# HipGraph/iSpLib

Measured on AMD Instinct MI355X. Metric: edges_aggregated_per_sec, higher is better.
Workload: dtype f32

## Files before the change

### include/isplib_hip.h

```cpp
#ifndef ISPLIB_HIP_H
#define ISPLIB_HIP_H

#include <stddef.h>
#include <stdint.h>

#ifdef __cplusplus
extern "C" {
#endif

#define ISPLIB_HIP_ABI_VERSION 1
#define ISPLIB_MAX_SLICES 4096

#define ISPLIB_VOP_COPY_RHS 0x2
#define ISPLIB_ROP_NOOP     0x00
#define ISPLIB_SOP_COPY     0x100
#define ISPLIB_VSC_MUL      0x1000
#define ISPLIB_VSC_MEAN     0x3000
#define ISPLIB_AOP_ADD      0x10000
#define ISPLIB_AOP_MAX      0x20000
#define ISPLIB_AOP_MIN      0x30000
#define ISPLIB_MSG_SPMM_SUM  (ISPLIB_VOP_COPY_RHS | ISPLIB_ROP_NOOP | ISPLIB_SOP_COPY | ISPLIB_VSC_MUL  | ISPLIB_AOP_ADD)
#define ISPLIB_MSG_SPMM_MEAN (ISPLIB_VOP_COPY_RHS | ISPLIB_ROP_NOOP | ISPLIB_SOP_COPY | ISPLIB_VSC_MEAN | ISPLIB_AOP_ADD)
#define ISPLIB_MSG_SPMM_MAX  (ISPLIB_VOP_COPY_RHS | ISPLIB_ROP_NOOP | ISPLIB_SOP_COPY | ISPLIB_VSC_MUL  | ISPLIB_AOP_MAX)
#define ISPLIB_MSG_SPMM_MIN  (ISPLIB_VOP_COPY_RHS | ISPLIB_ROP_NOOP | ISPLIB_SOP_COPY | ISPLIB_VSC_MUL  | ISPLIB_AOP_MIN)
// ... 103 lines not shown
                              const int64_t *pntrb, const int64_t *pntre,
                              const int64_t *sliceptr, int slices,
                              const float *y, int64_t ldy, float *z, int64_t ldz,
                              int64_t *z_arg, void *workspace,
                              size_t workspace_bytes, void *stream);

int    fusedMM_csr_sliced_phase_hip(int32_t imessage, int64_t m, int64_t n, int64_t k,
                                    int64_t nnz, const float *val, const int64_t *indx,
                                    const int64_t *pntrb, const int64_t *pntre,
                                    const int64_t *sliceptr, int slices,
                                    int slice_first, int slice_count, int combine,
                                    const float *y, int64_t ldy, float *z, int64_t ldz,
                                    int64_t *z_arg, void *workspace,
                                    size_t workspace_bytes, void *stream);

typedef struct isplib_task_plan_info {
   int64_t n_tasks;
   int64_t lane_off[9];
   int32_t slices, chunk, short_row, reserved;
} isplib_task_plan_info;

size_t isplib_spmm_tasks_plan_workspace_bytes(int64_t m, int slices);
int    isplib_spmm_tasks_count_hip(int64_t m, const int64_t *pntrb, const int64_t *pntre,
                                   const int64_t *sliceptr, int slices, int chunk, int short_row,
                                   int32_t *seg_off , void *workspace,
                                   size_t workspace_bytes, isplib_task_plan_info *info ,
                                   void *stream);
int    isplib_spmm_tasks_fill_hip(int64_t m, const int64_t *pntrb, const int64_t *pntre,
                                  const int64_t *sliceptr, const isplib_task_plan_info *info,
                                  const int32_t *seg_off, int32_t *task_row, int64_t *task_b,
                                  int32_t *task_len, void *stream);
size_t isplib_spmm_tasks_workspace_bytes(int32_t imessage, int64_t n_tasks, int64_t k);
int    isplib_pack_indices_hip(int64_t nnz, const int64_t *indx, int32_t *indx32, void *stream);
int    fusedMM_csr_tasks_hip(int32_t imessage, int64_t m, int64_t n, int64_t k, int64_t nnz,
                             const float *val, const int64_t *indx, const int32_t *indx32,
                             const int64_t *pntrb, const int64_t *pntre,
                             int64_t n_tasks, const int32_t *task_row,
                             const int64_t *task_b, const int32_t *task_len,
                             const int32_t *seg_off, int slices,
                             const int64_t *lane_off_host ,
                             const float *y, int64_t ldy, float *z, int64_t ldz,
                             int64_t *z_arg, void *workspace, size_t workspace_bytes,
                             void *stream);

typedef struct isplib_epilogue {
   const float *row_scale;
   const float *self;
   int64_t      ld_self;
   const float *bias;
   int          relu;
} isplib_epilogue;
int    fusedMM_csr_tasks_epilogue_hip(int32_t imessage, int64_t m, int64_t n, int64_t k, int64_t nnz,
                                      const float *val, const int64_t *indx, const int32_t *indx32,
                                      const int64_t *pntrb, const int64_t *pntre,
                                      int64_t n_tasks, const int32_t *task_row,
                                      const int64_t *task_b, const int32_t *task_len,
                                      const int32_t *seg_off, int slices,
                                      const int64_t *lane_off_host ,
                                      const float *y, int64_t ldy, float *z, int64_t ldz,
                                      void *workspace, size_t workspace_bytes,
                                      const isplib_epilogue *epilogue ,
                                      void *stream);

int    isplib_row_scale_hip(int64_t n, int64_t k, const float *x , int64_t ldx, const float *scale ,
                            float *y , int64_t ldy, void *stream);
size_t isplib_masked_scale_colsum_workspace_bytes(int64_t n, int64_t k);
int    isplib_masked_scale_colsum_hip(int64_t n, int64_t k, const float *dz, int64_t lddz, const float *out ,
                                      int64_t ldo, const float *scale , float *gy ,
                                      int64_t ldgy, float *grad_bias , void *workspace, size_t workspace_bytes,
                                      void *stream);

typedef struct isplib_stream_plan {
   int64_t rows, cols;
   int32_t slices, gens, waves_per_gen, rows_per_wave, streams , chunk ;
   int64_t n_steps, n_parts, n_hub;
   const int32_t *words;
   const float   *vals;
   const int64_t *wave_step_off;
   const int32_t *wave_row;
   const int32_t *wave_part;
   const int32_t *hub_row;
   const int32_t *hub_off;
   const int32_t *perm;
} isplib_stream_plan;
int  isplib_stream_plan_build_hip(int64_t m, int64_t n, int64_t nnz, const int64_t *rowptr, const int64_t *col,
                                  const float *val, int streams, int slices, int chunk, int waves_per_gen,
                                  isplib_stream_plan *out , void *stream);
#define ISPLIB_STREAM_CAP_ONE 4096u
int  isplib_stream_capacities_hip(int device, int streams, int waves_per_gen, int64_t nnz, uint32_t *caps ,
                                  int *levelled , void *stream);
int  isplib_stream_plan_build_caps_hip(int64_t m, int64_t n, int64_t nnz, const int64_t *rowptr, const int64_t *col,
                                       const float *val, int streams, int slices, int chunk, int waves_per_gen,
                                       const uint32_t *caps , isplib_stream_plan *out , void *stream);
int  isplib_stream_plan_set_values_hip(isplib_stream_plan *plan, const float *val , void *stream);
void isplib_stream_plan_free(isplib_stream_plan *plan);
int    isplib_spmm_stream_geometry(int streams, int *rows_per_wave , int *waves_resident );
int    isplib_suggest_stream(int64_t m, int64_t n, int64_t nnz, int64_t k, int *streams, int *slices, int *chunk);
int    isplib_suggest_stream_weighted(int64_t m, int64_t n, int64_t nnz, int64_t k, int weighted, int *streams, int *slices, int *chunk);
int    isplib_spmm_stream_minmax_geometry(int streams , int *rows_per_wave , int *waves_resident );
int    isplib_suggest_stream_minmax(int64_t m, int64_t n, int64_t nnz, int64_t k, int *streams, int *slices, int *chunk);
int    isplib_stream_plan_build_minmax_hip(int64_t m, int64_t n, int64_t nnz, const int64_t *rowptr, const int64_t *col,
                                           const float *val, int streams, int slices, int chunk, int waves_per_gen,
                                           isplib_stream_plan *out , void *stream);
size_t isplib_spmm_stream_minmax_workspace_bytes(const isplib_stream_plan *plan);
int    fusedMM_csr_stream_minmax_hip(int32_t imessage , int64_t m, int64_t n, int64_t k,
                                     int64_t nnz, const int64_t *pntrb, const int64_t *pntre,
                                     const isplib_stream_plan *plan ,
                                     const float *y, int64_t ldy, float *z, int64_t ldz, int64_t *z_arg,
                                     void *workspace, size_t workspace_bytes, void *stream);
size_t isplib_spmm_stream_workspace_bytes(const isplib_stream_plan *plan);
int    fusedMM_csr_stream_hip(int32_t imessage , int64_t m, int64_t n, int64_t k,
                              int64_t nnz, const int64_t *pntrb, const int64_t *pntre,
                              const isplib_stream_plan *plan ,
                              const float *y, int64_t ldy, float *z, int64_t ldz,
                              void *workspace, size_t workspace_bytes,
                              const isplib_epilogue *epilogue , void *stream);
#define ISPLIB_DTYPE_BF16 1
#define ISPLIB_DTYPE_F16  2
int    fusedMM_csr_stream16_hip(int32_t imessage , int dtype, int64_t m, int64_t n, int64_t k,
                                int64_t nnz, const int64_t *pntrb, const int64_t *pntre,
                                const isplib_stream_plan *plan ,
                                const void *y, int64_t ldy, void *z, int64_t ldz,
                                void *workspace, size_t workspace_bytes, void *stream);
static inline int isplib_stream16_native_pays(int streams, int weighted) {
   (void)streams; (void)weighted;
   return 0;
}
int    isplib_stream16_auto(int streams, int weighted);
int    fusedMM_csr_rows16_hip(int32_t imessage , int dtype ,
                              int64_t m, int64_t n, int64_t k, int64_t nnz, const float *val ,
                              const int64_t *indx, const int64_t *pntrb, const int64_t *pntre,
                              const int32_t *row_order , const void *y, int64_t ldy, void *z, int64_t ldz, void *stream);
static inline int isplib_rows16_native_pays(int64_t n, int64_t ldy, int ordered, int weighted) {
   const int beyond = n > 0 && ldy > 0 && (double)n * (double)ldy * 2.0 > 256.0 * 1048576.0;
   (void)weighted;
   return (beyond || !ordered) ? 1 : 0;
}
int    isplib_rows16_auto(int64_t n, int64_t ldy, int ordered, int weighted);
int    isplib_rows16_domain(int64_t n, int64_t k, int64_t ldy, int64_t ldz);
int    fusedMM_csr_rows16_colscale_hip(int32_t imessage , int dtype ,
                                       int64_t m, int64_t n, int64_t k, int64_t nnz, const float *col_scale ,
                                       const int64_t *indx, const int64_t *pntrb, const int64_t *pntre,
                                       const int32_t *row_order , const void *y, int64_t ldy, void *z, int64_t ldz, void *stream);
static inline int isplib_rows16_colscale_native_pays(int64_t n, int64_t ldy, int ordered) {
   const int beyond = n > 0 && ldy > 0 && (double)n * (double)ldy * 2.0 > 256.0 * 1048576.0;
   return (beyond || !ordered) ? 1 : 0;
}
int    isplib_rows16_colscale_auto(int64_t n, int64_t ldy, int ordered);
typedef struct isplib_epilogue16 {
   const float *row_scale;
   const float *self_scale;
   const float *bias;
   int          relu;
} isplib_epilogue16;
int    fusedMM_csr_rows16_epilogue_hip(int dtype , int64_t m, int64_t n, int64_t k, int64_t nnz,
                                       const float *col_scale , const int64_t *indx, const int64_t *pntrb,
                                       const int64_t *pntre, const int32_t *row_order , const void *y, int64_t ldy, void *z,
                                       int64_t ldz, const isplib_epilogue16 *epilogue , void *stream);
static inline int isplib_rows16_gcn_native_pays(int64_t n, int64_t ldy, int ordered) {
   (void)ordered;
   return (n > 0 && ldy > 0 && (double)n * (double)ldy * 2.0 > 256.0 * 1048576.0) ? 1 : 0;
}
int    isplib_rows16_gcn_auto(int64_t n, int64_t ldy, int ordered);
size_t isplib_masked_colsum16_workspace_bytes(int64_t n, int64_t k);
int    isplib_masked_colsum16_hip(int dtype, int64_t n, int64_t k, const void *dz, int64_t lddz, const void *out , int64_t ldo,
                                  void *g , int64_t ldg, float *grad_bias , void *workspace,
                                  size_t workspace_bytes, void *stream);
// ... 265 lines not shown
```

### isplib_amd/cabi.py

```python
from __future__ import annotations

import ctypes
import os
from typing import Optional

import torch

from . import _lib

MSG_SPMM_SUM = 0x2 | 0x00 | 0x100 | 0x1000 | 0x10000
MSG_SPMM_MEAN = 0x2 | 0x00 | 0x100 | 0x3000 | 0x10000
MSG_SPMM_MAX = 0x2 | 0x00 | 0x100 | 0x1000 | 0x20000
MSG_SPMM_MIN = 0x2 | 0x00 | 0x100 | 0x1000 | 0x30000
MESSAGE = {"sum": MSG_SPMM_SUM, "add": MSG_SPMM_SUM, "mean": MSG_SPMM_MEAN, "max": MSG_SPMM_MAX, "min": MSG_SPMM_MIN}

SUCCESS, FAIL, NOT_ENOUGH_MEM, NO_OPT_IMPL, HIP_ERROR = 0, 1, -1, 128, 256
UNDEFINED_USER_FUNCTION = 64
ISPLIB_SUCCESS, ISPLIB_FAIL, ISPLIB_NOT_ENOUGH_MEM, ISPLIB_NO_OPT_IMPL, ISPLIB_HIP_ERROR = SUCCESS, FAIL, NOT_ENOUGH_MEM, NO_OPT_IMPL, HIP_ERROR

DENSE_BYTES_MAX = 7 * 2 ** 29
DENSE_OOB_OFFSET = 15 * 2 ** 28
STREAM_N_END = 2 ** 24
STREAM_LDY_END = 2 ** 22
STREAM_NNZ_END = 2 ** 31
# ... 65 lines not shown
        return False
    if heads > 1 and (d < 4 or d & (d - 1)):
        return False
    return ld >= heads * d and rows_gathered < 2 ** 31 and (rows_gathered <= 0 or rows_gathered * ld * 4 <= DENSE_BYTES_MAX)


def gat_edge_serves(nnz: int, heads: int) -> bool:
    return heads >= 1 and 0 <= nnz < 2 ** 31 and nnz * heads * 4 <= DENSE_BYTES_MAX


def gatv2_serves(rows_gathered: int, heads: int, d: int, ld: int) -> bool:
    return gat_serves(rows_gathered, heads, d, ld)


ATTENTION16_K_MIN, ATTENTION16_K_MAX = 8, 512


def attention16_serves(rows_gathered: int, k: int, ld: int) -> bool:
    return (ATTENTION16_K_MIN <= k <= ATTENTION16_K_MAX and k % 2 == 0 and ld % 2 == 0 and ld >= k and rows_gathered < 2 ** 31 and
            (rows_gathered <= 0 or rows_gathered * ld * 2 <= DENSE_BYTES_MAX))


def attention16_native_pays(rows_gathered: int, ld: int) -> bool:
    return bool(rows_gathered > 0 and ld > 0)


GAT16_K_MIN, GAT16_K_MAX = 8, 512


def gat16_serves(rows_gathered: int, heads: int, d: int, ld: int) -> bool:
    if heads < 1 or d < 1 or not GAT16_K_MIN <= heads * d <= GAT16_K_MAX:
        return False
    if (d % 2) if heads == 1 else (d < 8 or d & (d - 1)):
        return False
    return (ld % 2 == 0 and ld >= heads * d and rows_gathered < 2 ** 31 and
            (rows_gathered <= 0 or rows_gathered * ld * 2 <= DENSE_BYTES_MAX))


def gat16_native_pays(rows_gathered: int, ld: int) -> bool:
    return bool(rows_gathered > 0 and ld > 0)


def gatv2_16_serves(rows_gathered: int, heads: int, d: int, ld: int) -> bool:
    return gat16_serves(rows_gathered, heads, d, ld)


def gatv2_16_native_pays(rows_gathered: int, ld: int) -> bool:
    return bool(rows_gathered > 0 and ld > 0)


def owner_exchange_serves(m: int, k: int, world: int, cuts) -> bool:
    if not 1 <= world <= OWNER_WORLD_MAX or m < 0 or k < 0 or m * k >= MINMAX_BW_PAIRS_END:
        return False
    return all(cuts[p + 1] >= cuts[p] and (cuts[p + 1] - cuts[p]) * k <= MINMAX_BW_KEYS_MAX for p in range(world))


def scatter_keys_serves(total: int, n: int, k: int) -> bool:
    return 0 <= total < MINMAX_BW_PAIRS_END and n >= 0 and k >= 0 and n * k <= MINMAX_BW_KEYS_MAX

VOP = {"copy_lhs": 0x1, "copy_rhs": 0x2, "add": 0x3, "subl": 0x4, "subr": 0x5, "max": 0x6, "min": 0x7, "udef": 0xF}
ROP = {"noop": 0x00, "dot": 0x10, "add_lhs": 0x20, "add_rhs": 0x30, "norml": 0x40, "normr": 0x50, "udef": 0xF0}
SOP = {"noop": 0x000, "copy": 0x100, "udef": 0xF00}
VSC = {"noop": 0x0000, "mul": 0x1000, "add": 0x2000, "mean": 0x3000, "udef": 0xF000}
AOP = {"add": 0x10000, "max": 0x20000, "min": 0x30000, "udef": 0xF0000}
SOP_UDEF = {"none": 0, "sigmoid": 1, "one_minus_sigmoid": 2, "tdist": 3, "scale": 4, "exp": 5, "leaky_exp": 6}
PATTERNS = {
    "spmm": (MSG_SPMM_SUM, "none"),
    "sigmoid_embedding": (VOP["copy_rhs"] | ROP["dot"] | SOP["udef"] | VSC["mul"] | AOP["add"], "sigmoid"),
    "tdist_embedding": (VOP["subr"] | ROP["normr"] | SOP["udef"] | VSC["mul"] | AOP["add"], "tdist"),
    "attention_sum": (VOP["copy_rhs"] | ROP["dot"] | SOP["udef"] | VSC["mul"] | AOP["add"], "leaky_exp"),
}

EXPORTS = (
    "isplib_hip_abi_version", "isplib_hip_last_error", "isplib_hip_set_empty_row", "isplib_hip_get_empty_row", "fusedMM_csr_hip", "performDummySpMM_hip",
    "isplib_spmm_minmax_bw_hip", "isplib_sddmm_csr_hip", "isplib_csr_row_ids_hip",
    "isplib_csr2csc_workspace_bytes", "isplib_csr2csc_hip",
    "isplib_spmm_slices_bytes", "isplib_spmm_slices_build_hip", "isplib_spmm_sliced_workspace_bytes",
    "fusedMM_csr_sliced_hip", "fusedMM_csr_sliced_phase_hip", "isplib_hip_tune",
    "isplib_spmm_tasks_workspace_bytes", "fusedMM_csr_tasks_hip",
    "isplib_spmm_tasks_plan_workspace_bytes", "isplib_spmm_tasks_count_hip", "isplib_spmm_tasks_fill_hip",
    "isplib_sddmm_csr_tasks_hip", "fusedMM_csr_tasks_epilogue_hip", "fusedMM_csr_udef_hip", "fusedMM_csr_udef_tasks_hip", "isplib_pack_indices_hip",
    "isplib_suggest_slices", "isplib_graph_create", "isplib_graph_set_slices", "isplib_graph_set_values", "isplib_graph_spmm", "isplib_graph_spmm_backward",
    "isplib_graph_destroy", "isplib_suggest_slices_whole_rows", "isplib_graph_sddmm",
    "fusedMM_csr_stream_hip", "isplib_spmm_stream_workspace_bytes", "isplib_spmm_stream_geometry", "isplib_suggest_stream", "isplib_suggest_stream_weighted", "isplib_stream_plan_build_hip", "isplib_stream_plan_build_caps_hip", "isplib_stream_capacities_hip", "isplib_stream_plan_build_minmax_hip", "fusedMM_csr_stream_minmax_hip", "isplib_spmm_stream_minmax_geometry", "isplib_suggest_stream_minmax", "isplib_spmm_stream_minmax_workspace_bytes", "isplib_stream_plan_set_values_hip", "isplib_stream_plan_free", "isplib_spmm_minmax_bw_det_hip", "isplib_spmm_minmax_bw_workspace_bytes", "isplib_scatter_rows_det_hip",
    "isplib_minmax_bw_bucket_workspace_bytes", "isplib_minmax_bw_bucket_hip", "isplib_scatter_keys_workspace_bytes", "isplib_scatter_keys_det_hip",
    "isplib_fusedmm_stream_geometry", "isplib_suggest_fusedmm_stream", "isplib_stream_plan_build_fusedmm_hip", "fusedMM_csr_udef_stream_hip",
    "isplib_row_scale_hip", "isplib_masked_scale_colsum_hip", "isplib_masked_scale_colsum_workspace_bytes",
    "fusedMM_csr_ordered_hip", "isplib_community_order_hip", "isplib_community_order_workspace_bytes", "isplib_order_locality_hip",
    "isplib_graph_set_row_order", "isplib_plain_panels",
    "fusedMM_csr_stream16_hip", "isplib_stream16_auto",
    "fusedMM_csr_rows16_hip", "isplib_rows16_auto", "isplib_rows16_domain",
    "fusedMM_csr_rows16_minmax_hip", "isplib_rows16_minmax_auto",
    "fusedMM_csr_rows16_colscale_hip", "isplib_rows16_colscale_auto",
    "fusedMM_csr_rows16_epilogue_hip", "isplib_rows16_gcn_auto", "isplib_masked_colsum16_hip", "isplib_masked_colsum16_workspace_bytes",
    "isplib_sddmm_csr_rows16_hip", "isplib_sddmm_rows16_auto",
    "isplib_attention_csr_hip", "isplib_attention_bw_rows_hip", "isplib_attention_bw_cols_hip", "isplib_attention_domain",
    "isplib_attention16_csr_hip", "isplib_attention16_bw_rows_hip", "isplib_attention16_bw_cols_hip", "isplib_attention16_domain",
    "isplib_attention16_auto",
    "isplib_gat_csr_hip", "isplib_gat_bw_rows_hip", "isplib_gat_bw_cols_hip", "isplib_gat_domain",
    "isplib_gat_edge_csr_hip", "isplib_gat_edge_bw_rows_hip", "isplib_gat_edge_bw_cols_hip", "isplib_gat_edge_domain",
    "isplib_gat16_csr_hip", "isplib_gat16_bw_rows_hip", "isplib_gat16_bw_cols_hip", "isplib_gat16_domain", "isplib_gat16_auto",
    "isplib_gatv2_csr_hip", "isplib_gatv2_bw_rows_hip", "isplib_gatv2_bw_rows_workspace_bytes", "isplib_gatv2_bw_cols_hip",
    "isplib_gatv2_domain",
)

GATV2_16_EXPORTS = (
    "isplib_gatv2_16_csr_hip", "isplib_gatv2_16_bw_rows_hip", "isplib_gatv2_16_bw_rows_workspace_bytes", "isplib_gatv2_16_bw_cols_hip",
    "isplib_gatv2_16_domain", "isplib_gatv2_16_auto",
)

EXP_EXPORTS = ("fusedMM_csr_sweep_hip", "isplib_spmm_sweep_workspace_bytes", "isplib_spmm_sweep_resident_waves",
               "fusedMM_csr_hybrid_hip", "isplib_spmm_hybrid_geometry", "isplib_spmm_hybrid_workspace_bytes", "isplib_sddmm_stream_hip",
               "isplib_hip_tune_experimental")

_i64, _f32, _vp, _i32 = ctypes.c_int64, ctypes.c_float, ctypes.c_void_p, ctypes.c_int32


class Epilogue(ctypes.Structure):
    _fields_ = [("row_scale", ctypes.c_void_p), ("self", ctypes.c_void_p), ("ld_self", ctypes.c_int64),
                ("bias", ctypes.c_void_p), ("relu", ctypes.c_int)]


class TaskPlanInfo(ctypes.Structure):
    _fields_ = [("n_tasks", ctypes.c_int64), ("lane_off", ctypes.c_int64 * 9), ("slices", ctypes.c_int32),
                ("chunk", ctypes.c_int32), ("short_row", ctypes.c_int32), ("reserved", ctypes.c_int32)]


class SweepPlanStruct(ctypes.Structure):
    _fields_ = [("rows", ctypes.c_int64), ("slices", ctypes.c_int32), ("gens", ctypes.c_int32),
                ("waves_per_gen", ctypes.c_int32), ("rows_per_wave", ctypes.c_int32), ("n_tasks", ctypes.c_int64),
                ("n_parts", ctypes.c_int64), ("n_hub", ctypes.c_int64), ("wave_row", ctypes.c_void_p),
                ("wave_part", ctypes.c_void_p), ("wave_task_off", ctypes.c_void_p), ("task_b", ctypes.c_void_p),
                ("task_meta", ctypes.c_void_p), ("hub_row", ctypes.c_void_p), ("hub_off", ctypes.c_void_p)]


class StreamPlanStruct(ctypes.Structure):
    _fields_ = [("rows", ctypes.c_int64), ("cols", ctypes.c_int64), ("slices", ctypes.c_int32), ("gens", ctypes.c_int32),
                ("waves_per_gen", ctypes.c_int32), ("rows_per_wave", ctypes.c_int32), ("streams", ctypes.c_int32),
                ("chunk", ctypes.c_int32), ("n_steps", ctypes.c_int64), ("n_parts", ctypes.c_int64), ("n_hub", ctypes.c_int64),
                ("words", ctypes.c_void_p), ("vals", ctypes.c_void_p), ("wave_step_off", ctypes.c_void_p),
                ("wave_row", ctypes.c_void_p), ("wave_part", ctypes.c_void_p),
                ("hub_row", ctypes.c_void_p), ("hub_off", ctypes.c_void_p), ("perm", ctypes.c_void_p)]


class HybridPlanStruct(ctypes.Structure):
    _fields_ = [("cold", StreamPlanStruct), ("table_rows", ctypes.c_int32), ("hot_cap", ctypes.c_int32), ("n_hot_steps", ctypes.c_int64),
                ("hot_rows", ctypes.c_void_p), ("hot_words", ctypes.c_void_p), ("hot_step_off", ctypes.c_void_p),
                ("hot_perm", ctypes.c_void_p)]


_sigs_set = False


def lib() -> ctypes.CDLL:
    global _sigs_set
    L = _lib.cdll()
    if not _sigs_set:
        L.isplib_hip_abi_version.restype = ctypes.c_int
        L.isplib_hip_last_error.restype = ctypes.c_char_p
        L.fusedMM_csr_hip.restype = ctypes.c_int
        L.fusedMM_csr_hip.argtypes = [_i32, _i64, _i64, _i64, _f32, _i64, _i64, _i64, _vp, _vp, _vp, _vp,
                                      _vp, _i64, _vp, _i64, _f32, _vp, _i64, _vp, _vp]
        L.fusedMM_csr_udef_hip.restype = ctypes.c_int
        L.fusedMM_csr_udef_hip.argtypes = [_i32, _i64, _i64, _i64, _f32, _i64, _i64, _i64, _vp, _vp, _vp, _vp,
                                           _vp, _i64, _vp, _i64, _f32, _vp, _i64, _vp, ctypes.c_int, _f32, _vp]
        L.fusedMM_csr_udef_tasks_hip.restype = ctypes.c_int
        L.fusedMM_csr_udef_tasks_hip.argtypes = [_i32, _i64, _i64, _i64, _i64, _vp, _vp, _vp, _vp, _vp, _vp, _i64, _i64, _vp, _vp,
                                                 _vp, _vp, ctypes.c_int, _vp, _vp, _i64, _vp, _i64, _vp, ctypes.c_int, _f32,
                                                 _vp, ctypes.c_size_t, _vp]
        L.performDummySpMM_hip.restype = None
        L.performDummySpMM_hip.argtypes = [_i64, _vp]
        L.isplib_spmm_minmax_bw_hip.restype = ctypes.c_int
        L.isplib_spmm_minmax_bw_hip.argtypes = [_i64, _i64, _i64, _i64, _vp, _vp, _vp, _vp, _vp, _vp, _vp, _vp]
        L.isplib_sddmm_csr_hip.restype = ctypes.c_int
        L.isplib_sddmm_csr_hip.argtypes = [_i64, _i64, _vp, _vp, _vp, _vp, _i64, _vp, _i64, ctypes.c_int, _vp, _vp]
        L.isplib_csr_row_ids_hip.restype = ctypes.c_int
        L.isplib_csr_row_ids_hip.argtypes = [_i64, _i64, _vp, _vp, _vp]
        L.isplib_csr2csc_workspace_bytes.restype = ctypes.c_size_t
        L.isplib_csr2csc_workspace_bytes.argtypes = [_i64, _i64, _i64]
        L.isplib_csr2csc_hip.restype = ctypes.c_int
        L.isplib_csr2csc_hip.argtypes = [_i64, _i64, _i64, _vp, _vp, _vp, ctypes.c_int, _vp, _vp, _vp, _vp,
                                         _vp, ctypes.c_size_t, _vp]
        L.isplib_spmm_slices_bytes.restype = ctypes.c_size_t
        L.isplib_spmm_slices_bytes.argtypes = [_i64, ctypes.c_int]
        L.isplib_spmm_slices_build_hip.restype = ctypes.c_int
        L.isplib_spmm_slices_build_hip.argtypes = [_i64, _i64, _i64, _vp, _vp, _vp, ctypes.c_int, _vp, _vp, _vp]
        L.isplib_spmm_sliced_workspace_bytes.restype = ctypes.c_size_t
        L.isplib_spmm_sliced_workspace_bytes.argtypes = [_i32, _i64, _i64, ctypes.c_int]
        L.fusedMM_csr_sliced_hip.restype = ctypes.c_int
        L.fusedMM_csr_sliced_hip.argtypes = [_i32, _i64, _i64, _i64, _i64, _vp, _vp, _vp, _vp, _vp, ctypes.c_int,
                                             _vp, _i64, _vp, _i64, _vp, _vp, ctypes.c_size_t, _vp]
        L.fusedMM_csr_sliced_phase_hip.restype = ctypes.c_int
        L.fusedMM_csr_sliced_phase_hip.argtypes = [_i32, _i64, _i64, _i64, _i64, _vp, _vp, _vp, _vp, _vp, ctypes.c_int,
                                                   ctypes.c_int, ctypes.c_int, ctypes.c_int, _vp, _i64, _vp, _i64, _vp,
                                                   _vp, ctypes.c_size_t, _vp]
        L.isplib_spmm_tasks_workspace_bytes.restype = ctypes.c_size_t
        L.isplib_spmm_tasks_workspace_bytes.argtypes = [_i32, _i64, _i64]
        L.fusedMM_csr_tasks_hip.restype = ctypes.c_int
        L.isplib_pack_indices_hip.restype = ctypes.c_int
        L.isplib_pack_indices_hip.argtypes = [_i64, _vp, _vp, _vp]
        L.fusedMM_csr_tasks_hip.argtypes = [_i32, _i64, _i64, _i64, _i64, _vp, _vp, _vp, _vp, _vp, _i64, _vp, _vp, _vp, _vp,
                                            ctypes.c_int, _vp, _vp, _i64, _vp, _i64, _vp, _vp, ctypes.c_size_t, _vp]
        L.isplib_spmm_tasks_plan_workspace_bytes.restype = ctypes.c_size_t
        L.isplib_spmm_tasks_plan_workspace_bytes.argtypes = [_i64, ctypes.c_int]
        L.isplib_spmm_tasks_count_hip.restype = ctypes.c_int
        L.isplib_spmm_tasks_count_hip.argtypes = [_i64, _vp, _vp, _vp, ctypes.c_int, ctypes.c_int, ctypes.c_int, _vp, _vp,
                                                  ctypes.c_size_t, ctypes.POINTER(TaskPlanInfo), _vp]
        L.isplib_spmm_tasks_fill_hip.restype = ctypes.c_int
        L.isplib_spmm_tasks_fill_hip.argtypes = [_i64, _vp, _vp, _vp, ctypes.POINTER(TaskPlanInfo), _vp, _vp, _vp, _vp, _vp]
        L.isplib_sddmm_csr_tasks_hip.restype = ctypes.c_int
        L.isplib_sddmm_csr_tasks_hip.argtypes = [_i64, _i64, _i64, _vp, _vp, _vp, _vp, _i64, _vp, _vp, _vp, _vp, _vp, _i64, _vp,
                                                 _i64, ctypes.c_int, _vp, _vp]
        L.fusedMM_csr_tasks_epilogue_hip.restype = ctypes.c_int
        L.fusedMM_csr_tasks_epilogue_hip.argtypes = [_i32, _i64, _i64, _i64, _i64, _vp, _vp, _vp, _vp, _vp, _i64, _vp, _vp, _vp, _vp,
                                                     ctypes.c_int, _vp, _vp, _i64, _vp, _i64, _vp, ctypes.c_size_t,
                                                     ctypes.POINTER(Epilogue), _vp]
        L.isplib_suggest_slices.restype = ctypes.c_int
        L.isplib_suggest_slices.argtypes = [_i64, _i64, _i64, _i64, ctypes.c_int]
        L.isplib_graph_create.restype = ctypes.c_int
        L.isplib_graph_create.argtypes = [_i64, _i64, _i64, _vp, _vp, _vp, ctypes.POINTER(_vp)]
        L.isplib_graph_set_slices.restype = ctypes.c_int
        L.isplib_graph_set_slices.argtypes = [_vp, ctypes.c_int]
        L.isplib_graph_set_values.restype = ctypes.c_int
        L.isplib_graph_set_values.argtypes = [_vp, _vp]
        L.isplib_graph_spmm.restype = ctypes.c_int
        L.isplib_graph_spmm.argtypes = [_vp, _i32, _i64, _vp, _i64, _vp, _i64, _vp, _vp]
        L.isplib_graph_spmm_backward.restype = ctypes.c_int
        L.isplib_graph_spmm_backward.argtypes = [_vp, ctypes.c_int, _i64, _vp, _i64, _vp, _i64, _vp]
        L.isplib_suggest_slices_whole_rows.restype = ctypes.c_int
        L.isplib_suggest_slices_whole_rows.argtypes = [_i64, _i64, _i64, _i64]
        L.isplib_graph_sddmm.restype = ctypes.c_int
        L.isplib_graph_sddmm.argtypes = [_vp, ctypes.c_int, _i64, _vp, _i64, _vp, _i64, _vp, _vp]
        L.isplib_graph_destroy.restype = None
        L.isplib_graph_destroy.argtypes = [_vp]
        L.isplib_hip_tune.restype = ctypes.c_int
        L.isplib_hip_tune.argtypes = [ctypes.c_int, ctypes.c_int]
        L.isplib_spmm_minmax_bw_workspace_bytes.restype = ctypes.c_size_t
        L.isplib_spmm_minmax_bw_workspace_bytes.argtypes = [_i64, _i64, _i64]
        L.isplib_spmm_minmax_bw_det_hip.restype = ctypes.c_int
        L.isplib_spmm_minmax_bw_det_hip.argtypes = [_i64, _i64, _i64, _i64, _vp, _vp, _vp, _vp, _vp, _vp, _vp, _vp, ctypes.c_size_t, _vp]
        L.isplib_fusedmm_stream_geometry.restype = ctypes.c_int
        L.isplib_fusedmm_stream_geometry.argtypes = [ctypes.c_int, ctypes.POINTER(ctypes.c_int), ctypes.POINTER(ctypes.c_int)]
        L.isplib_suggest_fusedmm_stream.restype = ctypes.c_int
        L.isplib_suggest_fusedmm_stream.argtypes = [_i32, _i64, _i64, _i64, _i64] + [ctypes.POINTER(ctypes.c_int)] * 3
        L.isplib_stream_plan_build_fusedmm_hip.restype = ctypes.c_int
        L.isplib_stream_plan_build_fusedmm_hip.argtypes = [_i64, _i64, _i64, _vp, _vp, ctypes.c_int, ctypes.c_int, ctypes.c_int, ctypes.c_int,
                                                           ctypes.POINTER(StreamPlanStruct), _vp]
        L.fusedMM_csr_udef_stream_hip.restype = ctypes.c_int
        L.fusedMM_csr_udef_stream_hip.argtypes = [_i32, _i64, _i64, _i64, _i64, _vp, _vp, ctypes.POINTER(StreamPlanStruct), _vp, _i64, _vp, _i64,
                                                  _vp, _i64, ctypes.c_int, _f32, _vp, ctypes.c_size_t, _vp]
        L.isplib_row_scale_hip.restype = ctypes.c_int
        L.isplib_row_scale_hip.argtypes = [_i64, _i64, _vp, _i64, _vp, _vp, _i64, _vp]
        L.isplib_masked_scale_colsum_workspace_bytes.restype = ctypes.c_size_t
        L.isplib_masked_scale_colsum_workspace_bytes.argtypes = [_i64, _i64]
        L.isplib_masked_scale_colsum_hip.restype = ctypes.c_int
        L.isplib_masked_scale_colsum_hip.argtypes = [_i64, _i64, _vp, _i64, _vp, _i64, _vp, _vp, _i64, _vp, _vp, ctypes.c_size_t, _vp]
        L.isplib_scatter_rows_det_hip.restype = ctypes.c_int
        L.isplib_scatter_rows_det_hip.argtypes = [_i64, _i64, _i64, _i64, _vp, _vp, _vp, _vp, ctypes.c_size_t, _vp]
        L.isplib_minmax_bw_bucket_workspace_bytes.restype = ctypes.c_size_t
        L.isplib_minmax_bw_bucket_workspace_bytes.argtypes = [_i64, _i64, ctypes.c_int]
        L.isplib_minmax_bw_bucket_hip.restype = ctypes.c_int
        L.isplib_minmax_bw_bucket_hip.argtypes = [_i64, _i64, _i64, _i64, _vp, _vp, _vp, _vp, ctypes.c_int, ctypes.POINTER(_i64), _vp, _vp, _vp,
                                                  _vp, ctypes.c_size_t, _vp]
        L.isplib_scatter_keys_workspace_bytes.restype = ctypes.c_size_t
        L.isplib_scatter_keys_workspace_bytes.argtypes = [_i64, _i64, _i64]
        L.isplib_scatter_keys_det_hip.restype = ctypes.c_int
        L.isplib_scatter_keys_det_hip.argtypes = [_i64, _i64, _i64, _vp, _vp, _vp, _vp, ctypes.c_size_t, _vp]
        L.isplib_stream_plan_build_hip.restype = ctypes.c_int
        L.isplib_stream_plan_build_hip.argtypes = [_i64, _i64, _i64, _vp, _vp, _vp, ctypes.c_int, ctypes.c_int, ctypes.c_int, ctypes.c_int,
                                                   ctypes.POINTER(StreamPlanStruct), _vp]
        L.isplib_stream_plan_build_caps_hip.restype = ctypes.c_int
        L.isplib_stream_plan_build_caps_hip.argtypes = [_i64, _i64, _i64, _vp, _vp, _vp, ctypes.c_int, ctypes.c_int, ctypes.c_int, ctypes.c_int,
                                                        _vp, ctypes.POINTER(StreamPlanStruct), _vp]
        L.isplib_stream_capacities_hip.restype = ctypes.c_int
        L.isplib_stream_capacities_hip.argtypes = [ctypes.c_int, ctypes.c_int, ctypes.c_int, _i64, _vp, ctypes.POINTER(ctypes.c_int), _vp]
        L.isplib_stream_level_set.restype = ctypes.c_int
        L.isplib_stream_level_set.argtypes = [ctypes.c_int]
        L.isplib_stream_plan_build_minmax_hip.restype = ctypes.c_int
        L.isplib_stream_plan_build_minmax_hip.argtypes = [_i64, _i64, _i64, _vp, _vp, _vp, ctypes.c_int, ctypes.c_int, ctypes.c_int, ctypes.c_int,
                                                          ctypes.POINTER(StreamPlanStruct), _vp]
        L.isplib_spmm_stream_minmax_geometry.restype = ctypes.c_int
        L.isplib_spmm_stream_minmax_geometry.argtypes = [ctypes.c_int, ctypes.POINTER(ctypes.c_int), ctypes.POINTER(ctypes.c_int)]
        L.isplib_suggest_stream_minmax.restype = ctypes.c_int
        L.isplib_suggest_stream_minmax.argtypes = [_i64, _i64, _i64, _i64, ctypes.POINTER(ctypes.c_int), ctypes.POINTER(ctypes.c_int), ctypes.POINTER(ctypes.c_int)]
        L.isplib_spmm_stream_minmax_workspace_bytes.restype = ctypes.c_size_t
        L.isplib_spmm_stream_minmax_workspace_bytes.argtypes = [ctypes.POINTER(StreamPlanStruct)]
        L.fusedMM_csr_stream_minmax_hip.restype = ctypes.c_int
        L.fusedMM_csr_stream_minmax_hip.argtypes = [_i32, _i64, _i64, _i64, _i64, _vp, _vp, ctypes.POINTER(StreamPlanStruct), _vp, _i64,
                                                    _vp, _i64, _vp, _vp, ctypes.c_size_t, _vp]
        L.isplib_stream_plan_set_values_hip.restype = ctypes.c_int
        L.isplib_stream_plan_set_values_hip.argtypes = [ctypes.POINTER(StreamPlanStruct), _vp, _vp]
        L.isplib_stream_plan_free.restype = None
        L.isplib_stream_plan_free.argtypes = [ctypes.POINTER(StreamPlanStruct)]
        L.isplib_community_order_workspace_bytes.restype = ctypes.c_size_t
        L.isplib_community_order_workspace_bytes.argtypes = [_i64, _i64]
        L.isplib_community_order_hip.restype = ctypes.c_int
        L.isplib_community_order_hip.argtypes = [_i64, _i64, _vp, _vp, ctypes.c_int, ctypes.c_int, _vp, _vp, ctypes.POINTER(ctypes.c_int), _vp,
                                                 ctypes.c_size_t, _vp]
        L.isplib_order_locality_hip.restype = ctypes.c_int
        L.isplib_order_locality_hip.argtypes = [_i64, _i64, _vp, _vp, _vp, _i64, ctypes.POINTER(ctypes.c_double), _vp, ctypes.c_size_t, _vp]
        L.isplib_graph_set_row_order.restype = ctypes.c_int
        L.isplib_graph_set_row_order.argtypes = [_vp, _vp, _vp]
        L.fusedMM_csr_ordered_hip.restype = ctypes.c_int
        L.fusedMM_csr_ordered_hip.argtypes = [_i32, _i64, _i64, _i64, _i64, _vp, _vp, _vp, _vp, _vp, _vp, _i64, _vp, _i64, _vp, _vp]
        L.isplib_plain_panels.restype = ctypes.c_int
        L.isplib_plain_panels.argtypes = [_i64, _i64]
        L.isplib_suggest_stream.restype = ctypes.c_int
        L.isplib_suggest_stream.argtypes = [_i64, _i64, _i64, _i64, ctypes.POINTER(ctypes.c_int), ctypes.POINTER(ctypes.c_int), ctypes.POINTER(ctypes.c_int)]
        L.isplib_suggest_stream_weighted.restype = ctypes.c_int
        L.isplib_suggest_stream_weighted.argtypes = [_i64, _i64, _i64, _i64, ctypes.c_int, ctypes.POINTER(ctypes.c_int), ctypes.POINTER(ctypes.c_int), ctypes.POINTER(ctypes.c_int)]
        L.isplib_spmm_stream_geometry.restype = ctypes.c_int
        L.isplib_spmm_stream_geometry.argtypes = [ctypes.c_int, ctypes.POINTER(ctypes.c_int), ctypes.POINTER(ctypes.c_int)]
        L.isplib_spmm_stream_workspace_bytes.restype = ctypes.c_size_t
        L.isplib_spmm_stream_workspace_bytes.argtypes = [ctypes.POINTER(StreamPlanStruct)]
        L.fusedMM_csr_stream_hip.restype = ctypes.c_int
        L.fusedMM_csr_stream_hip.argtypes = [_i32, _i64, _i64, _i64, _i64, _vp, _vp, ctypes.POINTER(StreamPlanStruct), _vp, _i64,
                                             _vp, _i64, _vp, ctypes.c_size_t, ctypes.POINTER(Epilogue), _vp]
        L.fusedMM_csr_stream16_hip.restype = ctypes.c_int
        L.fusedMM_csr_stream16_hip.argtypes = [_i32, ctypes.c_int, _i64, _i64, _i64, _i64, _vp, _vp, ctypes.POINTER(StreamPlanStruct), _vp, _i64,
                                               _vp, _i64, _vp, ctypes.c_size_t, _vp]
        L.isplib_stream16_auto.restype = ctypes.c_int
        L.isplib_stream16_auto.argtypes = [ctypes.c_int, ctypes.c_int]
        L.fusedMM_csr_rows16_hip.restype = ctypes.c_int
        L.fusedMM_csr_rows16_hip.argtypes = [_i32, ctypes.c_int, _i64, _i64, _i64, _i64, _vp, _vp, _vp, _vp, _vp, _vp, _i64, _vp, _i64, _vp]
        L.isplib_rows16_auto.restype = ctypes.c_int
        L.isplib_rows16_auto.argtypes = [_i64, _i64, ctypes.c_int, ctypes.c_int]
        L.isplib_rows16_domain.restype = ctypes.c_int
        L.isplib_rows16_domain.argtypes = [_i64, _i64, _i64, _i64]
        L.fusedMM_csr_rows16_minmax_hip.restype = ctypes.c_int
        L.fusedMM_csr_rows16_minmax_hip.argtypes = [_i32, ctypes.c_int, _i64, _i64, _i64, _i64, _vp, _vp, _vp, _vp, _vp, _vp, _i64, _vp, _i64, _vp, _i64, _vp]
        L.isplib_rows16_minmax_auto.restype = ctypes.c_int
        L.isplib_rows16_minmax_auto.argtypes = [_i64, _i64, ctypes.c_int, ctypes.c_int, ctypes.c_int]
        L.fusedMM_csr_rows16_colscale_hip.restype = ctypes.c_int
        L.fusedMM_csr_rows16_colscale_hip.argtypes = [_i32, ctypes.c_int, _i64, _i64, _i64, _i64, _vp, _vp, _vp, _vp, _vp, _vp, _i64, _vp, _i64, _vp]
        L.isplib_rows16_colscale_auto.restype = ctypes.c_int
        L.isplib_rows16_colscale_auto.argtypes = [_i64, _i64, ctypes.c_int]
        L.fusedMM_csr_rows16_epilogue_hip.restype = ctypes.c_int
        L.fusedMM_csr_rows16_epilogue_hip.argtypes = [ctypes.c_int, _i64, _i64, _i64, _i64, _vp, _vp, _vp, _vp, _vp, _vp, _i64, _vp, _i64, _vp, _vp]
        L.isplib_rows16_gcn_auto.restype = ctypes.c_int
        L.isplib_rows16_gcn_auto.argtypes = [_i64, _i64, ctypes.c_int]
        L.isplib_masked_colsum16_workspace_bytes.restype = ctypes.c_size_t
        L.isplib_masked_colsum16_workspace_bytes.argtypes = [_i64, _i64]
        L.isplib_masked_colsum16_hip.restype = ctypes.c_int
        L.isplib_masked_colsum16_hip.argtypes = [ctypes.c_int, _i64, _i64, _vp, _i64, _vp, _i64, _vp, _i64, _vp, _vp, ctypes.c_size_t, _vp]
        L.isplib_sddmm_csr_rows16_hip.restype = ctypes.c_int
        L.isplib_sddmm_csr_rows16_hip.argtypes = [ctypes.c_int, _i64, _i64, _i64, _i64, _vp, _vp, _vp, _vp, _vp, _i64, _vp, _i64, ctypes.c_int, _vp, _vp]
        L.isplib_sddmm_rows16_auto.restype = ctypes.c_int
        L.isplib_sddmm_rows16_auto.argtypes = [_i64, _i64, ctypes.c_int]
        L.isplib_attention_domain.restype = ctypes.c_int
        L.isplib_attention_domain.argtypes = [_i64, _i64, _i64]
        L.isplib_attention_csr_hip.restype = ctypes.c_int
        L.isplib_attention_csr_hip.argtypes = [_i64, _i64, _i64, _i64, _vp, _vp, _vp, _vp, _i64, _vp, _i64, _f32, _vp, _i64, _vp, _vp]
        L.isplib_attention_bw_rows_hip.restype = ctypes.c_int
        L.isplib_attention_bw_rows_hip.argtypes = [_i64, _i64, _i64, _i64, _vp, _vp, _vp, _vp, _i64, _vp, _i64, _f32, _vp, _i64, _vp, _i64, _vp,
                                                   _vp, _i64, _vp, _vp]
        L.isplib_attention_bw_cols_hip.restype = ctypes.c_int
        L.isplib_attention_bw_cols_hip.argtypes = [_i64, _i64, _i64, _i64, _vp, _vp, _vp, _vp, _i64, _vp, _i64, _f32, _vp, _i64, _vp, _vp, _vp,
                                                   _i64, _vp]
# ... 2138 lines not shown
    return tuple(x.value for x in v)


def fusedMM_csr_hybrid_hip(imessage: int, rowptr, nnz: int, plan, y, z, workspace=None, epilogue=None, check: bool = True) -> int:
    assert y.is_cuda and y.dtype == torch.float32 and y.dim() == 2 and y.stride(1) == 1
    m, n, k = rowptr.numel() - 1, y.size(0), y.size(1)
    rp = rowptr.data_ptr()
    ps = plan.struct()
    with torch.cuda.device(y.device):
        st = exp_lib().fusedMM_csr_hybrid_hip(int(imessage), m, n, k, int(nnz), ctypes.c_void_p(rp), ctypes.c_void_p(rp + 8),
                                          ctypes.byref(ps), _ptr(y), y.stride(0) if n > 1 else max(k, y.stride(0)), _ptr(z),
                                          z.stride(0) if m > 1 else max(k, z.stride(0)), _ptr(workspace),
                                          0 if workspace is None else workspace.numel(),
                                          None if epilogue is None else ctypes.byref(epilogue), _stream(y.device))
    if check:
        _check(st, "fusedMM_csr_hybrid_hip")
    return st


def spmm_hybrid(rowptr, nnz: int, plan, y, reduce: str = "sum", workspace=None, row_scale=None, self_term=None, bias=None, relu=False):
    rowptr = _dev(rowptr, "rowptr", torch.int64)
    y = y.contiguous()
    m, k = rowptr.numel() - 1, y.size(1)
    out = torch.empty((m, k), dtype=torch.float32, device=y.device)
    if workspace is None:
        workspace = plan.workspace()
    ep = None
    if row_scale is not None or self_term is not None or bias is not None or relu:
        ep = Epilogue(None if row_scale is None else row_scale.data_ptr(), None if self_term is None else self_term.data_ptr(),
                      k if self_term is None else self_term.stride(0), None if bias is None else bias.data_ptr(), int(bool(relu)))
    fusedMM_csr_hybrid_hip(MESSAGE[reduce], rowptr, nnz, plan, y, out, workspace, ep)
    return out


def suggest_stream(m: int, n: int, nnz: int, k: int, weighted: bool = False):
    st, sl, ch = ctypes.c_int(0), ctypes.c_int(0), ctypes.c_int(0)
    if not lib().isplib_suggest_stream_weighted(int(m), int(n), int(nnz), int(k), int(bool(weighted)), ctypes.byref(st), ctypes.byref(sl), ctypes.byref(ch)):
        return None
    return st.value, sl.value, ch.value


class _DevView:

    def __init__(self, ptr: int, count: int, typestr: str, owner=None):
        self.__cuda_array_interface__ = {"shape": (count,), "typestr": typestr, "data": (ptr, False), "version": 2}
        self._owner = owner


class NativeStreamPlan:

    def __init__(self, rowptr, col, val, ncols: int, streams: int, slices: int, chunk: int, waves_per_gen: int = 0,
                 minmax: bool = False, fusedmm: bool = False, capacities=None):
        assert capacities is None or not (minmax or fusedmm), "max / min and FusedMM plans keep equal capacities"
        self._s = StreamPlanStruct()
        self.device = col.device
        m = rowptr.numel() - 1
        with torch.cuda.device(col.device):
            if fusedmm:
                _check(lib().isplib_stream_plan_build_fusedmm_hip(m, int(ncols), col.numel(), _ptr(rowptr), _ptr(col), int(streams), int(slices),
                                                                  int(chunk), int(waves_per_gen), ctypes.byref(self._s), _stream(col.device)),
                       "isplib_stream_plan_build_fusedmm_hip")
            elif minmax:
                _check(lib().isplib_stream_plan_build_minmax_hip(m, int(ncols), col.numel(), _ptr(rowptr), _ptr(col), _ptr(val),
                                                                 int(streams), int(slices), int(chunk), int(waves_per_gen), ctypes.byref(self._s),
                                                                 _stream(col.device)), "isplib_stream_plan_build_minmax_hip")
            elif capacities is not None:
                caps = (ctypes.c_uint32 * len(capacities))(*[int(c) for c in capacities])
                rpw, resident = stream_geometry(streams)
                if len(caps) != (int(waves_per_gen) if waves_per_gen > 0 else resident):
                    raise ValueError("one capacity per wave of a generation")
                _check(lib().isplib_stream_plan_build_caps_hip(m, int(ncols), col.numel(), _ptr(rowptr), _ptr(col), _ptr(val), int(streams),
                                                               int(slices), int(chunk), int(waves_per_gen), ctypes.cast(caps, _vp),
                                                               ctypes.byref(self._s), _stream(col.device)), "isplib_stream_plan_build_caps_hip")
            else:
                _check(lib().isplib_stream_plan_build_hip(m, int(ncols), col.numel(), _ptr(rowptr), _ptr(col), _ptr(val), int(streams),
                                                          int(slices), int(chunk), int(waves_per_gen), ctypes.byref(self._s),
                                                          _stream(col.device)), "isplib_stream_plan_build_hip")
        for name in ("rows", "cols", "slices", "gens", "waves_per_gen", "rows_per_wave", "streams", "n_steps", "n_parts", "n_hub"):
            setattr(self, name, int(getattr(self._s, name)))

    def struct(self):
        return self._s

    def workspace(self, minmax: bool = False):
        L = lib()
        nbytes = (L.isplib_spmm_stream_minmax_workspace_bytes if minmax else L.isplib_spmm_stream_workspace_bytes)(ctypes.byref(self._s))
        return torch.empty(nbytes, dtype=torch.uint8, device=self.device)

    def set_values(self, val):
        with torch.cuda.device(self.device):
            _check(lib().isplib_stream_plan_set_values_hip(ctypes.byref(self._s), _ptr(val), _stream(self.device)), "isplib_stream_plan_set_values_hip")

    def array(self, name: str) -> torch.Tensor:
        nw = self.gens * self.waves_per_gen
        count, typestr = {"words": (self.n_steps * self.streams, "<i4"), "perm": (self.n_steps * self.streams, "<i4"),
                          "vals": (self.n_steps * self.streams, "<f4"), "wave_step_off": (nw + 1, "<i8"),
                          "wave_row": (nw * self.rows_per_wave, "<i4"), "wave_part": (nw * self.rows_per_wave, "<i4"),
                          "hub_row": (self.n_hub, "<i4"), "hub_off": (self.n_hub + 1, "<i4")}[name]
        ptr = getattr(self._s, name)
        if not ptr or count == 0:
            return torch.empty(0, device=self.device)
        return torch.as_tensor(_DevView(ptr, count, typestr), device=self.device).clone()

    def view(self, name: str, dtype: torch.dtype) -> torch.Tensor:
        nw = self.gens * self.waves_per_gen
        count, typestr = {"words": (self.n_steps * self.streams, "<i4"), "perm": (self.n_steps * self.streams, "<i4"),
                          "wave_step_off": (nw + 1, "<i8"), "wave_row": (nw * self.rows_per_wave, "<i4"),
                          "wave_part": (nw * self.rows_per_wave, "<i4"), "hub_row": (self.n_hub, "<i4"),
                          "hub_off": (self.n_hub + 1, "<i4")}[name]
        ptr = getattr(self._s, name)
        if not ptr or count == 0:
            return torch.empty(0, dtype=dtype, device=self.device)
        t = torch.as_tensor(_DevView(ptr, count, typestr, owner=self), device=self.device)
        assert t.dtype == dtype and t.data_ptr() == ptr, "zero-copy view of a library array"
        return t

    def close(self):
        if self._s.words or self._s.wave_row:
            lib().isplib_stream_plan_free(ctypes.byref(self._s))

    def __del__(self):
        try:
            self.close()
        except Exception:
            pass


STREAM_CAP_ONE = 4096


def stream_capacities(device, streams: int, waves_per_gen: int, nnz: int):
    device = torch.device(device)
    if device.type != "cuda":
        return None
    _, resident = stream_geometry(streams)
    wpg = int(waves_per_gen) if waves_per_gen > 0 else resident
    caps = (ctypes.c_uint32 * wpg)()
    levelled = ctypes.c_int(0)
    with torch.cuda.device(device):
        _check(lib().isplib_stream_capacities_hip(-1, int(streams), wpg, int(nnz), ctypes.cast(caps, _vp), ctypes.byref(levelled),
                                                  _stream(device)), "isplib_stream_capacities_hip")
    return list(caps) if levelled.value else None


def stream_level_set(mode: int) -> None:
    _check(lib().isplib_stream_level_set(int(mode)), "isplib_stream_level_set")


def stream_geometry(streams: int = 4):
    rpw, res = ctypes.c_int(0), ctypes.c_int(0)
    _check(lib().isplib_spmm_stream_geometry(int(streams), ctypes.byref(rpw), ctypes.byref(res)), "isplib_spmm_stream_geometry")
    return rpw.value, res.value


def sweep_resident_waves(reduce: str, k: int, rows_per_wave: int = 16) -> int:
    return int(exp_lib().isplib_spmm_sweep_resident_waves(MESSAGE[reduce], int(k), int(rows_per_wave)))


class GraphHandle:

    def __init__(self, rowptr, col, val, ncols: int):
        self.rowptr = _dev(rowptr, "rowptr", torch.int64)
        self.col = _dev(col, "col", torch.int64)
        self.val = None if val is None else _dev(val, "val", torch.float32)
        self.m, self.n = self.rowptr.numel() - 1, int(ncols)
        self._cols_ok = None
        self._h = ctypes.c_void_p()
        with torch.cuda.device(self.col.device):
            _check(lib().isplib_graph_create(self.m, self.n, self.col.numel(), _ptr(self.rowptr), _ptr(self.col),
                                             _ptr(self.val), ctypes.byref(self._h)), "isplib_graph_create")

    def set_slices(self, slices: int) -> None:
        _check(lib().isplib_graph_set_slices(self._h, int(slices)), "isplib_graph_set_slices")

    def set_row_order(self, order, order_t=None) -> None:
        self.order = None if order is None else _dev(order, "order", torch.int32)
        self.order_t = None if order_t is None else _dev(order_t, "order_t", torch.int32)
        assert self.order is None or self.order.numel() == self.m
        assert self.order_t is None or self.order_t.numel() == self.n
        _check(lib().isplib_graph_set_row_order(self._h, _ptr(self.order), _ptr(self.order_t)), "isplib_graph_set_row_order")

    def set_values(self, val) -> None:
        self.val = None if val is None else _dev(val, "val", torch.float32)
        assert self.val is None or self.val.numel() == self.col.numel()
        _check(lib().isplib_graph_set_values(self._h, _ptr(self.val)), "isplib_graph_set_values")

    def spmm(self, y: torch.Tensor, reduce: str = "sum"):
        if not (y.is_cuda and y.dtype == torch.float32 and y.dim() == 2 and y.stride(1) == 1 and y.stride(0) >= y.size(1)):
            y = _dev(y, "y", torch.float32)
        k = y.size(1)
        ldy = y.stride(0) if y.size(0) > 1 else max(k, y.stride(0))
        out = torch.empty((self.m, k), dtype=torch.float32, device=y.device)
        arg = torch.empty((self.m, k), dtype=torch.int64, device=y.device) if reduce in ("max", "min") else None
        with torch.cuda.device(y.device):
            _check(lib().isplib_graph_spmm(self._h, MESSAGE[reduce], k, _ptr(y), ldy, _ptr(out), k, _ptr(arg), _stream(y.device)),
                   "isplib_graph_spmm")
        return out, arg

    def spmm_backward(self, dy: torch.Tensor, mean: bool = False) -> torch.Tensor:
        dy = _dev(dy, "dy", torch.float32)
        k = dy.size(1)
        dx = torch.empty((self.n, k), dtype=torch.float32, device=dy.device)
        with torch.cuda.device(dy.device):
            _check(lib().isplib_graph_spmm_backward(self._h, int(bool(mean)), k, _ptr(dy), k, _ptr(dx), k, _stream(dy.device)),
                   "isplib_graph_spmm_backward")
        return dx

    def sddmm(self, y: torch.Tensor, g: torch.Tensor, mean: bool = False, *, out=None, check: bool = True) -> torch.Tensor:
        _, _, out, ldy, ldg = _sddmm_operands(self.rowptr, self.col, y, g, out, False, self.n, "the handle")
        if check and self._cols_ok is None:
            self._cols_ok = self.col.numel() == 0 or (int(self.col.min()) >= 0 and int(self.col.max()) < self.n)
        if check and not self._cols_ok:
            raise ValueError(f"isplib_amd: the handle's column ids must lie in [0, {self.n})")
        k = y.size(1)
        with torch.cuda.device(y.device):
            _check(lib().isplib_graph_sddmm(self._h, int(bool(mean)), k, _ptr(y), ldy, _ptr(g), ldg, _ptr(out), _stream(y.device)),
                   "isplib_graph_sddmm")
        return out

    def close(self) -> None:
        if self._h:
            lib().isplib_graph_destroy(self._h)
            self._h = ctypes.c_void_p()

    def __del__(self):
        try:
            self.close()
# ... 3 lines not shown
```

### isplib_amd/csrc/common.h

```cpp
#pragma once
#include <hip/hip_runtime.h>
#include <stdio.h>
#include <string.h>

#include "../../include/isplib_hip.h"

namespace isplib {

char *error_buffer();
int empty_row_init();

int stream_stage_mode();
void stream_stage_report(unsigned panels);
int stream_kernel_calibrate(int streams, int waves_per_gen, int launches, int degree, int col_mult, double *wave_ticks, hipStream_t st);
int stream_level_mode();

inline void clear_error() { error_buffer()[0] = '\0'; }

inline int fail(int code, const char *msg) {
   snprintf(error_buffer(), 512, "%s", msg);
   return code;
}

inline int fail(int code, const char *entry, const char *msg) {
   snprintf(error_buffer(), 512, "%s: %s", entry, msg);
   return code;
}

inline int hip_fail(hipError_t e, const char *what) {
   snprintf(error_buffer(), 512, "%s: %s", what, hipGetErrorString(e));
   return ISPLIB_HIP_ERROR;
}

__attribute__((noinline)) inline int check_launch(const char *what) {
   const hipError_t e = hipGetLastError();
   return e == hipSuccess ? ISPLIB_SUCCESS : hip_fail(e, what);
}

#define ISPLIB_HIP_TRY(expr)                                        \
   do {                                                             \
      const hipError_t e_ = (expr);                                 \
      if (e_ != hipSuccess) return ::isplib::hip_fail(e_, #expr);   \
   } while (0)

}
```

### isplib_amd/csrc/runtime.hip

```cpp
#include <stdlib.h>
#include <string.h>

#include "common.h"

namespace isplib {
char *error_buffer() {
   static thread_local char buf[512] = {0};
   return buf;
}
}

namespace isplib {
static int g_empty_row = -1;
int empty_row_init() {
   if (g_empty_row < 0) {
      const char *e = getenv("ISPLIB_EMPTY_ROW");
      g_empty_row = (e && (strcmp(e, "init") == 0 || strcmp(e, "1") == 0)) ? 1 : 0;
   }
   return g_empty_row;
}
}

extern "C" int isplib_hip_set_empty_row(int init) {
   isplib::clear_error();
   if (init != 0 && init != 1) return isplib::fail(ISPLIB_FAIL, "isplib_hip_set_empty_row: 0 (zero) or 1 (the launcher's init value)");
   isplib::g_empty_row = init;
   return ISPLIB_SUCCESS;
}
extern "C" int isplib_hip_get_empty_row(void) { return isplib::empty_row_init(); }

namespace isplib {
static int g_stream_stage = -1;
static thread_local unsigned g_stream_stage_last = 0;
int stream_stage_mode() {
   if (g_stream_stage < 0) {
      const char *e = getenv("ISPLIB_STREAM_STAGE");
      g_stream_stage = !e ? ISPLIB_STAGE_AUTO : strcmp(e, "0") == 0 ? ISPLIB_STAGE_OFF : strcmp(e, "1") == 0 ? ISPLIB_STAGE_FORCE : ISPLIB_STAGE_AUTO;
   }
   return g_stream_stage;
}
void stream_stage_report(unsigned panels) { g_stream_stage_last = panels; }
}

extern "C" int isplib_stream_stage_set(int mode) {
   isplib::clear_error();
   if (mode != ISPLIB_STAGE_OFF && mode != ISPLIB_STAGE_FORCE && mode != ISPLIB_STAGE_AUTO) return isplib::fail(ISPLIB_FAIL, "isplib_stream_stage_set: 0 (off), 1 (force) or 2 (auto)");
   isplib::g_stream_stage = mode;
   return ISPLIB_SUCCESS;
}
extern "C" unsigned isplib_stream_stage_last(void) { return isplib::g_stream_stage_last; }

namespace isplib {
static int g_stream_level = -1;
int stream_level_mode() {
   if (g_stream_level < 0) {
      const char *e = getenv("ISPLIB_STREAM_LEVEL");
      g_stream_level = !e ? 2 : strcmp(e, "0") == 0 ? 0 : strcmp(e, "1") == 0 ? 1 : 2;
   }
   return g_stream_level;
}
}

extern "C" int isplib_stream_level_set(int mode) {
   isplib::clear_error();
   if (mode < 0 || mode > 2) return isplib::fail(ISPLIB_FAIL, "isplib_stream_level_set: 0 (off), 1 (on) or 2 (auto)");
   isplib::g_stream_level = mode;
   return ISPLIB_SUCCESS;
}

extern "C" int isplib_hip_abi_version(void) { return ISPLIB_HIP_ABI_VERSION; }
extern "C" const char *isplib_hip_last_error(void) { return isplib::error_buffer(); }
```

### isplib_amd/csrc/spmm_sweep.hip

```cpp
#include <vector>

#include "sweep_common.h"

extern "C" void isplib_debug_wave_times(unsigned long long *buf);

namespace isplib {

template <int LPR, bool HAS_VAL, int NVMAX, int NBW, int WGS, bool TIMED = false>
__global__ __launch_bounds__(256, (stream_wgs_per_cu<LPR, NVMAX, WGS>())) void spmm_stream_kernel(const SweepArgs a) {
   using Wave = StreamWave<LPR, NVMAX, NBW>;
   constexpr int WAVES = Wave::WAVES, G = Wave::G, PANEL = Wave::PANEL, U = Wave::U, PER = Wave::PER;
   constexpr int WAVE_FLOATS = NVMAX * PANEL;
   static_assert(NVMAX <= 256 && NVMAX % G == 0, "the local row is the top byte of a word");
   __shared__ __attribute__((aligned(16))) float s_all[WAVES * WAVE_FLOATS];
   Wave sw;
   if (!stream_wave_id(a, sw)) return;
   const int lane = sw.lane;
   unsigned long long t_start = 0, t_loop = 0, t_loop_end = 0;
   if constexpr (TIMED) t_start = __builtin_amdgcn_s_memtime();
   float *my = s_all + sw.wave * WAVE_FLOATS;
   for (int i = lane * 4; i < WAVE_FLOATS; i += 256)
      *reinterpret_cast<float4 *>(my + i) = make_float4(0.0f, 0.0f, 0.0f, 0.0f);
   __amdgpu_buffer_rsrc_t rsrc = dense_rsrc(a);
   stream_columns<true>(a, sw);
   float *lane_base = my + sw.lc * 4;
   stream_bounds(a, sw);
   const float *vp = HAS_VAL ? a.vals + sw.s0 * G : nullptr;
   unsigned w1[NBW], w2[NBW];
   float v0[NBW] = {}, v1[NBW] = {};
   v4i_t t[U];
   unsigned la[U];
   const unsigned pad_word = stream_pad_own_row(a, sw);
   stream_load_batch(sw, sw.wp, 0, pad_word, w1);
   if (HAS_VAL) stream_load_batch(sw, vp, 0, 0.0f, v0);
#pragma unroll
   for (int u = 0; u < U; u++) stream_issue<ISPLIB_EXP_GATHER_AUX>(sw, rsrc, w1, u, la[u], t[u]);
   stream_load_batch(sw, sw.wp, 64 * NBW, pad_word, w1);
   if (HAS_VAL) stream_load_batch(sw, vp, 64 * NBW, 0.0f, v1);
   stream_load_batch(sw, sw.wp, 128 * NBW, pad_word, w2);
   unsigned cur = (unsigned)(sw.g * PER * PANEL);
   float acc[4] = {0.0f, 0.0f, 0.0f, 0.0f};
   const int64_t nb = (sw.nwords + 64 * NBW - 1) / (64 * NBW);
   if constexpr (TIMED) t_loop = __builtin_amdgcn_s_memtime();
   for (int64_t b = 0; b < nb; b++) {
      float vnext = HAS_VAL ? __shfl(v0[0], sw.g) : 0.0f;
#pragma unroll
      for (int u = 0; u < U; u++) {
         const float vcur = vnext;
         if (HAS_VAL && u + 1 < U) vnext = __shfl(v0[((u + 1) * G) / 64], ((u + 1) * G) % 64 + sw.g);
         if (la[u] != cur) {
            stream_flush(lane_base + cur, acc);
            cur = la[u];
            acc[0] = acc[1] = acc[2] = acc[3] = 0.0f;
         }
#pragma unroll
         for (int v = 0; v < 4; v++) {
            const float x = __int_as_float(t[u][v]);
            acc[v] = HAS_VAL ? fmaf(vcur, x, acc[v]) : acc[v] + x;
         }
         stream_issue<ISPLIB_EXP_GATHER_AUX>(sw, rsrc, w1, u, la[u], t[u]);
      }
#pragma unroll
      for (int q = 0; q < NBW; q++) { w1[q] = w2[q]; v0[q] = v1[q]; }
      stream_load_batch(sw, sw.wp, (b + 3) * 64 * NBW, pad_word, w2);
      if (HAS_VAL) stream_load_batch(sw, vp, (b + 2) * 64 * NBW, 0.0f, v1);
   }
   stream_flush(lane_base + cur, acc);
   if constexpr (TIMED) t_loop_end = __builtin_amdgcn_s_memtime();
   int row_[PER], part_[PER];
#pragma unroll
   for (int jj = 0; jj < PER; jj++) {
      row_[jj] = sw.cok ? a.wave_row[(size_t)sw.w * NVMAX + sw.g * PER + jj] : -1;
      part_[jj] = a.wave_part[(size_t)sw.w * NVMAX + sw.g * PER + jj];
   }
#pragma unroll 4
   for (int jj = 0; jj < PER; jj++) {
      const int lrow = sw.g * PER + jj;
      const int row = row_[jj];
      if (row < 0) continue;
      const int part = part_[jj];
      const float4 t4 = *reinterpret_cast<const float4 *>(lane_base + lrow * PANEL);
      float v[4] = {t4.x, t4.y, t4.z, t4.w};
      int bi[4] = {INT_MAX, INT_MAX, INT_MAX, INT_MAX};
      const int c = sw.ccol;
      if (part >= 0) {
         store_tail<4>(a.part_val + (size_t)part * (size_t)a.k + c, v, sw.vfirst);
         continue;
      }
      int64_t arg[4];
      finish_row<OP_ADD>(a, row, c, v, bi, arg);
      store_tail<4>(a.z + (size_t)row * (size_t)a.ldz + c, v, sw.vfirst);
   }
   if constexpr (TIMED) if (a.dbg && lane == 0) {
      a.dbg[(size_t)sw.wl * 5 + 0] = t_start;
      a.dbg[(size_t)sw.wl * 5 + 1] = t_loop;
      a.dbg[(size_t)sw.wl * 5 + 2] = t_loop_end;
      a.dbg[(size_t)sw.wl * 5 + 3] = __builtin_amdgcn_s_memtime();
      a.dbg[(size_t)sw.wl * 5 + 4] = (__builtin_amdgcn_s_getreg(20u | (3u << 11)) << 24) | ((__builtin_amdgcn_s_getreg(4u | (31u << 11)) >> 8) & 0xFFFFu);
   }
}

typedef float v2f_t __attribute__((ext_vector_type(2)));

template <int OP, int LPR, bool HAS_VAL, int NVMAX, int NBW, int WGS, bool ARG>
__global__ __launch_bounds__(256, (stream_wgs_per_cu<LPR, 2 * (NVMAX + 1), WGS>())) void spmm_stream_minmax_kernel(const SweepArgs a) {
   using Wave = StreamWave<LPR, NVMAX, NBW>;
   constexpr int WAVES = Wave::WAVES, G = Wave::G, PANEL = Wave::PANEL, U = Wave::U, PER = Wave::PER;
   constexpr int ROWS = NVMAX + 1;
   constexpr int WAVE_DWORDS = 2 * ROWS * PANEL;
   constexpr int IDX0 = ROWS * PANEL;
   constexpr int NONE = INT_MAX;
   static_assert(ROWS <= 256 && NVMAX % G == 0, "the local row (and the spare row) is the top byte of a word");
   __shared__ __attribute__((aligned(16))) float s_all[WAVES * WAVE_DWORDS];
   Wave sw;
   if (!stream_wave_id(a, sw)) return;
   const int lane = sw.lane;
   float *my = s_all + sw.wave * WAVE_DWORDS;
   for (int i = lane * 4; i < ROWS * PANEL; i += 256)
      *reinterpret_cast<float4 *>(my + i) = make_float4(identity<OP>(), identity<OP>(), identity<OP>(), identity<OP>());
   if (ARG)
      for (int i = lane * 4; i < ROWS * PANEL; i += 256)
         *reinterpret_cast<int4 *>(my + IDX0 + i) = make_int4(INT_MAX, INT_MAX, INT_MAX, INT_MAX);
   __amdgpu_buffer_rsrc_t rsrc = dense_rsrc(a);
   stream_columns<true>(a, sw);
   const unsigned cbyte = sw.cok ? sw.cbyte : 0x80000000u;
   float *lane_base = my + sw.lc * 4;
   int *lane_idx = reinterpret_cast<int *>(my + IDX0) + sw.lc * 4;
   stream_bounds(a, sw);
   const float *vp = HAS_VAL ? a.vals + sw.s0 * G : nullptr;
   const unsigned pad_word = stream_pad_spare_row(a, sw);
   const int g4 = sw.g * 4;
   unsigned w1[NBW], w2[NBW];
   float v0[NBW] = {}, v1[NBW] = {};
   v4i_t t[U];
   unsigned la[U];
   auto fetch = [&](int u, const unsigned (&word_l)[NBW]) {
      return (unsigned)__builtin_amdgcn_ds_bpermute(g4 + (int)(((u * G) % 64) * 4), (int)word_l[(u * G) / 64]);
   };
   auto issue = [&](int u, unsigned word) {
      const unsigned o = __umul24(word, sw.ldyb) + cbyte;
      la[u] = word;
      t[u] = __builtin_amdgcn_raw_buffer_load_b128(rsrc, (int)o, 0, 0);
   };
   stream_load_batch(sw, sw.wp, 0, pad_word, w1);
   if (HAS_VAL) stream_load_batch(sw, vp, 0, 0.0f, v0);
#pragma unroll
   for (int u = 0; u < U; u++) issue(u, fetch(u, w1));
// ... 64 lines not shown
   const int32_t *ids = a.ids + sw.s0 * G;
   int row_[PER], part_[PER], best_[PER][4];
   float val_[PER][4];
#pragma unroll
   for (int jj = 0; jj < PER; jj++) {
      const int lrow = sw.g * PER + jj;
      row_[jj] = sw.cok ? a.wave_row[(size_t)sw.w * NVMAX + lrow] : -1;
      part_[jj] = a.wave_part[(size_t)sw.w * NVMAX + lrow];
      const float4 t4 = *reinterpret_cast<const float4 *>(lane_base + lrow * PANEL);
      val_[jj][0] = t4.x; val_[jj][1] = t4.y; val_[jj][2] = t4.z; val_[jj][3] = t4.w;
      if constexpr (ARG) {
         const int4 i4 = *reinterpret_cast<const int4 *>(lane_idx + lrow * PANEL);
         best_[jj][0] = i4.x; best_[jj][1] = i4.y; best_[jj][2] = i4.z; best_[jj][3] = i4.w;
      } else {
         best_[jj][0] = best_[jj][1] = best_[jj][2] = best_[jj][3] = INT_MAX;
      }
   }
   if constexpr (ARG) {
#pragma unroll
      for (int jj = 0; jj < PER; jj++)
#pragma unroll
         for (int i = 0; i < 4; i++)
            best_[jj][i] = (row_[jj] >= 0 && (unsigned)best_[jj][i] < (unsigned)sw.nwords) ? ids[best_[jj][i]] : INT_MAX;
   }
#pragma unroll
   for (int jj = 0; jj < PER; jj++) {
      const int row = row_[jj];
      if (row < 0) continue;
      const int c = sw.ccol;
      if (part_[jj] >= 0) {
         const size_t po = (size_t)part_[jj] * (size_t)a.k + c;
         store_tail<4>(a.part_val + po, val_[jj], sw.vfirst);
         if constexpr (ARG) {
#pragma unroll
            for (int i = 0; i < 4; i++) if (i >= sw.vfirst) a.part_idx[po + i] = best_[jj][i];
         }
         continue;
      }
      int64_t arg[4];
      finish_row<OP>(a, row, c, val_[jj], best_[jj], arg);
      store_tail<4>(a.z + (size_t)row * (size_t)a.ldz + c, val_[jj], sw.vfirst);
      if (a.z_arg) {
         int64_t *ar = a.z_arg + (size_t)row * (size_t)a.ldz + c;
#pragma unroll
         for (int i = 0; i < 4; i++) if (i >= sw.vfirst) ar[i] = arg[i];
      }
   }
}


__global__ __launch_bounds__(256) void stream_stage_copy_kernel(const float *__restrict__ y, int64_t ldy, int64_t n, float *__restrict__ dst) {
   const int64_t total = n * 16;
   const int64_t stride = (int64_t)gridDim.x * blockDim.x;
   for (int64_t i = (int64_t)blockIdx.x * blockDim.x + threadIdx.x; i < total; i += stride) {
      const int64_t r = i >> 4;
      const int j = (int)(i & 15) * 4;
      *reinterpret_cast<float4 *>(dst + r * (ISPLIB_STREAM_STAGE_PITCH / 4) + j) = *reinterpret_cast<const float4 *>(y + r * ldy + j);
   }
}

static int launch_stage_copy(const float *y, int64_t ldy, int64_t n, float *dst, hipStream_t st) {
   int64_t blocks = (n * 16 + 255) / 256;
   if (blocks > 4096) blocks = 4096;
   if (blocks <= 0) return ISPLIB_SUCCESS;
   hipLaunchKernelGGL(stream_stage_copy_kernel, dim3((unsigned)blocks), dim3(256), 0, st, y, ldy, n, dst);
   return check_launch("stream_stage_copy_kernel");
}

static thread_local unsigned long long *g_dbg = nullptr;
static thread_local int g_dbg_launch = 0;
template <int STREAMS, bool HAS_VAL>
static int launch_stream(const SweepArgs &a_in, hipStream_t st) {
   constexpr StreamGeom ge = stream_geom(STREAM_SUM, STREAMS);
   SweepArgs a = a_in;
   const unsigned blocks = (unsigned)((a.wave_count + 3) / 4);
   if (blocks == 0) return ISPLIB_SUCCESS;
   if constexpr (!HAS_VAL) {
      if (g_dbg) {
         a.dbg = g_dbg + (size_t)(g_dbg_launch++ % 4) * (size_t)a.wave_count * 5;
         hipLaunchKernelGGL((spmm_stream_kernel<ge.lpr, false, ge.nvmax, ge.nbw, ge.wgs, true>), dim3(blocks), dim3(256), 0, st, a);
         return check_launch("spmm_stream_kernel");
      }
   }
   hipLaunchKernelGGL((spmm_stream_kernel<ge.lpr, HAS_VAL, ge.nvmax, ge.nbw, ge.wgs>), dim3(blocks), dim3(256), 0, st, a);
   return check_launch("spmm_stream_kernel");
}

template <int OP, int STREAMS, bool HAS_VAL, bool ARG>
static void launch_minmax_kernel(const SweepArgs &a, unsigned blocks, hipStream_t st) {
   constexpr StreamGeom ge = stream_geom(STREAM_MINMAX, STREAMS);
   hipLaunchKernelGGL((spmm_stream_minmax_kernel<OP, ge.lpr, HAS_VAL, ge.nvmax, ge.nbw, ge.wgs, ARG>), dim3(blocks), dim3(256), 0, st, a);
}

template <int OP, bool HAS_VAL>
static int launch_stream_minmax(const SweepArgs &a, hipStream_t st, int streams) {
   const unsigned blocks = (unsigned)((a.wave_count + 3) / 4);
   if (blocks == 0) return ISPLIB_SUCCESS;
   return with_streams<STREAM_MINMAX>(streams, [&](auto s) {
      if (a.z_arg) launch_minmax_kernel<OP, s(), HAS_VAL, true>(a, blocks, st);
      else launch_minmax_kernel<OP, s(), HAS_VAL, false>(a, blocks, st);
      return check_launch("spmm_stream_minmax_kernel");
   });
}

}

using namespace isplib;


extern "C" int isplib_spmm_stream_geometry(int streams, int *rows_per_wave, int *waves_resident) {
   return stream_geometry("isplib_spmm_stream_geometry", STREAM_SUM, streams, rows_per_wave, waves_resident);
}

extern "C" int isplib_spmm_stream_minmax_geometry(int streams, int *rows_per_wave, int *waves_resident) {
   return stream_geometry("isplib_spmm_stream_minmax_geometry", STREAM_MINMAX, streams, rows_per_wave, waves_resident);
}

extern "C" int isplib_suggest_stream_weighted(int64_t m, int64_t n, int64_t nnz, int64_t k, int weighted, int *streams, int *slices, int *chunk) {
   clear_error();
   if (m <= 0 || n <= 0 || nnz < STREAM_MIN_NNZ) return 0;
   if (!isplib_stream_serves(n, k, k, nnz, 0)) return 0;
   int st = k <= 32 ? 8 : (k <= 64 ? 4 : (k < 128 ? 2 : 4));
   if (weighted && k >= 128 && (k % 128) == 0) st = 2;
   int rpw = 0, resident = 0;
   if (isplib_spmm_stream_geometry(st, &rpw, &resident) != ISPLIB_SUCCESS || rpw <= 0 || resident <= 0) return 0;
   if (!suggest_stream_geom(m, n, nnz, st, rpw, resident, 1.9e6, 3.4, slices, chunk)) {
      if (st != 2 || k < 128) return 0;
      st = 4;
      if (isplib_spmm_stream_geometry(st, &rpw, &resident) != ISPLIB_SUCCESS || rpw <= 0 || resident <= 0) return 0;
      if (!suggest_stream_geom(m, n, nnz, st, rpw, resident, 1.9e6, 3.4, slices, chunk)) return 0;
   }
   if (streams) *streams = st;
   return 1;
}

extern "C" int isplib_suggest_stream(int64_t m, int64_t n, int64_t nnz, int64_t k, int *streams, int *slices, int *chunk) {
   return isplib_suggest_stream_weighted(m, n, nnz, k, 0, streams, slices, chunk);
}

extern "C" int isplib_suggest_stream_minmax(int64_t m, int64_t n, int64_t nnz, int64_t k, int *streams, int *slices, int *chunk) {
   clear_error();
   if (m <= 0 || n <= 0 || nnz < STREAM_MIN_NNZ) return 0;
   if (!isplib_stream_serves(n, k, k, nnz, 1)) return 0;
   const int st = k <= 32 ? 8 : 4;
   int rpw = 0, resident = 0;
   if (isplib_spmm_stream_minmax_geometry(st, &rpw, &resident) != ISPLIB_SUCCESS || rpw <= 0 || resident <= 0) return 0;
   if (!suggest_stream_geom(m, n, nnz, st, rpw, resident, 3.3e6, st == 8 ? 1.7 : 1.17, slices, chunk)) return 0;
   if (streams) *streams = st;
   return 1;
}

extern "C" size_t isplib_spmm_stream_workspace_bytes(const isplib_stream_plan *plan) {
   size_t bytes = stream_parts_bytes(plan);
   if (plan && plan->streams == 4 && plan->cols > 0 && (uint64_t)plan->cols <= (ISPLIB_STREAM_STAGE_BYTES_MAX - ISPLIB_STREAM_STAGE_PITCH) / ISPLIB_STREAM_STAGE_PITCH)
      bytes += (size_t)plan->cols * ISPLIB_STREAM_STAGE_PITCH + ISPLIB_STREAM_STAGE_PITCH;
   return bytes;
}

extern "C" size_t isplib_spmm_stream_minmax_workspace_bytes(const isplib_stream_plan *plan) {
   return 2 * stream_parts_bytes(plan);
}

static int stream_run(int32_t imessage, int64_t m, int64_t n, int64_t k, int64_t nnz, const int64_t *pntrb, const int64_t *pntre,
                      const isplib_stream_plan *plan, const float *y, int64_t ldy, float *z, int64_t ldz, int64_t *z_arg,
                      void *workspace, size_t workspace_bytes, const isplib_epilogue *ep, void *stream) {
   clear_error();
   const char *entry = "fusedMM_csr_stream_hip";
   const bool mm = imessage == ISPLIB_MSG_SPMM_MAX || imessage == ISPLIB_MSG_SPMM_MIN;
   if (imessage != ISPLIB_MSG_SPMM_SUM && imessage != ISPLIB_MSG_SPMM_MEAN && !mm) return fail(ISPLIB_NO_OPT_IMPL, entry, "message outside the SpMM set");
   const StreamCall c = {entry, "fusedMM_csr_hip", mm ? STREAM_MINMAX : STREAM_SUM, m, n, k, nnz,  m == 0 || k == 0, pntrb, pntre, plan, y, ldy,
                          ldz,  z != nullptr,  true, workspace, workspace_bytes, (mm ? 2 : 1) * stream_parts_bytes(plan)};
   bool done;
   int rc = check_stream_call(c, &done);
   if (done) return rc;
   if (mm && plan->n_steps > 0 && !plan->perm) return fail(ISPLIB_FAIL, entry, "max / min need the plan's perm array (the winners' CSR positions)");
   if (mm && nnz >= ISPLIB_STREAM_NNZ_END) return fail(ISPLIB_FAIL, entry, "max / min need nnz < 2^31");
   if (mm && !isplib_rows_within(n, ldy, ISPLIB_STREAM_MINMAX_BYTES_END - 1u))
      return fail(ISPLIB_FAIL, "fusedMM_csr_stream_minmax_hip", "dense operand of 2 GiB or more (use fusedMM_csr_tasks_hip)");
   if ((rc = check_stream_workspace(c)) != ISPLIB_SUCCESS) return rc;
   SweepArgs a = stream_args(c, z, ldz);
   a.z_arg = z_arg;
   a.mean = imessage == ISPLIB_MSG_SPMM_MEAN ? 1 : 0;
   a.part_idx = mm && workspace ? (int *)((char *)workspace + stream_parts_bytes(plan)) : nullptr;
   if ((rc = set_epilogue(entry, ep, a)) != ISPLIB_SUCCESS) return rc;
   hipStream_t st = (hipStream_t)stream;
   const bool has_val = plan->vals != nullptr;
   const int stage_mode = mm ? ISPLIB_STAGE_OFF : stream_stage_mode();
   float *stage_base = nullptr;
   uint64_t stage_room = 0;
   if (stage_mode != ISPLIB_STAGE_OFF && workspace) {
      const uintptr_t lo = ((uintptr_t)workspace + stream_parts_bytes(plan) + (ISPLIB_STREAM_STAGE_PITCH - 1)) & ~(uintptr_t)(ISPLIB_STREAM_STAGE_PITCH - 1);
      const uintptr_t hi = (uintptr_t)workspace + workspace_bytes;
      if (lo < hi) { stage_base = (float *)lo; stage_room = hi - lo; }
   }
   unsigned staged = 0;
   auto stage = [&](SweepArgs &p, int64_t c0) {
      if (!isplib_stream_stage_panel((uint64_t)(uintptr_t)y, ldy, c0, k, plan->streams, n, nnz, stage_room, stage_mode)) return (int)ISPLIB_SUCCESS;
      const int rc = launch_stage_copy(p.y, ldy, n, stage_base, st);
      if (rc) return rc;
      p.y = stage_base;
      p.ldy = ISPLIB_STREAM_STAGE_PITCH / 4;
      p.ybytes = (unsigned)((uint64_t)n * ISPLIB_STREAM_STAGE_PITCH);
      staged |= 1u << ((c0 / 64) & 31);
      return (int)ISPLIB_SUCCESS;
   };
   const int rc_run = run_stream_panels(plan, a,
      [&](const SweepArgs &p) {
         if (imessage == ISPLIB_MSG_SPMM_MAX) return has_val ? launch_stream_minmax<OP_MAX, true>(p, st, plan->streams) : launch_stream_minmax<OP_MAX, false>(p, st, plan->streams);
         if (imessage == ISPLIB_MSG_SPMM_MIN) return has_val ? launch_stream_minmax<OP_MIN, true>(p, st, plan->streams) : launch_stream_minmax<OP_MIN, false>(p, st, plan->streams);
         return with_streams<STREAM_SUM>(plan->streams, [&](auto s) { return has_val ? launch_stream<s(), true>(p, st) : launch_stream<s(), false>(p, st); });
      },
      [&](const SweepArgs &p) {
         return imessage == ISPLIB_MSG_SPMM_MAX ? launch_hub_fold<OP_MAX, true>(p, st)
              : imessage == ISPLIB_MSG_SPMM_MIN ? launch_hub_fold<OP_MIN, true>(p, st) : launch_hub_fold<OP_ADD, true>(p, st);
      }, stage);
   if (!mm) stream_stage_report(staged);
   return rc_run;
}

extern "C" int fusedMM_csr_stream_hip(int32_t imessage, int64_t m, int64_t n, int64_t k, int64_t nnz,
                                      const int64_t *pntrb, const int64_t *pntre, const isplib_stream_plan *plan,
                                      const float *y, int64_t ldy, float *z, int64_t ldz, void *workspace,
                                      size_t workspace_bytes, const isplib_epilogue *ep, void *stream) {
   if (imessage != ISPLIB_MSG_SPMM_SUM && imessage != ISPLIB_MSG_SPMM_MEAN) {
      clear_error();
      return fail(ISPLIB_NO_OPT_IMPL, "fusedMM_csr_stream_hip: sum and mean only (max / min: fusedMM_csr_stream_minmax_hip)");
   }
   return stream_run(imessage, m, n, k, nnz, pntrb, pntre, plan, y, ldy, z, ldz, nullptr, workspace, workspace_bytes, ep, stream);
}

extern "C" int fusedMM_csr_stream_minmax_hip(int32_t imessage, int64_t m, int64_t n, int64_t k, int64_t nnz,
                                             const int64_t *pntrb, const int64_t *pntre, const isplib_stream_plan *plan,
                                             const float *y, int64_t ldy, float *z, int64_t ldz, int64_t *z_arg,
                                             void *workspace, size_t workspace_bytes, void *stream) {
   if (imessage != ISPLIB_MSG_SPMM_MAX && imessage != ISPLIB_MSG_SPMM_MIN) {
      clear_error();
      return fail(ISPLIB_NO_OPT_IMPL, "fusedMM_csr_stream_minmax_hip: max and min only");
   }
   return stream_run(imessage, m, n, k, nnz, pntrb, pntre, plan, y, ldy, z, ldz, z_arg, workspace, workspace_bytes, nullptr, stream);
}

namespace isplib {
__global__ __launch_bounds__(256) void stream_calib_graph_kernel(int64_t n, int64_t ncols, int64_t degree, int64_t *__restrict__ rowptr, int64_t *__restrict__ col) {
   const int64_t stride = (int64_t)gridDim.x * blockDim.x, nnz = n * degree;
   for (int64_t i = (int64_t)blockIdx.x * blockDim.x + threadIdx.x; i <= n; i += stride) rowptr[i] = i * degree;
   for (int64_t e = (int64_t)blockIdx.x * blockDim.x + threadIdx.x; e < nnz; e += stride) {
      uint64_t h = (uint64_t)e * 0x9E3779B97F4A7C15ull;
      h ^= h >> 29; h *= 0xBF58476D1CE4E5B9ull; h ^= h >> 32;
      col[e] = (int64_t)(h % (uint64_t)ncols);
   }
}

int stream_kernel_calibrate(int streams, int waves_per_gen, int launches, int degree, int col_mult, double *wave_ticks, hipStream_t st) {
   int rpw = 0, resident = 0;
   if (isplib_spmm_stream_geometry(streams, &rpw, &resident) != ISPLIB_SUCCESS) return ISPLIB_FAIL;
   if (waves_per_gen < 4 || waves_per_gen % 4 != 0 || waves_per_gen > resident || launches < 1 || launches > 16 || degree < 1 || degree > 1024 ||
       col_mult < 1 || col_mult > 8)
      return fail(ISPLIB_FAIL, "stream calibration: whole workgroups of one resident generation, 1..16 launches");
   const int64_t n = (int64_t)waves_per_gen * rpw, ncols = n * col_mult, nnz = n * degree, k = 256 / streams;
   struct Temps {
      std::vector<void *> p;
      isplib_stream_plan plan;
      unsigned long long *callers_dbg = g_dbg;
      Temps() { memset(&plan, 0, sizeof(plan)); }
      ~Temps() { isplib_debug_wave_times(callers_dbg); isplib_stream_plan_free(&plan); for (void *q : p) (void)hipFree(q); }
      void *get(size_t bytes) { void *q = nullptr; if (hipMalloc(&q, bytes) != hipSuccess) { (void)hipGetLastError(); return nullptr; } p.push_back(q); return q; }
   } T;
   int64_t *rowptr = (int64_t *)T.get((size_t)(n + 1) * 8), *col = (int64_t *)T.get((size_t)nnz * 8);
   float *y = (float *)T.get((size_t)ncols * k * 4), *z = (float *)T.get((size_t)n * k * 4);
// ... 28 lines not shown
```

### isplib_amd/csrc/stream_plan.hip

```cpp
#include <hip/hip_runtime.h>
#include <stdint.h>
#include <string.h>

#include <map>
#include <mutex>
#include <new>
#include <tuple>
#include <vector>

#include "../../include/isplib_hip.h"
#include "common.h"

#include "prims.h"
#include "sweep_common.h"

namespace isplib {

static inline unsigned sp_grid(int64_t n) {
   int64_t b = (n + 255) / 256;
   if (b < 1) b = 1;
   if (b > 256 * 64) b = 256 * 64;
   return (unsigned)b;
}

// ... 76 lines not shown
   }
}

__device__ __forceinline__ int64_t sp_row_of(int64_t e, int64_t m, const int64_t *rowptr) {
   int64_t lo = 0, hi = m;
   while (hi - lo > 1) {
      const int64_t mid = lo + (hi - lo) / 2;
      if (rowptr[mid] <= e) lo = mid; else hi = mid;
   }
   return lo;
}

__global__ __launch_bounds__(256) void sp_edge_keys_kernel(int64_t m, int64_t nnz, int64_t width, int slices, int per, int snake,
                                                           const int64_t *__restrict__ rowptr, const int64_t *__restrict__ col,
                                                           const int *__restrict__ nchunk, const int *__restrict__ first,
                                                           const int *__restrict__ sid, const int *__restrict__ rnd,
                                                           uint32_t *__restrict__ keys, uint32_t *__restrict__ vals) {
   const int64_t stride = (int64_t)gridDim.x * blockDim.x;
   for (int64_t e = (int64_t)blockIdx.x * blockDim.x + threadIdx.x; e < nnz; e += stride) {
      const int64_t row = sp_row_of(e, m, rowptr);
      const int v = first[row] + (int)((e - rowptr[row]) % nchunk[row]);
      const int64_t sl = col[e] / width;
      keys[e] = (uint32_t)(((int64_t)sid[v] * slices + sl) * per + ((snake && (sl & 1)) ? per - 1 - rnd[v] : rnd[v]));
      vals[e] = (uint32_t)e;
   }
}

__global__ __launch_bounds__(256) void sp_pad_kernel(int64_t n_words, int streams, int per, int pad_row, uint32_t null_col, int32_t *__restrict__ words,
                                                     int32_t *__restrict__ perm, float *__restrict__ vals) {
   const int64_t stride = (int64_t)gridDim.x * blockDim.x;
   for (int64_t i = (int64_t)blockIdx.x * blockDim.x + threadIdx.x; i < n_words; i += stride) {
      const uint32_t lrow = pad_row >= 0 ? (uint32_t)pad_row : (uint32_t)(i % streams) * (uint32_t)per;
      words[i] = (int32_t)((lrow << 24) | null_col);
      perm[i] = -1;
      if (vals) vals[i] = 0.0f;
   }
}

__global__ __launch_bounds__(256) void sp_place_kernel(int64_t m, int64_t nnz, int streams, int per, const int64_t *__restrict__ rowptr,
                                                       const int64_t *__restrict__ col, const float *__restrict__ val,
                                                       const int *__restrict__ nchunk, const int *__restrict__ first,
                                                       const int *__restrict__ sid, const int *__restrict__ rnd,
                                                       const uint32_t *__restrict__ sorted_e, const int64_t *__restrict__ stream_start,
                                                       const int64_t *__restrict__ wave_step_off, int32_t *__restrict__ words,
                                                       int32_t *__restrict__ perm, float *__restrict__ vals) {
   const int64_t stride = (int64_t)gridDim.x * blockDim.x;
   for (int64_t q = (int64_t)blockIdx.x * blockDim.x + threadIdx.x; q < nnz; q += stride) {
      const int64_t e = (int64_t)sorted_e[q];
      const int64_t row = sp_row_of(e, m, rowptr);
      const int v = first[row] + (int)((e - rowptr[row]) % nchunk[row]);
      const int s = sid[v];
      const int64_t p = q - stream_start[s];
      const int64_t idx = (wave_step_off[s / streams] + p) * streams + s % streams;
      const uint32_t lrow = (uint32_t)((s % streams) * per + rnd[v]);
      words[idx] = (int32_t)((lrow << 24) | (uint32_t)col[e]);
      perm[idx] = (int32_t)e;
      if (vals) vals[idx] = val[e];
   }
}

__global__ __launch_bounds__(256) void sp_wave_rows_kernel(int64_t nv, int streams, int per, int rows_per_wave,
                                                           const int *__restrict__ vrow_row, const int *__restrict__ vhub,
                                                           const int *__restrict__ part_of, const int *__restrict__ sid,
                                                           const int *__restrict__ rnd, int32_t *__restrict__ wave_row,
                                                           int32_t *__restrict__ wave_part, const int *__restrict__ first,
                                                           const int *__restrict__ hub_idx, int32_t *__restrict__ hub_off) {
   const int64_t stride = (int64_t)gridDim.x * blockDim.x;
   for (int64_t v = (int64_t)blockIdx.x * blockDim.x + threadIdx.x; v < nv; v += stride) {
      const int s = sid[v];
      const int64_t at = (int64_t)(s / streams) * rows_per_wave + (s % streams) * per + rnd[v];
      const int row = vrow_row[v];
      wave_row[at] = row;
      wave_part[at] = vhub[v] ? part_of[v] : -1;
      if (vhub[v] && first[row] == (int)v) hub_off[hub_idx[row]] = part_of[v];
   }
}

__global__ __launch_bounds__(256) void sp_gather_vals_kernel(int64_t n_words, const int32_t *__restrict__ perm, const float *__restrict__ src,
                                                             float *__restrict__ vals) {
   const int64_t stride = (int64_t)gridDim.x * blockDim.x;
   for (int64_t i = (int64_t)blockIdx.x * blockDim.x + threadIdx.x; i < n_words; i += stride) vals[i] = perm[i] >= 0 ? src[perm[i]] : 0.0f;
}

struct SpTemp {
   std::vector<void *> ptrs;
   ~SpTemp() { for (void *p : ptrs) (void)hipFree(p); }
   template <class T> bool alloc(T **out, size_t count) {
      void *p = nullptr;
      if (hipMalloc(&p, (count ? count : 1) * sizeof(T)) != hipSuccess) { (void)hipGetLastError(); *out = nullptr; return false; }
      ptrs.push_back(p);
      *out = (T *)p;
      return true;
   }
};

template <class T> static bool sp_alloc_out(T **out, size_t count) {
   void *p = nullptr;
   if (hipMalloc(&p, (count ? count : 1) * sizeof(T)) != hipSuccess) { (void)hipGetLastError(); *out = nullptr; return false; }
   *out = (T *)p;
   return true;
}

static hipError_t sp_sort(void *temp, size_t &temp_bytes, const uint32_t *kin, uint32_t *kout, const uint32_t *vin, uint32_t *vout,
                          size_t n, unsigned bits, hipStream_t st) {
   return sort_pairs_u32(temp, temp_bytes, kin, kout, vin, vout, n, 0u, bits, st);
}

}

using namespace isplib;

extern "C" void isplib_stream_plan_free(isplib_stream_plan *plan) {
   if (!plan) return;
   (void)hipDeviceSynchronize();
   (void)hipFree(const_cast<int32_t *>(plan->words)); (void)hipFree(const_cast<float *>(plan->vals));
   (void)hipFree(const_cast<int64_t *>(plan->wave_step_off)); (void)hipFree(const_cast<int32_t *>(plan->wave_row));
   (void)hipFree(const_cast<int32_t *>(plan->wave_part)); (void)hipFree(const_cast<int32_t *>(plan->hub_row));
   (void)hipFree(const_cast<int32_t *>(plan->hub_off)); (void)hipFree(const_cast<int32_t *>(plan->perm));
   memset(plan, 0, sizeof(*plan));
}

extern "C" int isplib_stream_plan_set_values_hip(isplib_stream_plan *plan, const float *val, void *stream) {
   clear_error();
   if (!plan || !plan->perm) return fail(ISPLIB_FAIL, "isplib_stream_plan_set_values_hip: not a plan built by isplib_stream_plan_build_hip");
   const int64_t n_words = plan->n_steps * plan->streams;
   if (!val) {
      if (plan->vals) { (void)hipStreamSynchronize((hipStream_t)stream); (void)hipFree(const_cast<float *>(plan->vals)); plan->vals = nullptr; }
      return ISPLIB_SUCCESS;
   }
   if (!plan->vals) {
      float *v = nullptr;
      if (!sp_alloc_out(&v, (size_t)n_words)) return fail(ISPLIB_NOT_ENOUGH_MEM, "isplib_stream_plan_set_values_hip: device allocation failed");
      plan->vals = v;
   }
   if (n_words > 0) {
      hipLaunchKernelGGL(sp_gather_vals_kernel, dim3(sp_grid(n_words)), dim3(256), 0, (hipStream_t)stream, n_words, plan->perm, val,
                         const_cast<float *>(plan->vals));
      return check_launch("sp_gather_vals_kernel");
   }
   return ISPLIB_SUCCESS;
}

static int stream_plan_build(int64_t m, int64_t n, int64_t nnz, const int64_t *rowptr, const int64_t *col, const float *val,
                             int streams, int rpw, int resident, int slices, int chunk, int waves_per_gen,
                             isplib_stream_plan *out, void *stream, int pad_row = -1, const uint32_t *caps = nullptr) {
   if (!out) return fail(ISPLIB_FAIL, "isplib_stream_plan_build_hip: out is NULL");
   memset(out, 0, sizeof(*out));
   if (m <= 0 || n <= 0 || nnz < 0 || !rowptr || (nnz > 0 && !col)) return fail(ISPLIB_FAIL, "isplib_stream_plan_build_hip: bad operand");
   if (n >= ISPLIB_STREAM_N_END || nnz >= ISPLIB_STREAM_NNZ_END || m >= (1LL << 31)) return fail(ISPLIB_FAIL, "isplib_stream_plan_build_hip: n < 2^24, nnz < 2^31, m < 2^31 required");
   if (slices < 1 || slices > 4096 || chunk < 1 || chunk >= (1 << 24)) return fail(ISPLIB_FAIL, "isplib_stream_plan_build_hip: slices in [1, 4096], chunk in [1, 2^24)");
   if (waves_per_gen <= 0) waves_per_gen = resident;
   const int per = rpw / streams;
   hipStream_t st = (hipStream_t)stream;
   SpTemp T;
   if (caps) {
      bool equal = true;
      for (int w = 0; w < waves_per_gen; w++) {
         if (caps[w] < ISPLIB_STREAM_CAP_ONE / 16 || caps[w] > ISPLIB_STREAM_CAP_ONE * 16)
            return fail(ISPLIB_FAIL, "isplib_stream_plan_build_caps_hip: a capacity outside [ISPLIB_STREAM_CAP_ONE / 16, ISPLIB_STREAM_CAP_ONE * 16]");
         equal = equal && caps[w] == caps[0];
      }
      if (equal) caps = nullptr;
   }
   int *nchunk, *hub_flag, *first, *hub_idx;
   if (!T.alloc(&nchunk, (size_t)m) || !T.alloc(&hub_flag, (size_t)m) || !T.alloc(&first, (size_t)m + 1) || !T.alloc(&hub_idx, (size_t)m + 1))
      return fail(ISPLIB_NOT_ENOUGH_MEM, "isplib_stream_plan_build_hip: device allocation failed");
   hipLaunchKernelGGL(sp_row_chunks_kernel, dim3(sp_grid(m)), dim3(256), 0, st, m, (int64_t)chunk, rowptr, nchunk, hub_flag);
   int rc = check_launch("sp_row_chunks_kernel");
   if (rc) return rc;
   size_t scan_bytes = 0;
   ISPLIB_HIP_TRY(scan_exclusive_i32(nullptr, scan_bytes, nullptr, nullptr, (size_t)m, st));
   void *scan_tmp;
   {
      char *p;
      if (!T.alloc(&p, scan_bytes + 256)) return fail(ISPLIB_NOT_ENOUGH_MEM, "isplib_stream_plan_build_hip: device allocation failed");
      scan_tmp = p;
   }
   size_t sb = scan_bytes;
   ISPLIB_HIP_TRY(scan_exclusive_i32(scan_tmp, sb, (const int *)nchunk, first, (size_t)m, st));
   sb = scan_bytes;
   ISPLIB_HIP_TRY(scan_exclusive_i32(scan_tmp, sb, (const int *)hub_flag, hub_idx, (size_t)m, st));
   int last[4];
   ISPLIB_HIP_TRY(hipMemcpyAsync(&last[0], first + (m - 1), sizeof(int), hipMemcpyDeviceToHost, st));
   ISPLIB_HIP_TRY(hipMemcpyAsync(&last[1], nchunk + (m - 1), sizeof(int), hipMemcpyDeviceToHost, st));
   ISPLIB_HIP_TRY(hipMemcpyAsync(&last[2], hub_idx + (m - 1), sizeof(int), hipMemcpyDeviceToHost, st));
   ISPLIB_HIP_TRY(hipMemcpyAsync(&last[3], hub_flag + (m - 1), sizeof(int), hipMemcpyDeviceToHost, st));
   ISPLIB_HIP_TRY(hipStreamSynchronize(st));
   const int64_t nv = (int64_t)last[0] + last[1], n_hub = (int64_t)last[2] + last[3];
   const int64_t per_gen = (int64_t)waves_per_gen * rpw;
   const int64_t gens = (nv + per_gen - 1) / per_gen;
   const int64_t nw = gens * waves_per_gen, ns = nw * streams;
   if (gens > 4096 || ns >= (1LL << 31) || (double)ns * slices * per >= 4294967295.0)
      return fail(ISPLIB_FAIL, "isplib_stream_plan_build_hip: graph too large for this geometry (32-bit stream keys)");
   int *vrow_row, *vlen, *vhub, *part_of, *sid, *rnd;
   uint32_t *k_in, *k_out, *v_in, *v_out, *loads, *lk_out, *lv_in, *lv_out, *lk_in = nullptr, *d_caps = nullptr;
   const size_t big = (size_t)(nnz > nv ? nnz : nv) + 1;
   if (!T.alloc(&vrow_row, (size_t)nv) || !T.alloc(&vlen, (size_t)nv) || !T.alloc(&vhub, (size_t)nv) || !T.alloc(&part_of, (size_t)nv + 1) ||
       !T.alloc(&sid, (size_t)nv) || !T.alloc(&rnd, (size_t)nv) || !T.alloc(&k_in, big) || !T.alloc(&k_out, big) || !T.alloc(&v_in, big) ||
       !T.alloc(&v_out, big) || !T.alloc(&loads, (size_t)ns) || !T.alloc(&lk_out, (size_t)ns) || !T.alloc(&lv_in, (size_t)ns) ||
       !T.alloc(&lv_out, (size_t)ns))
      return fail(ISPLIB_NOT_ENOUGH_MEM, "isplib_stream_plan_build_hip: device allocation failed");
// ... 103 lines not shown
   }
   SP_TRY(hipStreamSynchronize(st));
#undef SP_FAIL
#undef SP_TRY
#undef SP_LAUNCHED
   out->rows = m; out->cols = n; out->slices = slices; out->gens = (int32_t)gens; out->waves_per_gen = waves_per_gen;
   out->rows_per_wave = rpw; out->streams = streams; out->chunk = chunk;
   out->n_steps = n_steps; out->n_parts = n_parts; out->n_hub = n_hub;
   return ISPLIB_SUCCESS;
}

namespace isplib {
constexpr int SP_CALIB_DEGREE = 512, SP_CALIB_COLS = 2;
constexpr double SP_CAP_CLAMP = 0.08;
static std::mutex g_caps_mutex;
static std::map<std::tuple<int, int, int>, std::vector<uint32_t>> g_caps;

static void caps_from_ticks(int streams, int waves_per_gen, const double *ticks, uint32_t *caps) {
   const int wgs_per_cu = with_streams<STREAM_SUM>(streams, [&](auto s) {
      constexpr StreamGeom ge = stream_geom(STREAM_SUM, s());
      return lds_wgs_per_cu(stream_lds_bytes(ge.lpr, ge.nvmax), ge.wgs);
   });
   const int nwg = waves_per_gen / 4;
   std::vector<double> sum((size_t)8 * wgs_per_cu, 0.0);
   std::vector<int> cnt((size_t)8 * wgs_per_cu, 0);
   double all = 0.0;
   auto group = [&](int w) { const int wg = w / 4; return (wg % 8) * wgs_per_cu + (int)((int64_t)wg * wgs_per_cu / nwg); };
   for (int w = 0; w < waves_per_gen; w++) { sum[group(w)] += ticks[w]; cnt[group(w)]++; all += ticks[w]; }
   for (int w = 0; w < waves_per_gen; w++) {
      double f = all > 0.0 && cnt[group(w)] ? (sum[group(w)] / cnt[group(w)]) / (all / waves_per_gen) - 1.0 : 0.0;
      f = f > SP_CAP_CLAMP ? SP_CAP_CLAMP : (f < -SP_CAP_CLAMP ? -SP_CAP_CLAMP : f);
      caps[w] = (uint32_t)((double)ISPLIB_STREAM_CAP_ONE / (1.0 + f) + 0.5);
   }
}
}

extern "C" int isplib_stream_calibrate_raw(int streams, int waves_per_gen, int launches, int degree, int col_mult, double *wave_ticks , void *stream) {
   clear_error();
   int rpw = 0, resident = 0;
   if (isplib_spmm_stream_geometry(streams, &rpw, &resident) != ISPLIB_SUCCESS) return ISPLIB_FAIL;
   if (!wave_ticks) return fail(ISPLIB_FAIL, "isplib_stream_calibrate_raw: wave_ticks is NULL");
   std::lock_guard<std::mutex> lock(g_caps_mutex);
   return stream_kernel_calibrate(streams, waves_per_gen, launches, degree, col_mult, wave_ticks, (hipStream_t)stream);
}

extern "C" int isplib_stream_capacities_hip(int device, int streams, int waves_per_gen, int64_t nnz, uint32_t *caps, int *levelled, void *stream) {
   clear_error();
   if (levelled) *levelled = 0;
   int rpw = 0, resident = 0;
   if (isplib_spmm_stream_geometry(streams, &rpw, &resident) != ISPLIB_SUCCESS) return ISPLIB_FAIL;
   if (waves_per_gen <= 0) waves_per_gen = resident;
   if (!caps) return fail(ISPLIB_FAIL, "isplib_stream_capacities_hip: caps is NULL");
   for (int w = 0; w < waves_per_gen; w++) caps[w] = ISPLIB_STREAM_CAP_ONE;
   const int mode = stream_level_mode();
   if (mode == 0 || waves_per_gen != resident || resident % 32 != 0 || (mode == 2 && nnz < STREAM_MIN_NNZ)) return ISPLIB_SUCCESS;
   int current = 0;
   ISPLIB_HIP_TRY(hipGetDevice(&current));
   if (device < 0) device = current;
   std::lock_guard<std::mutex> lock(g_caps_mutex);
   const auto key = std::make_tuple(device, streams, waves_per_gen);
   auto it = g_caps.find(key);
   if (it == g_caps.end()) {
      std::vector<double> ticks((size_t)waves_per_gen);
      if (device != current) ISPLIB_HIP_TRY(hipSetDevice(device));
      const int rc = stream_kernel_calibrate(streams, waves_per_gen, 3, SP_CALIB_DEGREE, SP_CALIB_COLS, ticks.data(), device == current ? (hipStream_t)stream : (hipStream_t) nullptr);
      if (device != current) (void)hipSetDevice(current);
      if (rc == ISPLIB_NOT_ENOUGH_MEM) { clear_error(); return ISPLIB_SUCCESS; }
      if (rc) return rc;
      std::vector<uint32_t> c((size_t)waves_per_gen);
      caps_from_ticks(streams, waves_per_gen, ticks.data(), c.data());
      it = g_caps.emplace(key, std::move(c)).first;
   }
   memcpy(caps, it->second.data(), (size_t)waves_per_gen * sizeof(uint32_t));
   if (levelled) *levelled = 1;
   return ISPLIB_SUCCESS;
}

extern "C" int isplib_stream_plan_build_caps_hip(int64_t m, int64_t n, int64_t nnz, const int64_t *rowptr, const int64_t *col,
                                                 const float *val, int streams, int slices, int chunk, int waves_per_gen,
                                                 const uint32_t *caps, isplib_stream_plan *out, void *stream) {
   clear_error();
   int rpw = 0, resident = 0;
   if (isplib_spmm_stream_geometry(streams, &rpw, &resident) != ISPLIB_SUCCESS) return ISPLIB_FAIL;
   return stream_plan_build(m, n, nnz, rowptr, col, val, streams, rpw, resident, slices, chunk, waves_per_gen, out, stream, -1, caps);
}

extern "C" int isplib_stream_plan_build_hip(int64_t m, int64_t n, int64_t nnz, const int64_t *rowptr, const int64_t *col,
                                            const float *val, int streams, int slices, int chunk, int waves_per_gen,
                                            isplib_stream_plan *out, void *stream) {
   clear_error();
   int rpw = 0, resident = 0, levelled = 0;
   if (isplib_spmm_stream_geometry(streams, &rpw, &resident) != ISPLIB_SUCCESS) return ISPLIB_FAIL;
   std::vector<uint32_t> caps((size_t)(waves_per_gen > 0 ? waves_per_gen : resident));
   const int rc = isplib_stream_capacities_hip(-1, streams, waves_per_gen, nnz, caps.data(), &levelled, stream);
   if (rc) return rc;
   return stream_plan_build(m, n, nnz, rowptr, col, val, streams, rpw, resident, slices, chunk, waves_per_gen, out, stream, -1,
                            levelled ? caps.data() : nullptr);
}

__global__ __launch_bounds__(256) void sp_unsorted_kernel(int64_t m, int64_t nnz, const int64_t *__restrict__ rowptr,
                                                          const int64_t *__restrict__ col, int *__restrict__ flag) {
   const int64_t stride = (int64_t)gridDim.x * blockDim.x;
   bool bad = false;
   for (int64_t e = (int64_t)blockIdx.x * blockDim.x + threadIdx.x + 1; e < nnz; e += stride)
      if (col[e] < col[e - 1] && e > rowptr[sp_row_of(e, m, rowptr)]) bad = true;
   if (bad) atomicOr(flag, 1);
}

extern "C" int isplib_stream_plan_build_minmax_hip(int64_t m, int64_t n, int64_t nnz, const int64_t *rowptr, const int64_t *col,
                                                   const float *val, int streams, int slices, int chunk, int waves_per_gen,
                                                   isplib_stream_plan *out, void *stream) {
   clear_error();
   int rpw = 0, resident = 0;
   if (isplib_spmm_stream_minmax_geometry(streams, &rpw, &resident) != ISPLIB_SUCCESS) return ISPLIB_FAIL;
   if (out) memset(out, 0, sizeof(*out));
   if (m <= 0 || nnz < 0 || !rowptr || (nnz > 0 && !col)) return fail(ISPLIB_FAIL, "isplib_stream_plan_build_minmax_hip: bad operand");
   if (nnz > 1) {
      int *flag = nullptr, host = 1;
      if (hipMalloc((void **)&flag, 256) != hipSuccess) { (void)hipGetLastError(); return fail(ISPLIB_NOT_ENOUGH_MEM, "isplib_stream_plan_build_minmax_hip: device allocation failed"); }
      hipStream_t st = (hipStream_t)stream;
      bool ok = hipMemsetAsync(flag, 0, sizeof(int), st) == hipSuccess;
      if (ok) {
         hipLaunchKernelGGL(sp_unsorted_kernel, dim3(sp_grid(nnz)), dim3(256), 0, st, m, nnz, rowptr, col, flag);
         ok = hipGetLastError() == hipSuccess && hipMemcpyAsync(&host, flag, sizeof(int), hipMemcpyDeviceToHost, st) == hipSuccess &&
              hipStreamSynchronize(st) == hipSuccess;
      }
      (void)hipFree(flag);
      if (!ok) return hip_fail(hipGetLastError(), "isplib_stream_plan_build_minmax_hip: sortedness check");
      if (host) return fail(ISPLIB_FAIL, "isplib_stream_plan_build_minmax_hip: rows are not column-sorted (use the task list)");
   }
   return stream_plan_build(m, n, nnz, rowptr, col, val, streams, rpw, resident, slices, chunk, waves_per_gen, out, stream,  rpw);
}

extern "C" int isplib_stream_plan_build_fusedmm_hip(int64_t m, int64_t n, int64_t nnz, const int64_t *rowptr, const int64_t *col,
                                                    int streams, int slices, int chunk, int waves_per_gen,
                                                    isplib_stream_plan *out, void *stream) {
   clear_error();
   int rpw = 0, resident = 0;
   if (isplib_fusedmm_stream_geometry(streams, &rpw, &resident) != ISPLIB_SUCCESS) return ISPLIB_FAIL;
   return stream_plan_build(m, n, nnz, rowptr, col, nullptr, streams, rpw, resident, slices, chunk, waves_per_gen, out, stream,  rpw);
}
```

### isplib_amd/csrc/sweep_common.h

```cpp
#pragma once
#include <hip/hip_runtime.h>
#include <stdint.h>
#include <float.h>
#include <limits.h>
#include <type_traits>

#include "../../include/isplib_hip.h"
#include "common.h"
#include "gather.h"

#ifndef ISPLIB_STREAM_NV4
#define ISPLIB_STREAM_NV4 64
#endif
#ifndef ISPLIB_STREAM_NBW4
#define ISPLIB_STREAM_NBW4 2
#endif
#ifndef ISPLIB_STREAM_WGS4
#define ISPLIB_STREAM_WGS4 2
#endif
#ifndef ISPLIB_EXP_GATHER_AUX
#define ISPLIB_EXP_GATHER_AUX 0
#endif
#ifndef ISPLIB_HYB4_NV
#define ISPLIB_HYB4_NV 64
// ... 9 lines not shown
#endif
#ifndef ISPLIB_HYB8_NV
#define ISPLIB_HYB8_NV 128
#endif
#ifndef ISPLIB_HYB8_NBW
#define ISPLIB_HYB8_NBW 4
#endif
#ifndef ISPLIB_HYB8_HT
#define ISPLIB_HYB8_HT 256
#endif
#ifndef ISPLIB_HYB8_HWR
#define ISPLIB_HYB8_HWR 8
#endif
#ifndef ISPLIB_STREAM_NV8
#define ISPLIB_STREAM_NV8 128
#endif
#ifndef ISPLIB_STREAM_NBW8
#define ISPLIB_STREAM_NBW8 4
#endif
#ifndef ISPLIB_STREAM_WGS8
#define ISPLIB_STREAM_WGS8 2
#endif
#ifndef ISPLIB_STREAM_MM_NV
#define ISPLIB_STREAM_MM_NV 32
#endif
#ifndef ISPLIB_STREAM_MM_NBW
#define ISPLIB_STREAM_MM_NBW 2
#endif
#ifndef ISPLIB_STREAM_MM_WGS
#define ISPLIB_STREAM_MM_WGS 2
#endif
#ifndef ISPLIB_STREAM_MM8_NV
#define ISPLIB_STREAM_MM8_NV 64
#endif
#ifndef ISPLIB_STREAM_MM8_NBW
#define ISPLIB_STREAM_MM8_NBW 4
#endif
#ifndef ISPLIB_STREAM_MM8_WGS
#define ISPLIB_STREAM_MM8_WGS 2
#endif

namespace isplib {

struct SweepArgs {
   int64_t k, nnz;
   const float *val;
   const int64_t *indx, *pntrb, *pntre;
   const int32_t *indx32;
   const float *y;
   int64_t ldy;
   unsigned ybytes;
   float *z;
   int64_t ldz;
   int64_t *z_arg;
   int mean;
   int empty_init;
   const int32_t *wave_row;
   const int32_t *wave_part;
   const int64_t *wave_task_off;
   const int64_t *task_b;
   const int32_t *task_meta;
   int wave_base, wave_count;
   const int32_t *words;
   const float *vals;
   const int64_t *wave_step_off;
   unsigned null_word;
   const int32_t *ids;
   int abs_ids;
   const int32_t *hot_rows;
   const int32_t *hot_words;
   const int64_t *hot_step_off;
   int slices;
   const float *g;
   int64_t ldg;
   float *dval;
   unsigned long long *dbg;
   float *part_val;
   int *part_idx;
   const int32_t *hub_row, *hub_off;
   int64_t n_hub;
   const float *ep_row_scale, *ep_self, *ep_bias;
   int64_t ep_ld_self;
   int ep_relu;
};

template <int OP, int VEC>
__device__ __forceinline__ void finish_row(const SweepArgs &a, int row, int c, float (&v)[VEC], int (&bi)[VEC], int64_t (&arg)[VEC]) {
   const int64_t rb = a.pntrb[row];
   const int64_t deg = a.pntre[row] - rb;
   if (OP == OP_ADD) {
      if (a.mean) {
         const float d = (float)(deg > 1 ? deg : 1);
#pragma unroll
         for (int i = 0; i < VEC; i++) v[i] = v[i] / d;
      }
      if (a.ep_self) {
         const float *sr = a.ep_self + (size_t)row * (size_t)a.ep_ld_self + c;
#pragma unroll
         for (int i = 0; i < VEC; i++) v[i] += sr[i];
      }
      if (a.ep_row_scale) {
         const float rs = a.ep_row_scale[row];
#pragma unroll
         for (int i = 0; i < VEC; i++) v[i] *= rs;
      }
      if (a.ep_bias) {
#pragma unroll
         for (int i = 0; i < VEC; i++) v[i] += a.ep_bias[c + i];
      }
      if (a.ep_relu) {
#pragma unroll
         for (int i = 0; i < VEC; i++) v[i] = v[i] > 0.0f ? v[i] : 0.0f;
      }
   } else {
#pragma unroll
      for (int i = 0; i < VEC; i++) {
         if (deg <= 0) v[i] = a.empty_init ? identity<OP>() : 0.0f;
         arg[i] = bi[i] == INT_MAX ? a.nnz : (a.abs_ids ? (int64_t)bi[i] : rb + (int64_t)bi[i]);
      }
   }
}

template <int OP, int VEC>
__global__ __launch_bounds__(256) void sweep_hub_fold_kernel(const SweepArgs a) {
   const int64_t kv = a.k / VEC;
   const int64_t total = a.n_hub * kv;
   const int64_t stride = (int64_t)gridDim.x * blockDim.x;
   for (int64_t i = (int64_t)blockIdx.x * blockDim.x + threadIdx.x; i < total; i += stride) {
      const int64_t h = i / kv;
      const int c = (int)(i - h * kv) * VEC;
      float v[VEC];
      int bi[VEC];
#pragma unroll
      for (int q = 0; q < VEC; q++) { v[q] = identity<OP>(); bi[q] = INT_MAX; }
      const int p1 = a.hub_off[h + 1];
      for (int p = a.hub_off[h]; p < p1; p++) {
         const size_t po = (size_t)p * (size_t)a.k + c;
         float t[VEC];
         load_vec<VEC>(a.part_val + po, t);
#pragma unroll
         for (int q = 0; q < VEC; q++) {
            if (OP == OP_ADD) {
               v[q] += t[q];
            } else {
               const int oi = a.z_arg ? a.part_idx[po + q] : p;
               const bool take = better<OP>(t[q], oi, v[q], bi[q]);
               v[q] = take ? t[q] : v[q];
               bi[q] = take ? oi : bi[q];
            }
         }
      }
      const int row = a.hub_row[h];
      int64_t arg[VEC];
      finish_row<OP, VEC>(a, row, c, v, bi, arg);
      store_vec<VEC>(a.z + (size_t)row * (size_t)a.ldz + c, v);
      if (OP != OP_ADD && a.z_arg) {
         int64_t *ar = a.z_arg + (size_t)row * (size_t)a.ldz + c;
#pragma unroll
         for (int q = 0; q < VEC; q++) ar[q] = arg[q];
      }
   }
}

template <int LPR_, int NVMAX_, int NBW_, int WAVES_ = 4>
struct StreamWave {
   static constexpr int LPR = LPR_, NVMAX = NVMAX_, NBW = NBW_, WAVES = WAVES_;
   static constexpr int G = 64 / LPR, PANEL = LPR * 4, U = 64 * NBW / G, PER = NVMAX / G;
   int lane, wave, g, lc;
   int wl;
   int64_t w;
   bool cok;
   int ccol, vfirst;
   unsigned cbyte, poison;
   int64_t s0, nwords;
   const int32_t *wp;
   unsigned ldyb;
};

template <class SW> __device__ __forceinline__ bool stream_wave_id(const SweepArgs &a, SW &sw) {
   sw.lane = threadIdx.x & 63;
   sw.wave = __builtin_amdgcn_readfirstlane(threadIdx.x >> 6);
   sw.g = sw.lane / SW::LPR;
   sw.lc = sw.lane % SW::LPR;
   sw.wl = (int)blockIdx.x * SW::WAVES + sw.wave;
   sw.w = (int64_t)a.wave_base + sw.wl;
   return sw.wl < a.wave_count;
}

template <bool RAGGED, class SW> __device__ __forceinline__ void stream_columns(const SweepArgs &a, SW &sw) {
   sw.cok = sw.lc * 4 < a.k;
   sw.ccol = sw.lc * 4;
   sw.vfirst = 0;
   if (RAGGED && sw.cok && sw.ccol + 4 > (int)a.k) { sw.vfirst = sw.ccol + 4 - (int)a.k; sw.ccol = (int)a.k - 4; }
   sw.cbyte = (unsigned)sw.ccol * 4u;
   sw.poison = sw.cok ? 0u : BUF_OOB;
}

template <class SW> __device__ __forceinline__ void stream_bounds(const SweepArgs &a, SW &sw) {
   sw.s0 = a.wave_step_off[sw.w];
   const int64_t s1 = a.wave_step_off[sw.w + 1];
   sw.nwords = (s1 - sw.s0) * SW::G;
   sw.wp = a.words + sw.s0 * SW::G;
   sw.ldyb = (unsigned)a.ldy * 4u;
}

template <class SW> __device__ __forceinline__ unsigned stream_pad_own_row(const SweepArgs &a, const SW &sw) {
   return ((unsigned)((sw.lane % SW::G) * SW::PER) << 24) | a.null_word;
}
template <class SW> __device__ __forceinline__ unsigned stream_pad_spare_row(const SweepArgs &a, const SW &) {
   return ((unsigned)SW::NVMAX << 24) | a.null_word;
}

template <class SW, class S, class T>
__device__ __forceinline__ void stream_load_batch(const SW &sw, const S *src, int64_t first, T pad, T (&reg)[SW::NBW]) {
#pragma unroll
   for (int q = 0; q < SW::NBW; q++) {
      const int64_t i = first + q * 64 + sw.lane;
      reg[q] = i < sw.nwords ? (T)src[i] : pad;
   }
}

template <int AUX, class SW>
__device__ __forceinline__ void stream_issue(const SW &sw, __amdgpu_buffer_rsrc_t rsrc, const unsigned (&word_l)[SW::NBW], int u, unsigned &la, v4i_t &t) {
   const unsigned word = (unsigned)__shfl((int)word_l[(u * SW::G) / 64], (u * SW::G) % 64 + sw.g);
   const unsigned o = (__umul24(word & 0xFFFFFFu, sw.ldyb) + sw.cbyte) | sw.poison;
   la = (word >> 24) * (unsigned)SW::PANEL;
   t = __builtin_amdgcn_raw_buffer_load_b128(rsrc, (int)o, 0, AUX);
}

__device__ __forceinline__ void stream_flush(float *lds_row, const float (&acc)[4]) {
   float4 *p = reinterpret_cast<float4 *>(lds_row);
   float4 o = *p;
   o.x += acc[0]; o.y += acc[1]; o.z += acc[2]; o.w += acc[3];
   *p = o;
}

enum StreamFamily { STREAM_SUM = 0, STREAM_MINMAX, STREAM_FUSEDMM, STREAM_HYBRID, STREAM_FAMILIES };
struct StreamGeom { int lpr, nvmax, nbw, wgs; bool two_planes; };
constexpr StreamGeom STREAM_GEOMS[STREAM_FAMILIES][3] = {
   {{32, 32, 1, 2, false},
    {16, ISPLIB_STREAM_NV4, ISPLIB_STREAM_NBW4, ISPLIB_STREAM_WGS4, false},
    {8, ISPLIB_STREAM_NV8, ISPLIB_STREAM_NBW8, ISPLIB_STREAM_WGS8, false}},
   {{32, 0, 0, 0, true},
    {16, ISPLIB_STREAM_MM_NV, ISPLIB_STREAM_MM_NBW, ISPLIB_STREAM_MM_WGS, true},
    {8, ISPLIB_STREAM_MM8_NV, ISPLIB_STREAM_MM8_NBW, ISPLIB_STREAM_MM8_WGS, true}},
   {{32, 16, 1, 2, true},
    {16, 32, 2, 2, true},
    {8, 64, 4, 2, true}},
   {{32, 0, 0, 0, false},
    {16, ISPLIB_HYB4_NV, ISPLIB_HYB4_NBW, 1, false},
    {8, ISPLIB_HYB8_NV, ISPLIB_HYB8_NBW, 1, false}},
};
constexpr bool stream_count_ok(int streams) { return streams == 2 || streams == 4 || streams == 8; }
constexpr StreamGeom stream_geom(int family, int streams) { return STREAM_GEOMS[family][streams == 2 ? 0 : (streams == 4 ? 1 : 2)]; }

template <int FAMILY, class F>
static inline int with_streams(int streams, F f) {
   if constexpr (stream_geom(FAMILY, 2).nvmax != 0) {
      if (streams == 2) return f(std::integral_constant<int, 2>());
   }
   if constexpr (stream_geom(FAMILY, 4).nvmax != 0) {
      if (streams == 4) return f(std::integral_constant<int, 4>());
   }
   return f(std::integral_constant<int, 8>());
}

constexpr int CU_LDS_BYTES = 163840;
constexpr int stream_lds_bytes(int lpr, int rows) { return 4 * rows * lpr * 4 * 4; }
constexpr int stream_lds_rows(const StreamGeom &ge) { return ge.two_planes ? 2 * (ge.nvmax + 1) : ge.nvmax; }
constexpr int lds_wgs_per_cu(int lds_bytes, int cap) { return CU_LDS_BYTES / lds_bytes < cap ? CU_LDS_BYTES / lds_bytes : cap; }
template <int LPR, int ROWS, int WGS> constexpr int stream_wgs_per_cu() { return lds_wgs_per_cu(stream_lds_bytes(LPR, ROWS), WGS); }
constexpr int stream_resident_waves(const StreamGeom &ge, int cus) {
   return cus * lds_wgs_per_cu(stream_lds_bytes(ge.lpr, stream_lds_rows(ge)), ge.wgs) * 4;
}

static inline int device_cus() {
   int dev = 0, cus = 0;
   if (hipGetDevice(&dev) != hipSuccess || hipDeviceGetAttribute(&cus, hipDeviceAttributeMultiprocessorCount, dev) != hipSuccess || cus <= 0) {
      (void)hipGetLastError();
      cus = 256;
   }
   return cus;
}

static inline int stream_geometry(const char *entry, int family, int streams, int *rows_per_wave, int *waves_resident) {
   clear_error();
   if (!stream_count_ok(streams) || !stream_geom(family, streams).nvmax)
      return fail(ISPLIB_FAIL, entry, stream_geom(family, 2).nvmax ? "streams must be 2, 4 or 8" : "streams must be 4 (64-column slots) or 8 (32-column slots)");
   const StreamGeom ge = stream_geom(family, streams);
   if (rows_per_wave) *rows_per_wave = ge.nvmax;
   if (waves_resident) *waves_resident = stream_resident_waves(ge, device_cus());
   return ISPLIB_SUCCESS;
}

constexpr int64_t STREAM_MIN_NNZ = 4 * 1048576;

static inline int suggest_stream_geom(int64_t m, int64_t n, int64_t nnz, int st, int rpw, int resident, double slice_bytes, double chunk_div,
                                      int *slices, int *chunk) {
   const int64_t per_gen = (int64_t)rpw * resident;
   const int64_t gens = (m + per_gen - 1) / per_gen;
   if ((double)nnz / (double)gens / 8.0 < 3.0 * (double)n) return 0;
   const double panel_bytes = 1024.0 / st;
   int sl = (int)((double)n * panel_bytes / slice_bytes + 0.5);
   sl = sl < 1 ? 1 : (sl > 512 ? 512 : sl);
   int64_t ch = (int64_t)((double)nnz / ((double)gens * resident * st) / chunk_div);
   ch = ch < 256 ? 256 : (ch > (1 << 20) ? (1 << 20) : ch);
   if (slices) *slices = sl;
   if (chunk) *chunk = (int)ch;
   return 1;
}

struct StreamCall {
   const char *entry;
   const char *instead;
   int family;
   int64_t m, n, k, nnz;
   bool empty;
   const int64_t *pntrb, *pntre;
   const isplib_stream_plan *plan;
   const float *y;
   int64_t ldy;
   int64_t ld_other;
   bool others;
   bool hub_fold;
   void *workspace;
   size_t workspace_bytes, workspace_need;
   int elt_bytes = 4;
};

static inline int check_stream_call(const StreamCall &c, bool *done) {
   const isplib_stream_plan *plan = c.plan;
   auto use_instead = [&](const char *what) {
      char msg[256];
      snprintf(msg, sizeof msg, "%s (use %s)", what, c.instead);
      return fail(ISPLIB_FAIL, c.entry, msg);
   };
   *done = true;
   if (c.m < 0 || c.n < 0 || c.k < 0 || c.nnz < 0) return fail(ISPLIB_FAIL, c.entry, "negative dimension");
   if (c.empty) return ISPLIB_SUCCESS;
   if (!plan) return fail(ISPLIB_FAIL, c.entry, "plan is required");
   if (plan->rows != c.m || plan->cols != c.n) return fail(ISPLIB_FAIL, c.entry, "the plan was built for another shape");
   if (c.n >= ISPLIB_STREAM_N_END || c.ldy >= ISPLIB_STREAM_LDY_END) return fail(ISPLIB_FAIL, c.entry, "n must be < 2^24 and ldy < 2^22 (24-bit address arithmetic)");
   if (!stream_count_ok(plan->streams)) return fail(ISPLIB_FAIL, c.entry, "bad plan geometry (streams 2, 4 or 8)");
   if (!stream_geom(c.family, plan->streams).nvmax) return fail(ISPLIB_FAIL, c.entry, "bad plan geometry (this entry runs on 4- or 8-stream plans)");
   if (plan->gens < 1 || plan->waves_per_gen < 1 || plan->rows_per_wave != stream_geom(c.family, plan->streams).nvmax)
      return fail(ISPLIB_FAIL, c.entry, "bad plan geometry (rows_per_wave must be what the geometry entry of this plan family reports)");
   if (c.k < ISPLIB_K_MIN) return use_instead("k >= 4 required");
   if (c.ldy < c.k || c.ld_other < c.k) return fail(ISPLIB_FAIL, c.entry, "leading dimension smaller than k");
   if (!isplib_rows_within(c.n, c.ldy, (uint64_t)ISPLIB_DENSE_BYTES_MAX * 4u / (uint64_t)c.elt_bytes)) return use_instead("dense operand larger than 3.5 GiB");
   if (!c.pntrb || !c.pntre || !c.y || !c.others || !plan->wave_row || !plan->wave_step_off || (plan->n_steps > 0 && !plan->words) ||
       (c.hub_fold && (!plan->wave_part || (plan->n_hub > 0 && (!plan->hub_row || !plan->hub_off)))))
      return fail(ISPLIB_FAIL, c.entry, "null operand");
   *done = false;
   return ISPLIB_SUCCESS;
}

static inline int check_stream_workspace(const StreamCall &c) {
   if (c.plan->n_parts <= 0) return ISPLIB_SUCCESS;
   if (!c.workspace || c.workspace_bytes < c.workspace_need) return fail(ISPLIB_NOT_ENOUGH_MEM, c.entry, "workspace too small");
   if (((uintptr_t)c.workspace & 255) != 0) return fail(ISPLIB_FAIL, c.entry, "workspace must be 256-byte aligned");
   return ISPLIB_SUCCESS;
}

static inline SweepArgs stream_args(const StreamCall &c, float *z, int64_t ldz) {
   const isplib_stream_plan *plan = c.plan;
   SweepArgs a = {};
   a.empty_init = empty_row_init();
   a.k = c.k; a.nnz = c.nnz; a.pntrb = c.pntrb; a.pntre = c.pntre;
   a.y = c.y; a.ldy = c.ldy; a.ybytes = (unsigned)((unsigned long long)c.n * (unsigned long long)c.ldy * 4ull); a.z = z; a.ldz = ldz;
   a.ids = plan->perm; a.abs_ids = 1;
   a.wave_row = plan->wave_row; a.wave_part = plan->wave_part;
   a.words = plan->words; a.vals = plan->vals; a.wave_step_off = plan->wave_step_off; a.null_word = (unsigned)c.n;
   a.hub_row = plan->hub_row; a.hub_off = plan->hub_off; a.n_hub = plan->n_hub;
   a.part_val = (float *)c.workspace;
   return a;
}

static inline int set_epilogue(const char *entry, const isplib_epilogue *ep, SweepArgs &a) {
   if (!ep) return ISPLIB_SUCCESS;
   if (ep->self && ep->ld_self < a.k) return fail(ISPLIB_FAIL, entry, "ld_self smaller than k");
   a.ep_row_scale = ep->row_scale; a.ep_self = ep->self; a.ep_ld_self = ep->ld_self; a.ep_bias = ep->bias;
   a.ep_relu = ep->relu ? 1 : 0;
   return ISPLIB_SUCCESS;
}

template <int OP, bool RAGGED>
static inline int launch_hub_fold(const SweepArgs &p, hipStream_t st) {
   if (p.n_hub <= 0) return ISPLIB_SUCCESS;
   const bool v4 = !RAGGED || ((p.k % 4) == 0 && (p.ldz % 4) == 0 && ((uintptr_t)p.z & 15) == 0 &&
                               (!p.ep_self || ((p.ep_ld_self % 4) == 0 && ((uintptr_t)p.ep_self & 15) == 0)));
   int64_t blocks = (p.n_hub * (v4 ? p.k / 4 : p.k) + 255) / 256;
   if (blocks > 4096) blocks = 4096;
   if (v4) hipLaunchKernelGGL((sweep_hub_fold_kernel<OP, 4>), dim3((unsigned)blocks), dim3(256), 0, st, p);
   else if constexpr (RAGGED) hipLaunchKernelGGL((sweep_hub_fold_kernel<OP, 1>), dim3((unsigned)blocks), dim3(256), 0, st, p);
   return check_launch("sweep_hub_fold_kernel");
}

template <class Launch>
static inline int run_generations(int gens, int waves_per_gen, SweepArgs &p, Launch launch) {
   for (int gen = 0; gen < gens; gen++) {
      p.wave_base = gen * waves_per_gen;
      p.wave_count = waves_per_gen;
      const int rc = launch(p);
      if (rc) return rc;
   }
   return ISPLIB_SUCCESS;
}

static inline size_t stream_parts_bytes(const isplib_stream_plan *plan) {
   if (!plan || plan->n_parts <= 0) return 256;
   const size_t pk = (size_t)(256 / (plan->streams > 0 ? plan->streams : 4));
   return ((size_t)plan->n_parts * pk * sizeof(float) + 255) & ~(size_t)255;
}

struct NoStage { int operator()(SweepArgs &, int64_t) const { return ISPLIB_SUCCESS; } };

template <class Launch, class Fold, class Stage>
static inline int run_stream_panels(const isplib_stream_plan *plan, const SweepArgs &a, Launch launch, Fold fold, Stage stage) {
   const int64_t k = a.k, pw = 256 / plan->streams;
   for (int64_t c0 = 0; c0 < k; c0 += pw) {
      SweepArgs p = a;
      p.k = (k - c0) < pw ? (k - c0) : pw;
      if (p.k < 4) {
         p.k = 4;
         c0 = k - 4;
      }
      p.y = a.y + c0;
      p.z = a.z + c0;
      p.ep_self = a.ep_self ? a.ep_self + c0 : nullptr;
      p.ep_bias = a.ep_bias ? a.ep_bias + c0 : nullptr;
      p.z_arg = a.z_arg ? a.z_arg + c0 : nullptr;
      p.ybytes = a.ybytes - (unsigned)c0 * 4u;
      int rc = stage(p, c0);
      if (!rc) rc = run_generations(plan->gens, plan->waves_per_gen, p, launch);
      if (!rc) rc = fold(p);
      if (rc) return rc;
   }
   return ISPLIB_SUCCESS;
}

}
```

### isplib_amd/csrc/torch_ops.cpp

```cpp
#include <ATen/ATen.h>
#include <c10/core/DeviceGuard.h>
#include <c10/hip/HIPStream.h>
#include <torch/csrc/autograd/custom_function.h>
#include <torch/library.h>

#include <hip/hip_runtime_api.h>

#include <cstdio>
#include <cstdlib>
#include <initializer_list>
#include <limits>
#include <mutex>
#include <tuple>
#include <unordered_map>
#include <vector>

#include "../../include/isplib_hip.h"

namespace {

using at::Tensor;
using c10::optional;
using torch::autograd::AutogradContext;
using torch::autograd::Variable;
// ... 20 lines not shown
bool is_half(const Tensor &t) { return t.defined() && (t.scalar_type() == at::kBFloat16 || t.scalar_type() == at::kHalf); }

void check_feature(const Tensor &t, const char *name) {
   TORCH_CHECK(t.defined(), "isplib: `", name, "` is missing");
   TORCH_CHECK(t.is_cuda(), "isplib: `", name, "` must be a GPU tensor -- isplib_amd has no CPU path");
   TORCH_CHECK(t.scalar_type() == at::kFloat || is_half(t), "isplib: `", name, "` must be float32, bfloat16 or float16");
}

Tensor as_float(const Tensor &t) { return t.defined() && t.scalar_type() != at::kFloat ? t.to(at::kFloat) : t; }

void *current_stream(const Tensor &t) { return (void *)c10::hip::getCurrentHIPStream(t.device().index()).stream(); }

struct OpTimer {
   const char *name;
   bool on;
   hipStream_t st = nullptr;
   hipEvent_t a = nullptr, b = nullptr;
   OpTimer(const char *n, const Tensor &t) : name(n) {
      static const bool enabled = [] { const char *e = std::getenv("ISPLIB_DEBUG"); return e && *e && *e != '0'; }();
      on = enabled && t.defined() && t.is_cuda();
      if (!on) return;
      st = (hipStream_t)current_stream(t);
      on = hipEventCreate(&a) == hipSuccess && hipEventCreate(&b) == hipSuccess && hipEventRecord(a, st) == hipSuccess;
   }
   ~OpTimer() {
      if (on && hipEventRecord(b, st) == hipSuccess && hipEventSynchronize(b) == hipSuccess) {
         float ms = 0.0f;
         if (hipEventElapsedTime(&ms, a, b) == hipSuccess) std::fprintf(stderr, "%s: %.3f ms\n", name, ms);
      }
      if (a) (void)hipEventDestroy(a);
      if (b) (void)hipEventDestroy(b);
   }
};

using Plan = std::vector<Tensor>;
static inline bool is_task_plan(const Plan &p) { return p.size() == 5 || p.size() == 6; }
static inline bool is_stream_plan(const Plan &p) { return p.size() == 8 || p.size() == 9; }
static inline Plan auto_plan() { return Plan{Tensor()}; }
static inline bool is_auto_plan(const Plan &p) { return p.size() == 1 && !p[0].defined(); }
static inline bool is_rows16_plan(const Plan &p) {
   return p.size() == 2 && p[0].defined() && p[0].scalar_type() == at::kInt && p[1].defined() && !p[1].is_cuda() &&
          p[1].scalar_type() == at::kInt && p[1].numel() == 1 && p[1].data_ptr<int32_t>()[0] == 16;
}
static inline bool is_rows16_colscale_plan(const Plan &p) {
   return p.size() == 3 && is_rows16_plan(Plan{p[0], p[1]}) && p[2].defined() && p[2].is_cuda() && p[2].scalar_type() == at::kFloat &&
          p[2].dim() == 1;
}
static inline bool is_rows16_da_plan(const Plan &p) {
   return p.size() == 3 && is_rows16_plan(Plan{p[0], p[1]}) && p[2].defined() && !p[2].is_cuda() && p[2].scalar_type() == at::kInt &&
          p[2].numel() == 1 && p[2].data_ptr<int32_t>()[0] == 0xDA;
}
static inline Plan forward_plan(const Plan &p) { return is_rows16_da_plan(p) ? Plan{p[0], p[1]} : p; }
static inline const int32_t *plan_col32(const Plan &p, const Tensor &col) {
   if (p.size() != 6) return nullptr;
   TORCH_CHECK(p[5].scalar_type() == at::kInt && p[5].numel() == col.numel() && p[5].device() == col.device(),
               "isplib: the plan's packed column ids do not match col");
   return p[5].data_ptr<int32_t>();
}
static isplib_stream_plan stream_plan_of(const Plan &plan) {
   const Tensor &words = plan[0], &vals = plan[1], &step_off = plan[2], &wave_row = plan[3], &wave_part = plan[4],
                &hub_row = plan[5], &hub_off = plan[6], &meta = plan[7];
   TORCH_CHECK(!meta.is_cuda() && meta.scalar_type() == at::kLong && meta.numel() == 11, "isplib: stream plan meta must be 11 host int64");
   TORCH_CHECK(words.is_cuda() && words.scalar_type() == at::kInt && step_off.scalar_type() == at::kLong &&
                   wave_row.scalar_type() == at::kInt && wave_part.scalar_type() == at::kInt &&
                   hub_row.scalar_type() == at::kInt && hub_off.scalar_type() == at::kInt &&
                   (vals.numel() == 0 || (vals.scalar_type() == at::kFloat && vals.numel() == words.numel())),
               "isplib: malformed stream plan");
   const int64_t *mt = meta.data_ptr<int64_t>();
   isplib_stream_plan sp;
   sp.rows = mt[0]; sp.cols = mt[1]; sp.slices = (int32_t)mt[2]; sp.gens = (int32_t)mt[3]; sp.waves_per_gen = (int32_t)mt[4];
   sp.rows_per_wave = (int32_t)mt[5]; sp.streams = (int32_t)mt[6]; sp.n_steps = mt[7]; sp.n_parts = mt[8]; sp.n_hub = mt[9]; sp.chunk = (int32_t)mt[10];
   TORCH_CHECK(words.numel() == sp.n_steps * sp.streams && step_off.numel() == (int64_t)sp.gens * sp.waves_per_gen + 1 &&
                   wave_row.numel() == (int64_t)sp.gens * sp.waves_per_gen * sp.rows_per_wave && wave_part.numel() == wave_row.numel() &&
                   hub_row.numel() == sp.n_hub && hub_off.numel() == sp.n_hub + 1,
               "isplib: stream plan arrays do not match its meta");
   sp.words = words.data_ptr<int32_t>();
   sp.vals = vals.numel() ? vals.data_ptr<float>() : nullptr;
   sp.wave_step_off = step_off.data_ptr<int64_t>();
   sp.wave_row = wave_row.data_ptr<int32_t>();
   sp.wave_part = wave_part.data_ptr<int32_t>();
   sp.hub_row = sp.n_hub ? hub_row.data_ptr<int32_t>() : nullptr;
   sp.hub_off = hub_off.data_ptr<int32_t>();
   sp.perm = nullptr;
   if (plan.size() == 9) {
      TORCH_CHECK(plan[8].is_cuda() && plan[8].scalar_type() == at::kInt && plan[8].numel() == words.numel(), "isplib: stream plan perm must be int32, one per word");
      sp.perm = plan[8].data_ptr<int32_t>();
   }
   return sp;
}

struct GraphCacheEntry {
   c10::weak_intrusive_ptr<c10::TensorImpl> rowptr, col, value;
   uint32_t v_rowptr = 0, v_col = 0, v_value = 0;
   bool has_value = false;
   isplib_graph *handle = nullptr;
   GraphCacheEntry(const Tensor &r, const Tensor &c, const Tensor &v)
       : rowptr(r.getIntrusivePtr()), col(c.getIntrusivePtr()), value(v.defined() ? v.getIntrusivePtr() : c.getIntrusivePtr()),
         v_rowptr(r._version()), v_col(c._version()), v_value(v.defined() ? v._version() : 0), has_value(v.defined()) {}
   bool alive() const { return !rowptr.expired() && !col.expired(); }
   bool same_structure(const Tensor &r, const Tensor &c) const {
      return rowptr.lock() == r.getIntrusivePtr() && col.lock() == c.getIntrusivePtr() && v_rowptr == r._version() && v_col == c._version();
   }
   bool same_values(const Tensor &v) const {
      return has_value == v.defined() && (!v.defined() || (value.lock() == v.getIntrusivePtr() && v_value == v._version()));
   }
   void remember_values(const Tensor &v, const Tensor &c) {
      value = c10::weak_intrusive_ptr<c10::TensorImpl>(v.defined() ? v.getIntrusivePtr() : c.getIntrusivePtr());
      v_value = v.defined() ? v._version() : 0;
      has_value = v.defined();
   }
};
struct GraphKey {
   const void *rowptr, *col;
   int64_t n;
   bool operator==(const GraphKey &o) const { return rowptr == o.rowptr && col == o.col && n == o.n; }
};
struct GraphKeyHash {
   size_t operator()(const GraphKey &k) const {
      return std::hash<const void *>()(k.rowptr) ^ (std::hash<const void *>()(k.col) << 1) ^ std::hash<int64_t>()(k.n);
   }
};
std::mutex g_graph_mutex;
std::unordered_map<GraphKey, GraphCacheEntry, GraphKeyHash> g_graphs;
std::vector<isplib_graph *> g_retired;

void retire_handle_locked(isplib_graph *h) { g_retired.push_back(h); }

void destroy_retired_locked() {
   for (isplib_graph *r : g_retired) isplib_graph_destroy(r);
   g_retired.clear();
}

isplib_graph *graph_handle_locked(const Tensor &rowptr, const Tensor &col, const Tensor &value, int64_t N, bool with_values = true) {
   const int64_t M = rowptr.numel() - 1, nnz = col.numel();
   const GraphKey key{rowptr.data_ptr(), col.data_ptr(), N};
   auto it = g_graphs.find(key);
   if (it != g_graphs.end() && !it->second.same_structure(rowptr, col)) {
      retire_handle_locked(it->second.handle);
      g_graphs.erase(it);
      it = g_graphs.end();
   }
   if (it == g_graphs.end()) {
      for (auto dead = g_graphs.begin(); dead != g_graphs.end();) {
         if (!dead->second.alive()) {
            retire_handle_locked(dead->second.handle);
            dead = g_graphs.erase(dead);
         } else {
            ++dead;
         }
      }
      destroy_retired_locked();
      const Tensor first = with_values ? value : Tensor();
      GraphCacheEntry e(rowptr, col, first);
      check_status(isplib_graph_create(M, N, nnz, rowptr.data_ptr<int64_t>(), col.data_ptr<int64_t>(),
                                       first.defined() ? first.data_ptr<float>() : nullptr, &e.handle),
                   "isplib_graph_create");
      it = g_graphs.emplace(key, std::move(e)).first;
   } else if (with_values && !it->second.same_values(value)) {
      check_status(isplib_graph_set_values(it->second.handle, value.defined() ? value.data_ptr<float>() : nullptr), "isplib_graph_set_values");
      it->second.remember_values(value, col);
   }
   return it->second.handle;
}

bool spmm_through_handle(int32_t msg, const Tensor &rowptr, const Tensor &col, const Tensor &value, const Tensor &mat,
                         Tensor &out, Tensor &arg) {
// ... 1625 lines not shown
```

### isplib_amd/plan.py

```python
from __future__ import annotations

import os
from dataclasses import dataclass
from typing import Optional

import torch

from . import cabi


@dataclass
class TaskPlan:
    slices: int
    n_tasks: int
    task_row: torch.Tensor
    task_b: torch.Tensor
    task_len: torch.Tensor
    seg_off: torch.Tensor
    lane_off: list
    chunk: int
    short_row: int
    col32: Optional[torch.Tensor] = None
    ncols: Optional[int] = None

# ... 94 lines not shown
    vlen = ve - vb
    gens = max(1, -(-nv // (waves_per_gen * rows_per_wave)))
    nw = gens * waves_per_gen
    order = torch.sort(vlen, descending=True, stable=True).indices
    rank = torch.empty(nv, **i64)
    rank[order] = torch.arange(nv, **i64)
    rnd, pos = rank // nw, rank % nw
    wave = torch.where(rnd % 2 == 0, pos, nw - 1 - pos)
    slot = rnd
    is_hub = nchunk[vrow] > 1
    part = torch.where(is_hub, torch.cumsum(is_hub.to(torch.int64), 0) - 1, torch.full((nv,), -1, **i64))
    wave_row = torch.full((nw * rows_per_wave,), -1, dtype=torch.int32, device=dev)
    wave_part = torch.full((nw * rows_per_wave,), -1, dtype=torch.int32, device=dev)
    at = wave * rows_per_wave + slot
    wave_row[at] = vrow.to(torch.int32)
    wave_part[at] = part.to(torch.int32)
    hub_rows = torch.nonzero(nchunk > 1).flatten()
    hub_off = torch.zeros(hub_rows.numel() + 1, dtype=torch.int32, device=dev)
    if hub_rows.numel():
        hub_off[1:] = torch.cumsum(nchunk[hub_rows], 0).to(torch.int32)
    s_r = (vlen // max(min_seg, 1)).clamp(min=1, max=slices)
    sl = torch.arange(slices, **i64)
    grp = (sl[None, :] * s_r[:, None]) // slices
    is_start = torch.ones((nv, slices), dtype=torch.bool, device=dev)
    is_start[:, 1:] = grp[:, 1:] != grp[:, :-1]
    e_slice = ((grp + 1) * slices + s_r[:, None] - 1) // s_r[:, None]
    tb = table[vrow]
    seg_b = torch.minimum(torch.maximum(tb[:, :-1], vb[:, None]), ve[:, None])
    seg_e = torch.minimum(torch.maximum(torch.gather(tb, 1, e_slice.clamp(max=slices)), vb[:, None]), ve[:, None])
    seg_len = seg_e - seg_b
    keep = is_start & (seg_len > 0)
    del grp, e_slice, tb, is_start
    vi, si = torch.nonzero(keep, as_tuple=True)
    t_b, t_len = seg_b[vi, si], seg_len[vi, si]
    del seg_b, seg_e, seg_len, keep
    t_wave, t_slot = wave[vi], slot[vi]
    key = (t_wave * slices + si) * rows_per_wave + t_slot
    perm = torch.sort(key).indices
    t_b, t_len, t_wave, t_slot = t_b[perm], t_len[perm], t_wave[perm], t_slot[perm]
    wave_task_off = torch.zeros(nw + 1, **i64)
    if t_wave.numel():
        wave_task_off[1:] = torch.cumsum(torch.bincount(t_wave, minlength=nw), 0)
    task_meta = ((t_slot << 24) | t_len).to(torch.int32)
    return dict(rows=m, slices=slices, gens=gens, waves_per_gen=waves_per_gen, rows_per_wave=rows_per_wave,
                n_tasks=int(t_b.numel()), n_parts=int(is_hub.sum()), n_hub=int(hub_rows.numel()), wave_row=wave_row,
                wave_part=wave_part, wave_task_off=wave_task_off, task_b=t_b.contiguous(), task_meta=task_meta.contiguous(),
                hub_row=hub_rows.to(torch.int32), hub_off=hub_off, chunk=chunk, min_seg=min_seg)


def build_sweep_plan(rowptr: torch.Tensor, col: torch.Tensor, ncols: int, slices: int, waves_per_gen: int,
                     rows_per_wave: int = 16, chunk: int = 2048, min_seg: int = 16,
                     col32: Optional[torch.Tensor] = None) -> Optional[SweepPlan]:
    table, ok = cabi.spmm_slices(rowptr, col, ncols, slices)
    if not ok:
        return None
    arrays = sweep_plan_arrays(rowptr, table, slices, waves_per_gen, rows_per_wave, chunk, min_seg)
    del table
    if col32 is None:
        col32 = cabi.pack_indices(col)
    return SweepPlan(col32=col32, **arrays)


@dataclass
class StreamPlan:
    rows: int
    cols: int
    slices: int
    gens: int
    waves_per_gen: int
    rows_per_wave: int
    streams: int
    n_steps: int
    n_parts: int
    n_hub: int
    words: torch.Tensor
    vals: Optional[torch.Tensor]
    perm: torch.Tensor
    wave_step_off: torch.Tensor
    wave_row: torch.Tensor
    wave_part: torch.Tensor
    hub_row: torch.Tensor
    hub_off: torch.Tensor
    chunk: int

    def struct(self) -> "cabi.StreamPlanStruct":
        p = lambda t: t.data_ptr() if t is not None and t.numel() else None
        return cabi.StreamPlanStruct(self.rows, self.cols, self.slices, self.gens, self.waves_per_gen, self.rows_per_wave,
                                     self.streams, int(self.chunk), self.n_steps, self.n_parts, self.n_hub, p(self.words), p(self.vals),
                                     p(self.wave_step_off), p(self.wave_row), p(self.wave_part), p(self.hub_row), p(self.hub_off),
                                     p(self.perm) if self.perm.dtype == torch.int32 else None)

    def workspace(self, minmax: bool = False) -> torch.Tensor:
        import ctypes
        ps = self.struct()
        L = cabi.lib()
        nbytes = (L.isplib_spmm_stream_minmax_workspace_bytes if minmax else L.isplib_spmm_stream_workspace_bytes)(ctypes.byref(ps))
        return torch.empty(nbytes, dtype=torch.uint8, device=self.words.device)

    def set_values(self, val: Optional[torch.Tensor]) -> None:
        if val is None:
            self.vals = None
            return
        ok = self.perm >= 0
        out = torch.zeros(self.perm.numel(), dtype=torch.float32, device=self.perm.device)
        out[ok] = val.detach().to(torch.float32)[self.perm[ok].to(torch.int64)]
        self.vals = out


def stream_plan_arrays(rowptr: torch.Tensor, col: torch.Tensor, ncols: int, slices: int, waves_per_gen: int,
                       rows_per_wave: int = 16, streams: int = 4, chunk: int = 2048, pad_row: Optional[int] = None,
                       capacities=None) -> dict:
    assert 1 <= slices <= 4096 and streams in (2, 4, 8) and waves_per_gen >= 1
    assert rows_per_wave % streams == 0 and rows_per_wave <= 128
    assert ncols < (1 << 24), "column ids share a 32-bit word with the local row and are multiplied in 24 bits"
    m = rowptr.numel() - 1
    dev = col.device
    i64 = dict(dtype=torch.int64, device=dev)
    nnz = col.numel()
    deg = rowptr[1:] - rowptr[:-1]
    nchunk = ((deg + chunk - 1) // chunk).clamp(min=1)
    nv = int(nchunk.sum())
    vrow = torch.repeat_interleave(torch.arange(m, **i64), nchunk)
    first = torch.cumsum(nchunk, 0) - nchunk
    ci = torch.arange(nv, **i64) - first[vrow]
    vlen = (deg[vrow] - ci + nchunk[vrow] - 1) // nchunk[vrow]
    erow = torch.repeat_interleave(torch.arange(m, **i64), deg)
    ev = first[erow] + (torch.arange(nnz, **i64) - rowptr[erow]) % nchunk[erow]
    del erow
    per = rows_per_wave // streams
    gens = max(1, -(-nv // (waves_per_gen * rows_per_wave)))
    nw = gens * waves_per_gen
    ns = nw * streams
    order = torch.sort(vlen, descending=True, stable=True).indices
    sid = torch.empty(nv, **i64)
    rnd = torch.empty(nv, **i64)
    loads = torch.zeros(ns, **i64)
    cap_s = None
    if capacities is not None:
        caps = torch.as_tensor(capacities, dtype=torch.int64).to(dev)
        assert caps.numel() == waves_per_gen and int(caps.min()) >= cabi.STREAM_CAP_ONE // 16 and int(caps.max()) <= cabi.STREAM_CAP_ONE * 16
        if bool((caps != caps[0]).any()):
            cap_s = caps[torch.arange(ns, **i64) // streams % waves_per_gen]
    for r in range(-(-nv // ns)):
        items = order[r * ns:(r + 1) * ns]
        keys = loads if cap_s is None else (loads * cabi.STREAM_CAP_ONE // cap_s).clamp(max=2 ** 32 - 1)
        to = torch.sort(keys, stable=True).indices[:items.numel()]
        sid[items] = to
        rnd[items] = r
        loads[to] += vlen[items]
    wave, slot = sid // streams, sid % streams
    lrow = slot * per + rnd
    is_hub = nchunk[vrow] > 1
    part = torch.where(is_hub, torch.cumsum(is_hub.to(torch.int64), 0) - 1, torch.full((nv,), -1, **i64))
    wave_row = torch.full((nw * rows_per_wave,), -1, dtype=torch.int32, device=dev)
    wave_part = torch.full((nw * rows_per_wave,), -1, dtype=torch.int32, device=dev)
    at = wave * rows_per_wave + lrow
    wave_row[at] = vrow.to(torch.int32)
    wave_part[at] = part.to(torch.int32)
    hub_rows = torch.nonzero(nchunk > 1).flatten()
    hub_off = torch.zeros(hub_rows.numel() + 1, dtype=torch.int32, device=dev)
    if hub_rows.numel():
        hub_off[1:] = torch.cumsum(nchunk[hub_rows], 0).to(torch.int32)
    width = -(-ncols // slices)
    if os.environ.get("ISPLIB_EXP_STREAM_ORDER") == "col":
        key = (sid[ev] * slices + col // width) * width + col % width
    elif pad_row is not None or os.environ.get("ISPLIB_EXP_SNAKE") == "1":
        sl = col // width
        key = (sid[ev] * slices + sl) * per + torch.where(sl % 2 == 1, per - 1 - rnd[ev], rnd[ev])
    else:
        key = (sid[ev] * slices + col // width) * per + rnd[ev]
    perm = torch.sort(key, stable=True).indices
    del key
    e_sid = sid[ev][perm]
    lens = torch.bincount(e_sid, minlength=ns)
    start = torch.cumsum(lens, 0) - lens
    p = torch.arange(nnz, **i64) - start[e_sid]
    steps = lens.view(nw, streams).max(dim=1).values
    wave_step_off = torch.zeros(nw + 1, **i64)
    wave_step_off[1:] = torch.cumsum(steps, 0)
    n_steps = int(wave_step_off[-1])
    idx = (wave_step_off[e_sid // streams] + p) * streams + e_sid % streams
    del p, start
    if pad_row is None:
        pad = ((torch.arange(streams, **i64) * per) << 24) | int(ncols)
    else:
        pad = torch.full((streams,), (int(pad_row) << 24) | int(ncols), **i64)
    pad = torch.where(pad >= 2 ** 31, pad - 2 ** 32, pad)
    words = pad.to(torch.int32).repeat(n_steps)
    words[idx] = ((lrow[ev][perm] << 24) | col[perm]).to(torch.int32)
    perm_out = torch.full((n_steps * streams,), -1, dtype=torch.int32 if nnz < 2 ** 31 else torch.int64, device=dev)
    perm_out[idx] = perm.to(perm_out.dtype)
    return dict(rows=m, cols=int(ncols), slices=slices, gens=gens, waves_per_gen=waves_per_gen, rows_per_wave=rows_per_wave,
                streams=streams, n_steps=n_steps, n_parts=int(is_hub.sum()), n_hub=int(hub_rows.numel()), words=words, vals=None,
                perm=perm_out, wave_step_off=wave_step_off, wave_row=wave_row, wave_part=wave_part,
                hub_row=hub_rows.to(torch.int32), hub_off=hub_off, chunk=chunk)


def build_stream_plan(rowptr: torch.Tensor, col: torch.Tensor, val: Optional[torch.Tensor], ncols: int, slices: int,
                      waves_per_gen: Optional[int] = None, rows_per_wave: Optional[int] = None, streams: int = 4,
                      chunk: int = 512, minmax: bool = False) -> Optional[StreamPlan]:
    if ncols >= cabi.STREAM_N_END:
        return None
    if minmax:
        if col.numel() > 1:
            starts = torch.zeros(col.numel(), dtype=torch.bool, device=col.device)
            starts[rowptr[:-1][rowptr[:-1] < col.numel()]] = True
            if bool(((col[1:] < col[:-1]) & ~starts[1:]).any()):
                return None
        rpw, resident = cabi.stream_minmax_geometry(streams)
    else:
        rpw, resident = cabi.stream_geometry(streams)
    rows_per_wave = rpw if rows_per_wave is None else rows_per_wave
    waves_per_gen = resident if waves_per_gen is None else waves_per_gen
    capacities = None if minmax or rows_per_wave != rpw else cabi.stream_capacities(col.device, streams, waves_per_gen, col.numel())
    plan = StreamPlan(**stream_plan_arrays(rowptr, col, ncols, slices, waves_per_gen, rows_per_wave, streams, chunk,
                                           pad_row=rows_per_wave if minmax else None, capacities=capacities))
    plan.set_values(val)
    return plan


def build_stream_plan_native(rowptr: torch.Tensor, col: torch.Tensor, ncols: int, slices: int, streams: int = 4,
                             chunk: int = 512, minmax: bool = False, waves_per_gen: int = 0, capacities=None) -> Optional[StreamPlan]:
    if ncols >= cabi.STREAM_N_END or col.numel() >= cabi.STREAM_NNZ_END:
        return None
    try:
        native = cabi.NativeStreamPlan(rowptr, col, None, ncols, streams, slices, chunk, waves_per_gen, minmax, capacities=capacities)
    except cabi.IsplibError as e:
        if e.status == cabi.ISPLIB_FAIL:
            return None
        if e.status == cabi.ISPLIB_NOT_ENOUGH_MEM:
            torch.cuda.empty_cache()
            return None
        raise
    i32, i64 = torch.int32, torch.int64
    plan = StreamPlan(rows=native.rows, cols=native.cols, slices=native.slices, gens=native.gens, waves_per_gen=native.waves_per_gen,
                      rows_per_wave=native.rows_per_wave, streams=native.streams, n_steps=native.n_steps, n_parts=native.n_parts,
                      n_hub=native.n_hub, words=native.view("words", i32), vals=None, perm=native.view("perm", i32),
                      wave_step_off=native.view("wave_step_off", i64), wave_row=native.view("wave_row", i32),
                      wave_part=native.view("wave_part", i32), hub_row=native.view("hub_row", i32),
                      hub_off=native.view("hub_off", i32), chunk=chunk)
    plan._native = native
    return plan


@dataclass
class HybridPlan:
    cold: StreamPlan
    table_rows: int
    hot_cap: int
    n_hot_steps: int
    hot_rows: torch.Tensor
    hot_words: torch.Tensor
    hot_step_off: torch.Tensor
    hot_perm: torch.Tensor
    hot_edges: int = 0

    def struct(self) -> "cabi.HybridPlanStruct":
        p = lambda t: t.data_ptr() if t is not None and t.numel() else None
        return cabi.HybridPlanStruct(self.cold.struct(), self.table_rows, self.hot_cap, self.n_hot_steps, p(self.hot_rows),
                                     p(self.hot_words), p(self.hot_step_off), p(self.hot_perm))

    def workspace(self) -> torch.Tensor:
        return self.cold.workspace()


def hybrid_plan_arrays(rowptr: torch.Tensor, col: torch.Tensor, ncols: int, slices: int, waves_per_gen: int, rows_per_wave: int,
                       streams: int, chunk: int, table_rows: int, hot_cap: int, min_refs: int = 2) -> dict:
    assert 1 <= slices <= 4096 and streams in (4, 8) and waves_per_gen >= 8 and waves_per_gen % 8 == 0
    assert rows_per_wave % streams == 0 and rows_per_wave <= 256 and 2 <= table_rows <= 65536 and hot_cap >= 1
    assert ncols < (1 << 24)
    m = rowptr.numel() - 1
    dev = col.device
    i64 = dict(dtype=torch.int64, device=dev)
    nnz = col.numel()
    assert nnz < 2 ** 31
    per = rows_per_wave // streams
    width = -(-ncols // slices)
    indeg = torch.bincount(col, minlength=ncols)
    cslice = torch.arange(ncols, **i64) // width
    top = int(indeg.max()) + 1 if ncols else 1
    order = torch.sort(cslice * top + (top - 1 - indeg), stable=True).indices
    s_sorted = cslice[order]
    counts = torch.bincount(cslice, minlength=slices)
    starts = torch.cumsum(counts, 0) - counts
    rank = torch.arange(ncols, **i64) - starts[s_sorted]
    is_top = (rank < table_rows - 1) & (indeg[order] >= min_refs)
    tidx = torch.full((ncols,), -1, **i64)
    tidx[order[is_top]] = rank[is_top]
    hot_rows = torch.full((slices * table_rows,), int(ncols), dtype=torch.int32, device=dev)
    hot_rows[s_sorted[is_top] * table_rows + rank[is_top]] = order[is_top].to(torch.int32)
    del order, s_sorted, rank, is_top, counts, starts, indeg, cslice
    e_hot = tidx[col] >= 0
    deg = rowptr[1:] - rowptr[:-1]
    nchunk = ((deg + chunk - 1) // chunk).clamp(min=1)
    nv = int(nchunk.sum())
    vrow = torch.repeat_interleave(torch.arange(m, **i64), nchunk)
    first = torch.cumsum(nchunk, 0) - nchunk
    erow = torch.repeat_interleave(torch.arange(m, **i64), deg)
    ev = first[erow] + (torch.arange(nnz, **i64) - rowptr[erow]) % nchunk[erow]
    del erow
    vlen = torch.bincount(ev[~e_hot], minlength=nv)
    gens = max(1, -(-nv // (waves_per_gen * rows_per_wave)))
    nw = gens * waves_per_gen
    ns = nw * streams
    order = torch.sort(vlen, descending=True, stable=True).indices
    sid = torch.empty(nv, **i64)
    rnd = torch.empty(nv, **i64)
    loads = torch.zeros(ns, **i64)
    for r in range(-(-nv // ns)):
        items = order[r * ns:(r + 1) * ns]
        to = torch.sort(loads, stable=True).indices[:items.numel()]
        sid[items] = to
        rnd[items] = r
        loads[to] += vlen[items]
    del order, loads
    wave, slot = sid // streams, sid % streams
    lrow = slot * per + rnd
    is_hub = nchunk[vrow] > 1
    part = torch.where(is_hub, torch.cumsum(is_hub.to(torch.int64), 0) - 1, torch.full((nv,), -1, **i64))
    wave_row = torch.full((nw * rows_per_wave,), -1, dtype=torch.int32, device=dev)
    wave_part = torch.full((nw * rows_per_wave,), -1, dtype=torch.int32, device=dev)
    at = wave * rows_per_wave + lrow
    wave_row[at] = vrow.to(torch.int32)
# ... 77 lines not shown
```

Measured before the change: 46.17 billion.

## Add compressed packed word stream for stream SpMM kernel

Adds a packed encoding of the stream plan's column/row words. Each 128-word batch is stored in 76 dwords instead of 128, holding a slice-relative 13-bit column, a 4-bit row nibble, slice-advance flags and a per-slot header. The stream kernel decodes this with ballots, popcounts and ds_bpermute. The aim is to cut index-stream memory traffic on large graphs, at the cost of extra ALU and cross-lane work per batch. Packing runs at plan build, is validated for representability, and is enabled automatically above a nnz threshold for the 4-stream, nbw=2, nvmax=64 geometry.

```diff
diff --git a/include/isplib_hip.h b/include/isplib_hip.h
--- a/include/isplib_hip.h
+++ b/include/isplib_hip.h
@@ -209,7 +209,15 @@
    const int32_t *hub_row;
    const int32_t *hub_off;
    const int32_t *perm;
+   const uint32_t *packed;
+   int32_t has_packed;
 } isplib_stream_plan;
+#define ISPLIB_STREAM_PACK_DWORDS 76
+#define ISPLIB_STREAM_PACK_COL_BITS 13
+#define ISPLIB_STREAM_PACK_MIN_WORDS (4 * 1048576)
+size_t isplib_stream_packed_dwords(const isplib_stream_plan *plan );
+int  isplib_stream_pack_hip(const isplib_stream_plan *plan , uint32_t *out , int64_t out_dwords,
+                            int *representable , void *stream);
 int  isplib_stream_plan_build_hip(int64_t m, int64_t n, int64_t nnz, const int64_t *rowptr, const int64_t *col,
                                   const float *val, int streams, int slices, int chunk, int waves_per_gen,
                                   isplib_stream_plan *out , void *stream);
diff --git a/isplib_amd/cabi.py b/isplib_amd/cabi.py
--- a/isplib_amd/cabi.py
+++ b/isplib_amd/cabi.py
@@ -171,7 +171,7 @@
     "isplib_sddmm_csr_tasks_hip", "fusedMM_csr_tasks_epilogue_hip", "fusedMM_csr_udef_hip", "fusedMM_csr_udef_tasks_hip", "isplib_pack_indices_hip",
     "isplib_suggest_slices", "isplib_graph_create", "isplib_graph_set_slices", "isplib_graph_set_values", "isplib_graph_spmm", "isplib_graph_spmm_backward",
     "isplib_graph_destroy", "isplib_suggest_slices_whole_rows", "isplib_graph_sddmm",
-    "fusedMM_csr_stream_hip", "isplib_spmm_stream_workspace_bytes", "isplib_spmm_stream_geometry", "isplib_suggest_stream", "isplib_suggest_stream_weighted", "isplib_stream_plan_build_hip", "isplib_stream_plan_build_caps_hip", "isplib_stream_capacities_hip", "isplib_stream_plan_build_minmax_hip", "fusedMM_csr_stream_minmax_hip", "isplib_spmm_stream_minmax_geometry", "isplib_suggest_stream_minmax", "isplib_spmm_stream_minmax_workspace_bytes", "isplib_stream_plan_set_values_hip", "isplib_stream_plan_free", "isplib_spmm_minmax_bw_det_hip", "isplib_spmm_minmax_bw_workspace_bytes", "isplib_scatter_rows_det_hip",
+    "fusedMM_csr_stream_hip", "isplib_spmm_stream_workspace_bytes", "isplib_spmm_stream_geometry", "isplib_suggest_stream", "isplib_suggest_stream_weighted", "isplib_stream_plan_build_hip", "isplib_stream_plan_build_caps_hip", "isplib_stream_capacities_hip", "isplib_stream_plan_build_minmax_hip", "fusedMM_csr_stream_minmax_hip", "isplib_spmm_stream_minmax_geometry", "isplib_suggest_stream_minmax", "isplib_spmm_stream_minmax_workspace_bytes", "isplib_stream_plan_set_values_hip", "isplib_stream_plan_free", "isplib_stream_packed_dwords", "isplib_stream_pack_hip", "isplib_spmm_minmax_bw_det_hip", "isplib_spmm_minmax_bw_workspace_bytes", "isplib_scatter_rows_det_hip",
     "isplib_minmax_bw_bucket_workspace_bytes", "isplib_minmax_bw_bucket_hip", "isplib_scatter_keys_workspace_bytes", "isplib_scatter_keys_det_hip",
     "isplib_fusedmm_stream_geometry", "isplib_suggest_fusedmm_stream", "isplib_stream_plan_build_fusedmm_hip", "fusedMM_csr_udef_stream_hip",
     "isplib_row_scale_hip", "isplib_masked_scale_colsum_hip", "isplib_masked_scale_colsum_workspace_bytes",
@@ -229,7 +229,8 @@
                 ("chunk", ctypes.c_int32), ("n_steps", ctypes.c_int64), ("n_parts", ctypes.c_int64), ("n_hub", ctypes.c_int64),
                 ("words", ctypes.c_void_p), ("vals", ctypes.c_void_p), ("wave_step_off", ctypes.c_void_p),
                 ("wave_row", ctypes.c_void_p), ("wave_part", ctypes.c_void_p),
-                ("hub_row", ctypes.c_void_p), ("hub_off", ctypes.c_void_p), ("perm", ctypes.c_void_p)]
+                ("hub_row", ctypes.c_void_p), ("hub_off", ctypes.c_void_p), ("perm", ctypes.c_void_p),
+                ("packed", ctypes.c_void_p), ("has_packed", ctypes.c_int32)]
 
 
 class HybridPlanStruct(ctypes.Structure):
@@ -363,6 +364,14 @@
                                                         _vp, ctypes.POINTER(StreamPlanStruct), _vp]
         L.isplib_stream_capacities_hip.restype = ctypes.c_int
         L.isplib_stream_capacities_hip.argtypes = [ctypes.c_int, ctypes.c_int, ctypes.c_int, _i64, _vp, ctypes.POINTER(ctypes.c_int), _vp]
+        L.isplib_stream_packed_dwords.restype = ctypes.c_size_t
+        L.isplib_stream_packed_dwords.argtypes = [ctypes.POINTER(StreamPlanStruct)]
+        L.isplib_stream_pack_hip.restype = ctypes.c_int
+        L.isplib_stream_pack_hip.argtypes = [ctypes.POINTER(StreamPlanStruct), _vp, _i64, ctypes.POINTER(ctypes.c_int), _vp]
+        L.isplib_stream_pack_set.restype = ctypes.c_int
+        L.isplib_stream_pack_set.argtypes = [ctypes.c_int]
+        L.isplib_stream_pack_last.restype = ctypes.c_int
+        L.isplib_stream_pack_last.argtypes = []
         L.isplib_stream_level_set.restype = ctypes.c_int
         L.isplib_stream_level_set.argtypes = [ctypes.c_int]
         L.isplib_stream_plan_build_minmax_hip.restype = ctypes.c_int
@@ -2667,6 +2676,9 @@
     def struct(self):
         return self._s
 
+    def packed_dwords(self) -> int:
+        return int(lib().isplib_stream_packed_dwords(ctypes.byref(self._s))) if self._s.has_packed else 0
+
     def workspace(self, minmax: bool = False):
         L = lib()
         nbytes = (L.isplib_spmm_stream_minmax_workspace_bytes if minmax else L.isplib_spmm_stream_workspace_bytes)(ctypes.byref(self._s))
@@ -2681,7 +2693,8 @@
         count, typestr = {"words": (self.n_steps * self.streams, "<i4"), "perm": (self.n_steps * self.streams, "<i4"),
                           "vals": (self.n_steps * self.streams, "<f4"), "wave_step_off": (nw + 1, "<i8"),
                           "wave_row": (nw * self.rows_per_wave, "<i4"), "wave_part": (nw * self.rows_per_wave, "<i4"),
-                          "hub_row": (self.n_hub, "<i4"), "hub_off": (self.n_hub + 1, "<i4")}[name]
+                          "hub_row": (self.n_hub, "<i4"), "hub_off": (self.n_hub + 1, "<i4"),
+                          "packed": (self.packed_dwords(), "<i4")}[name]
         ptr = getattr(self._s, name)
         if not ptr or count == 0:
             return torch.empty(0, device=self.device)
@@ -2692,7 +2705,7 @@
         count, typestr = {"words": (self.n_steps * self.streams, "<i4"), "perm": (self.n_steps * self.streams, "<i4"),
                           "wave_step_off": (nw + 1, "<i8"), "wave_row": (nw * self.rows_per_wave, "<i4"),
                           "wave_part": (nw * self.rows_per_wave, "<i4"), "hub_row": (self.n_hub, "<i4"),
-                          "hub_off": (self.n_hub + 1, "<i4")}[name]
+                          "hub_off": (self.n_hub + 1, "<i4"), "packed": (self.packed_dwords(), "<i4")}[name]
         ptr = getattr(self._s, name)
         if not ptr or count == 0:
             return torch.empty(0, dtype=dtype, device=self.device)
@@ -2728,6 +2741,27 @@
     return list(caps) if levelled.value else None
 
 
+def stream_pack(plan) -> Optional[torch.Tensor]:
+    ps = plan.struct()
+    ps.packed, ps.has_packed = None, 0
+    dwords = int(lib().isplib_stream_packed_dwords(ctypes.byref(ps)))
+    if dwords <= 0 or not plan.words.is_cuda:
+        return None
+    out = torch.empty(dwords, dtype=torch.int32, device=plan.words.device)
+    ok = ctypes.c_int(0)
+    with torch.cuda.device(out.device):
+        _check(lib().isplib_stream_pack_hip(ctypes.byref(ps), _ptr(out), dwords, ctypes.byref(ok), _stream(out.device)), "isplib_stream_pack_hip")
+    return out if ok.value else None
+
+
+def stream_pack_set(mode: int) -> None:
+    _check(lib().isplib_stream_pack_set(int(mode)), "isplib_stream_pack_set")
+
+
+def stream_pack_last() -> bool:
+    return bool(lib().isplib_stream_pack_last())
+
+
 def stream_level_set(mode: int) -> None:
     _check(lib().isplib_stream_level_set(int(mode)), "isplib_stream_level_set")
 
diff --git a/isplib_amd/csrc/common.h b/isplib_amd/csrc/common.h
--- a/isplib_amd/csrc/common.h
+++ b/isplib_amd/csrc/common.h
@@ -13,6 +13,9 @@
 int stream_stage_mode();
 void stream_stage_report(unsigned panels);
 int stream_kernel_calibrate(int streams, int waves_per_gen, int launches, int degree, int col_mult, double *wave_ticks, hipStream_t st);
+enum { ISPLIB_PACK_OFF = 0, ISPLIB_PACK_FORCE = 1, ISPLIB_PACK_AUTO = 2 };
+int stream_pack_mode();
+void stream_pack_report(int packed);
 int stream_level_mode();
 
 inline void clear_error() { error_buffer()[0] = '\0'; }
diff --git a/isplib_amd/csrc/runtime.hip b/isplib_amd/csrc/runtime.hip
--- a/isplib_amd/csrc/runtime.hip
+++ b/isplib_amd/csrc/runtime.hip
@@ -68,5 +68,27 @@
    return ISPLIB_SUCCESS;
 }
 
+namespace isplib {
+static int g_stream_pack = -1;
+static thread_local int g_stream_pack_last = 0;
+int stream_pack_mode() {
+   if (g_stream_pack < 0) {
+      const char *e = getenv("ISPLIB_STREAM_PACK");
+      g_stream_pack = !e ? ISPLIB_PACK_AUTO : strcmp(e, "0") == 0 ? ISPLIB_PACK_OFF : strcmp(e, "1") == 0 ? ISPLIB_PACK_FORCE : ISPLIB_PACK_AUTO;
+   }
+   return g_stream_pack;
+}
+void stream_pack_report(int packed) { g_stream_pack_last = packed; }
+}
+
+extern "C" int isplib_stream_pack_set(int mode) {
+   isplib::clear_error();
+   if (mode != isplib::ISPLIB_PACK_OFF && mode != isplib::ISPLIB_PACK_FORCE && mode != isplib::ISPLIB_PACK_AUTO)
+      return isplib::fail(ISPLIB_FAIL, "isplib_stream_pack_set: 0 (off), 1 (every plan that has a packed stream) or 2 (auto)");
+   isplib::g_stream_pack = mode;
+   return ISPLIB_SUCCESS;
+}
+extern "C" int isplib_stream_pack_last(void) { return isplib::g_stream_pack_last; }
+
 extern "C" int isplib_hip_abi_version(void) { return ISPLIB_HIP_ABI_VERSION; }
 extern "C" const char *isplib_hip_last_error(void) { return isplib::error_buffer(); }
diff --git a/isplib_amd/csrc/spmm_sweep.hip b/isplib_amd/csrc/spmm_sweep.hip
--- a/isplib_amd/csrc/spmm_sweep.hip
+++ b/isplib_amd/csrc/spmm_sweep.hip
@@ -6,7 +6,7 @@
 
 namespace isplib {
 
-template <int LPR, bool HAS_VAL, int NVMAX, int NBW, int WGS, bool TIMED = false>
+template <int LPR, bool HAS_VAL, int NVMAX, int NBW, int WGS, bool TIMED = false, bool PACKED = false>
 __global__ __launch_bounds__(256, (stream_wgs_per_cu<LPR, NVMAX, WGS>())) void spmm_stream_kernel(const SweepArgs a) {
    using Wave = StreamWave<LPR, NVMAX, NBW>;
    constexpr int WAVES = Wave::WAVES, G = Wave::G, PANEL = Wave::PANEL, U = Wave::U, PER = Wave::PER;
@@ -31,16 +31,32 @@
    v4i_t t[U];
    unsigned la[U];
    const unsigned pad_word = stream_pad_own_row(a, sw);
-   stream_load_batch(sw, sw.wp, 0, pad_word, w1);
+   const int64_t nb = (sw.nwords + 64 * NBW - 1) / (64 * NBW);
+   [[maybe_unused]] const uint32_t *pk = nullptr;
+   [[maybe_unused]] StreamPackLane pl;
+   if constexpr (PACKED) {
+      static_assert(!TIMED, "the TIMED instance reads the words");
+      pk = a.packed + ((sw.s0 * G) / (64 * NBW) + sw.w) * ISPLIB_STREAM_PACK_DWORDS;
+      pl = stream_pack_lane(sw);
+      stream_load_packed(sw, pk, 0, nb, w2);
+      stream_decode_packed<Wave>(pl, a.pack_width, pad_word, w2, w1);
+   } else {
+      stream_load_batch(sw, sw.wp, 0, pad_word, w1);
+   }
    if (HAS_VAL) stream_load_batch(sw, vp, 0, 0.0f, v0);
 #pragma unroll
    for (int u = 0; u < U; u++) stream_issue<ISPLIB_EXP_GATHER_AUX>(sw, rsrc, w1, u, la[u], t[u]);
-   stream_load_batch(sw, sw.wp, 64 * NBW, pad_word, w1);
+   if constexpr (PACKED) {
+      stream_load_packed(sw, pk, 1, nb, w2);
+      stream_decode_packed<Wave>(pl, a.pack_width, pad_word, w2, w1);
+   } else {
+      stream_load_batch(sw, sw.wp, 64 * NBW, pad_word, w1);
+   }
    if (HAS_VAL) stream_load_batch(sw, vp, 64 * NBW, 0.0f, v1);
-   stream_load_batch(sw, sw.wp, 128 * NBW, pad_word, w2);
+   if constexpr (PACKED) stream_load_packed(sw, pk, 2, nb, w2);
+   else stream_load_batch(sw, sw.wp, 128 * NBW, pad_word, w2);
    unsigned cur = (unsigned)(sw.g * PER * PANEL);
    float acc[4] = {0.0f, 0.0f, 0.0f, 0.0f};
-   const int64_t nb = (sw.nwords + 64 * NBW - 1) / (64 * NBW);
    if constexpr (TIMED) t_loop = __builtin_amdgcn_s_memtime();
    for (int64_t b = 0; b < nb; b++) {
       float vnext = HAS_VAL ? __shfl(v0[0], sw.g) : 0.0f;
@@ -61,8 +77,15 @@
          stream_issue<ISPLIB_EXP_GATHER_AUX>(sw, rsrc, w1, u, la[u], t[u]);
       }
 #pragma unroll
-      for (int q = 0; q < NBW; q++) { w1[q] = w2[q]; v0[q] = v1[q]; }
-      stream_load_batch(sw, sw.wp, (b + 3) * 64 * NBW, pad_word, w2);
+      for (int q = 0; q < NBW; q++) v0[q] = v1[q];
+      if constexpr (PACKED) {
+         stream_decode_packed<Wave>(pl, a.pack_width, pad_word, w2, w1);
+         stream_load_packed(sw, pk, b + 3, nb, w2);
+      } else {
+#pragma unroll
+         for (int q = 0; q < NBW; q++) w1[q] = w2[q];
+         stream_load_batch(sw, sw.wp, (b + 3) * 64 * NBW, pad_word, w2);
+      }
       if (HAS_VAL) stream_load_batch(sw, vp, (b + 2) * 64 * NBW, 0.0f, v1);
    }
    stream_flush(lane_base + cur, acc);
@@ -293,6 +316,12 @@
          return check_launch("spmm_stream_kernel");
       }
    }
+   if constexpr (STREAMS == 4 && ge.nbw == 2 && ge.nvmax == 64) {
+      if (a.packed) {
+         hipLaunchKernelGGL((spmm_stream_kernel<ge.lpr, HAS_VAL, ge.nvmax, ge.nbw, ge.wgs, false, true>), dim3(blocks), dim3(256), 0, st, a);
+         return check_launch("spmm_stream_kernel");
+      }
+   }
    hipLaunchKernelGGL((spmm_stream_kernel<ge.lpr, HAS_VAL, ge.nvmax, ge.nbw, ge.wgs>), dim3(blocks), dim3(256), 0, st, a);
    return check_launch("spmm_stream_kernel");
 }
@@ -396,6 +425,14 @@
    if ((rc = set_epilogue(entry, ep, a)) != ISPLIB_SUCCESS) return rc;
    hipStream_t st = (hipStream_t)stream;
    const bool has_val = plan->vals != nullptr;
+   const int pack_mode = mm ? ISPLIB_PACK_OFF : stream_pack_mode();
+   const bool packed = pack_mode != ISPLIB_PACK_OFF && plan->has_packed && plan->packed && plan->streams == 4 && plan->slices >= 1 &&
+                       (pack_mode == ISPLIB_PACK_FORCE || nnz >= ISPLIB_STREAM_PACK_MIN_WORDS);
+   if (packed) {
+      a.packed = plan->packed;
+      a.pack_width = (unsigned)((plan->cols + plan->slices - 1) / plan->slices);
+   }
+   if (!mm) stream_pack_report(packed ? 1 : 0);
    const int stage_mode = mm ? ISPLIB_STAGE_OFF : stream_stage_mode();
    float *stage_base = nullptr;
    uint64_t stage_room = 0;
diff --git a/isplib_amd/csrc/stream_plan.hip b/isplib_amd/csrc/stream_plan.hip
--- a/isplib_amd/csrc/stream_plan.hip
+++ b/isplib_amd/csrc/stream_plan.hip
@@ -182,6 +182,62 @@
    for (int64_t i = (int64_t)blockIdx.x * blockDim.x + threadIdx.x; i < n_words; i += stride) vals[i] = perm[i] >= 0 ? src[perm[i]] : 0.0f;
 }
 
+__global__ __launch_bounds__(256) void sp_pack_words_kernel(int64_t nw, int64_t nbatch_slots, unsigned width, unsigned n, const int32_t *__restrict__ words,
+                                                            const int64_t *__restrict__ wave_step_off, uint32_t *__restrict__ packed,
+                                                            int *__restrict__ bad) {
+   constexpr unsigned CM = (1u << ISPLIB_STREAM_PACK_COL_BITS) - 1u;
+   const int64_t stride = (int64_t)gridDim.x * blockDim.x;
+   for (int64_t i = (int64_t)blockIdx.x * blockDim.x + threadIdx.x; i < nbatch_slots; i += stride) {
+      const int64_t pb = i >> 2;
+      const unsigned slot = (unsigned)(i & 3);
+      int64_t lo = 0, hi = nw;
+      while (hi - lo > 1) {
+         const int64_t mid = lo + (hi - lo) / 2;
+         if ((wave_step_off[mid] * 4) / 128 + mid <= pb) lo = mid; else hi = mid;
+      }
+      const int64_t s0 = wave_step_off[lo], nwords = (wave_step_off[lo + 1] - s0) * 4;
+      const int64_t b = pb - ((s0 * 4) / 128 + lo);
+      if (b * 128 >= nwords) continue;
+      const int32_t *wp = words + s0 * 4 + b * 128;
+      const int64_t left = nwords - b * 128;
+      uint32_t *out = packed + pb * ISPLIB_STREAM_PACK_DWORDS;
+      const unsigned pad = ((slot * 16u) << 24) | n;
+      unsigned real = 0, base = 0, cur = 0, rows1[2] = {0u, 0u}, cols[16];
+      bool seen_pad = false, ok = true;
+#pragma unroll
+      for (int t = 0; t < 32; t++) {
+         const int e = t * 4 + (int)slot;
+         const unsigned w = e < left ? (unsigned)wp[e] : pad;
+         unsigned field = 0, row = 0, flag = 0;
+         if ((w & 0xFFFFFFu) == n) {
+            seen_pad = true;
+            ok = ok && w == pad;
+         } else {
+            ok = ok && !seen_pad;
+            const unsigned col = w & 0xFFFFFFu, sl = col / width;
+            if (real == 0) base = cur = sl;
+            flag = sl > cur ? 1u : 0u;
+            cur += flag;
+            field = col - cur * width;
+            row = (w >> 24) - slot * 16u;
+            ok = ok && sl >= cur && field <= CM && row < 16u && base < 4096u;
+            real = (unsigned)t + 1u;
+         }
+         if (t < 16) cols[t] = (field & CM) | ((row & 15u) << 26) | (flag << 30);
+         else {
+            cols[t - 16] |= ((field & CM) << ISPLIB_STREAM_PACK_COL_BITS) | (flag << 31);
+            rows1[(t - 16) >> 3] |= (row & 15u) << (((t - 16) & 7) * 4);
+         }
+      }
+#pragma unroll
+      for (int t = 0; t < 16; t++) out[t * 4 + (int)slot] = cols[t];
+      out[64 + slot * 2] = rows1[0];
+      out[64 + slot * 2 + 1] = rows1[1];
+      out[72 + slot] = (base & 0xFFFu) | (real << 12);
+      if (!ok) atomicOr(bad, 1);
+   }
+}
+
 struct SpTemp {
    std::vector<void *> ptrs;
    ~SpTemp() { for (void *p : ptrs) (void)hipFree(p); }
@@ -210,6 +266,59 @@
 
 using namespace isplib;
 
+static inline int64_t sp_packed_batches(const isplib_stream_plan *plan) {
+   const int64_t nw = (int64_t)plan->gens * plan->waves_per_gen;
+   return (plan->n_steps * 4) / 128 + nw + 1;
+}
+
+extern "C" size_t isplib_stream_packed_dwords(const isplib_stream_plan *plan) {
+   if (!plan || plan->streams != 4 || plan->rows_per_wave != 64 || plan->gens < 1 || plan->waves_per_gen < 1 || plan->n_steps < 0) return 0;
+   if (plan->slices < 1 || plan->slices > 4096 || plan->cols < 1 || plan->cols >= ISPLIB_STREAM_N_END) return 0;
+   if ((plan->cols + plan->slices - 1) / plan->slices > (1 << ISPLIB_STREAM_PACK_COL_BITS)) return 0;
+   return (size_t)sp_packed_batches(plan) * ISPLIB_STREAM_PACK_DWORDS;
+}
+
+extern "C" int isplib_stream_pack_hip(const isplib_stream_plan *plan, uint32_t *out, int64_t out_dwords, int *representable, void *stream) {
+   clear_error();
+   if (representable) *representable = 0;
+   const int64_t need = (int64_t)isplib_stream_packed_dwords(plan);
+   if (need <= 0) return fail(ISPLIB_FAIL, "isplib_stream_pack_hip: the plan's geometry has no packed form (isplib_stream_packed_dwords)");
+   if (!out || out_dwords < need || !representable) return fail(ISPLIB_FAIL, "isplib_stream_pack_hip: out of isplib_stream_packed_dwords(plan) dwords and representable are required");
+   if (!plan->wave_step_off || (plan->n_steps > 0 && !plan->words)) return fail(ISPLIB_FAIL, "isplib_stream_pack_hip: null operand");
+   hipStream_t st = (hipStream_t)stream;
+   int *bad = nullptr, host = 1;
+   if (hipMalloc((void **)&bad, 256) != hipSuccess) { (void)hipGetLastError(); return fail(ISPLIB_NOT_ENOUGH_MEM, "isplib_stream_pack_hip: device allocation failed"); }
+   hipError_t e = hipMemsetAsync(bad, 0, sizeof(int), st);
+   if (e == hipSuccess) e = hipMemsetAsync(out, 0, (size_t)need * sizeof(uint32_t), st);
+   if (e == hipSuccess) {
+      const int64_t nbs = sp_packed_batches(plan) * 4;
+      hipLaunchKernelGGL(sp_pack_words_kernel, dim3(sp_grid(nbs)), dim3(256), 0, st, (int64_t)plan->gens * plan->waves_per_gen, nbs,
+                         (unsigned)((plan->cols + plan->slices - 1) / plan->slices), (unsigned)plan->cols, plan->words, plan->wave_step_off, out, bad);
+      e = hipGetLastError();
+   }
+   if (e == hipSuccess) e = hipMemcpyAsync(&host, bad, sizeof(int), hipMemcpyDeviceToHost, st);
+   if (e == hipSuccess) e = hipStreamSynchronize(st);
+   (void)hipFree(bad);
+   if (e != hipSuccess) return hip_fail(e, "isplib_stream_pack_hip");
+   *representable = host ? 0 : 1;
+   return ISPLIB_SUCCESS;
+}
+
+static void sp_attach_packed(isplib_stream_plan *out, hipStream_t st) {
+   const int64_t dwords = (int64_t)isplib_stream_packed_dwords(out);
+   if (dwords <= 0) return;
+   uint32_t *packed = nullptr;
+   if (!sp_alloc_out(&packed, (size_t)dwords)) return;
+   int ok = 0;
+   if (isplib_stream_pack_hip(out, packed, dwords, &ok, st) != ISPLIB_SUCCESS || !ok) {
+      (void)hipFree(packed);
+      clear_error();
+      return;
+   }
+   out->packed = packed;
+   out->has_packed = 1;
+}
+
 extern "C" void isplib_stream_plan_free(isplib_stream_plan *plan) {
    if (!plan) return;
    (void)hipDeviceSynchronize();
@@ -217,6 +326,7 @@
    (void)hipFree(const_cast<int64_t *>(plan->wave_step_off)); (void)hipFree(const_cast<int32_t *>(plan->wave_row));
    (void)hipFree(const_cast<int32_t *>(plan->wave_part)); (void)hipFree(const_cast<int32_t *>(plan->hub_row));
    (void)hipFree(const_cast<int32_t *>(plan->hub_off)); (void)hipFree(const_cast<int32_t *>(plan->perm));
+   (void)hipFree(const_cast<uint32_t *>(plan->packed));
    memset(plan, 0, sizeof(*plan));
 }
 
@@ -486,7 +596,9 @@
    clear_error();
    int rpw = 0, resident = 0;
    if (isplib_spmm_stream_geometry(streams, &rpw, &resident) != ISPLIB_SUCCESS) return ISPLIB_FAIL;
-   return stream_plan_build(m, n, nnz, rowptr, col, val, streams, rpw, resident, slices, chunk, waves_per_gen, out, stream, -1, caps);
+   const int rc = stream_plan_build(m, n, nnz, rowptr, col, val, streams, rpw, resident, slices, chunk, waves_per_gen, out, stream, -1, caps);
+   if (rc == ISPLIB_SUCCESS) sp_attach_packed(out, (hipStream_t)stream);
+   return rc;
 }
 
 extern "C" int isplib_stream_plan_build_hip(int64_t m, int64_t n, int64_t nnz, const int64_t *rowptr, const int64_t *col,
@@ -498,8 +610,10 @@
    std::vector<uint32_t> caps((size_t)(waves_per_gen > 0 ? waves_per_gen : resident));
    const int rc = isplib_stream_capacities_hip(-1, streams, waves_per_gen, nnz, caps.data(), &levelled, stream);
    if (rc) return rc;
-   return stream_plan_build(m, n, nnz, rowptr, col, val, streams, rpw, resident, slices, chunk, waves_per_gen, out, stream, -1,
-                            levelled ? caps.data() : nullptr);
+   const int rc2 = stream_plan_build(m, n, nnz, rowptr, col, val, streams, rpw, resident, slices, chunk, waves_per_gen, out, stream, -1,
+                                     levelled ? caps.data() : nullptr);
+   if (rc2 == ISPLIB_SUCCESS) sp_attach_packed(out, (hipStream_t)stream);
+   return rc2;
 }
 
 __global__ __launch_bounds__(256) void sp_unsorted_kernel(int64_t m, int64_t nnz, const int64_t *__restrict__ rowptr,
diff --git a/isplib_amd/csrc/sweep_common.h b/isplib_amd/csrc/sweep_common.h
--- a/isplib_amd/csrc/sweep_common.h
+++ b/isplib_amd/csrc/sweep_common.h
@@ -115,6 +115,8 @@
    const float *ep_row_scale, *ep_self, *ep_bias;
    int64_t ep_ld_self;
    int ep_relu;
+   const uint32_t *packed;
+   unsigned pack_width;
 };
 
 template <int OP, int VEC>
@@ -251,6 +253,51 @@
       const int64_t i = first + q * 64 + sw.lane;
       reg[q] = i < sw.nwords ? (T)src[i] : pad;
    }
+}
+
+template <class SW>
+__device__ __forceinline__ void stream_load_packed(const SW &sw, const uint32_t *wave_packed, int64_t batch, int64_t nbatches, unsigned (&raw)[2]) {
+   static_assert(SW::NBW == 2 && SW::G == 4 && SW::PER == 16, "the packed stream is the 64-column sum geometry's: 128 words a batch, 16 rows a slot");
+   const uint32_t *p = wave_packed + batch * ISPLIB_STREAM_PACK_DWORDS;
+   const bool in = batch < nbatches;
+   raw[0] = in ? p[sw.lane] : 0u;
+   raw[1] = in && sw.lane < ISPLIB_STREAM_PACK_DWORDS - 64 ? p[64 + sw.lane] : 0u;
+}
+struct StreamPackLane {
+   unsigned row_hi;
+   unsigned mask_lo, mask_hi;
+   unsigned slot_lanes;
+   int nib_addr, hdr_addr;
+   unsigned nib_shift, step;
+};
+template <class SW> __device__ __forceinline__ StreamPackLane stream_pack_lane(const SW &sw) {
+   StreamPackLane pl;
+   const unsigned t = (unsigned)sw.lane >> 2, slot = (unsigned)sw.lane & 3u;
+   pl.row_hi = (slot * (unsigned)SW::PER) << 24;
+   pl.slot_lanes = 0x11111111u << slot;
+   pl.mask_lo = pl.slot_lanes & (sw.lane < 32 ? (2u << sw.lane) - 1u : 0xFFFFFFFFu);
+   pl.mask_hi = sw.lane < 32 ? 0u : pl.slot_lanes & ((2u << (sw.lane - 32)) - 1u);
+   pl.nib_addr = (int)(slot * 2u + (t >> 3)) * 4;
+   pl.hdr_addr = (int)(8u + slot) * 4;
+   pl.nib_shift = (t & 7u) * 4u;
+   pl.step = t;
+   return pl;
+}
+template <class SW>
+__device__ __forceinline__ void stream_decode_packed(const StreamPackLane &pl, unsigned width, unsigned pad_word, const unsigned (&raw)[2], unsigned (&reg)[2]) {
+   const unsigned d = raw[0];
+   const unsigned rows1 = (unsigned)__builtin_amdgcn_ds_bpermute(pl.nib_addr, (int)raw[1]);
+   const unsigned hdr = (unsigned)__builtin_amdgcn_ds_bpermute(pl.hdr_addr, (int)raw[1]);
+   const unsigned long long f0 = __ballot((d & 0x40000000u) != 0u), f1 = __ballot((int)d < 0);
+   const unsigned f0lo = (unsigned)f0, f0hi = (unsigned)(f0 >> 32), f1lo = (unsigned)f1, f1hi = (unsigned)(f1 >> 32);
+   const unsigned c0 = __popc(f0lo & pl.mask_lo) + __popc(f0hi & pl.mask_hi);
+   const unsigned c1 = __popc(f0lo & pl.slot_lanes) + __popc(f0hi & pl.slot_lanes) + __popc(f1lo & pl.mask_lo) + __popc(f1hi & pl.mask_hi);
+   const unsigned base = hdr & 0xFFFu, real = (hdr >> 12) & 0x3Fu;
+   constexpr unsigned CM = (1u << ISPLIB_STREAM_PACK_COL_BITS) - 1u;
+   const unsigned w0 = __umul24(base + c0, width) + (d & CM) + (pl.row_hi + (((d >> 26) & 15u) << 24));
+   const unsigned w1 = __umul24(base + c1, width) + ((d >> ISPLIB_STREAM_PACK_COL_BITS) & CM) + (pl.row_hi + (((rows1 >> pl.nib_shift) & 15u) << 24));
+   reg[0] = pl.step < real ? w0 : pad_word;
+   reg[1] = pl.step + 16u < real ? w1 : pad_word;
 }
 
 template <int AUX, class SW>
@@ -406,6 +453,7 @@
    a.words = plan->words; a.vals = plan->vals; a.wave_step_off = plan->wave_step_off; a.null_word = (unsigned)c.n;
    a.hub_row = plan->hub_row; a.hub_off = plan->hub_off; a.n_hub = plan->n_hub;
    a.part_val = (float *)c.workspace;
+   a.packed = nullptr;
    return a;
 }
 
diff --git a/isplib_amd/csrc/torch_ops.cpp b/isplib_amd/csrc/torch_ops.cpp
--- a/isplib_amd/csrc/torch_ops.cpp
+++ b/isplib_amd/csrc/torch_ops.cpp
@@ -126,6 +126,7 @@
    sp.hub_row = sp.n_hub ? hub_row.data_ptr<int32_t>() : nullptr;
    sp.hub_off = hub_off.data_ptr<int32_t>();
    sp.perm = nullptr;
+   sp.packed = nullptr; sp.has_packed = 0;
    if (plan.size() == 9) {
       TORCH_CHECK(plan[8].is_cuda() && plan[8].scalar_type() == at::kInt && plan[8].numel() == words.numel(), "isplib: stream plan perm must be int32, one per word");
       sp.perm = plan[8].data_ptr<int32_t>();
diff --git a/isplib_amd/plan.py b/isplib_amd/plan.py
--- a/isplib_amd/plan.py
+++ b/isplib_amd/plan.py
@@ -200,13 +200,15 @@
     hub_row: torch.Tensor
     hub_off: torch.Tensor
     chunk: int
+    packed: Optional[torch.Tensor] = None
 
     def struct(self) -> "cabi.StreamPlanStruct":
         p = lambda t: t.data_ptr() if t is not None and t.numel() else None
         return cabi.StreamPlanStruct(self.rows, self.cols, self.slices, self.gens, self.waves_per_gen, self.rows_per_wave,
                                      self.streams, int(self.chunk), self.n_steps, self.n_parts, self.n_hub, p(self.words), p(self.vals),
                                      p(self.wave_step_off), p(self.wave_row), p(self.wave_part), p(self.hub_row), p(self.hub_off),
-                                     p(self.perm) if self.perm.dtype == torch.int32 else None)
+                                     p(self.perm) if self.perm.dtype == torch.int32 else None,
+                                     p(self.packed), 1 if p(self.packed) else 0)
 
     def workspace(self, minmax: bool = False) -> torch.Tensor:
         import ctypes
@@ -334,7 +336,94 @@
     plan = StreamPlan(**stream_plan_arrays(rowptr, col, ncols, slices, waves_per_gen, rows_per_wave, streams, chunk,
                                            pad_row=rows_per_wave if minmax else None, capacities=capacities))
     plan.set_values(val)
+    if not minmax and streams == 4 and rows_per_wave == rpw:
+        plan.packed = cabi.stream_pack(plan)
     return plan
+
+
+STREAM_PACK_DWORDS = 76
+STREAM_PACK_COL_BITS = 13
+
+
+def stream_pack_batches(wave_step_off) -> int:
+    return int(wave_step_off[-1]) * 4 // 128 + (len(wave_step_off) - 1) + 1
+
+
+def stream_pack_words(words, wave_step_off, ncols: int, slices: int):
+    import numpy as np
+    words = np.asarray(words).astype(np.int64) & 0xFFFFFFFF
+    off = np.asarray(wave_step_off).astype(np.int64)
+    width = -(-int(ncols) // int(slices))
+    cm = (1 << STREAM_PACK_COL_BITS) - 1
+    ok = width <= cm + 1 and slices <= 4096
+    out = np.zeros(stream_pack_batches(off) * STREAM_PACK_DWORDS, dtype=np.uint32)
+    for w in range(len(off) - 1):
+        s0, nwords = int(off[w]), int(off[w + 1] - off[w]) * 4
+        first = s0 * 4 // 128 + w
+        for b in range(-(-nwords // 128)):
+            o = (first + b) * STREAM_PACK_DWORDS
+            for slot in range(4):
+                pad = ((slot * 16) << 24) | int(ncols)
+                real = base = cur = 0
+                seen_pad = False
+                for t in range(32):
+                    e = b * 128 + t * 4 + slot
+                    word = int(words[s0 * 4 + e]) if e < nwords else pad
+                    field = row = flag = 0
+                    if word & 0xFFFFFF == int(ncols):
+                        seen_pad = True
+                        ok = ok and word == pad
+                    else:
+                        col = word & 0xFFFFFF
+                        sl = col // width
+                        if real == 0:
+                            base = cur = sl
+                        flag = 1 if sl > cur else 0
+                        cur += flag
+                        field = col - cur * width
+                        row = (word >> 24) - slot * 16
+                        ok = ok and not seen_pad and sl >= cur and 0 <= field <= cm and 0 <= row < 16
+                        real = t + 1
+                    field, row = field & cm, row & 15
+                    lane = (t % 16) * 4 + slot
+                    if t < 16:
+                        out[o + lane] |= np.uint32(field | (row << 26) | (flag << 30))
+                    else:
+                        out[o + lane] |= np.uint32((field << STREAM_PACK_COL_BITS) | (flag << 31))
+                        out[o + 64 + slot * 2 + (t - 16) // 8] |= np.uint32(row << (((t - 16) % 8) * 4))
+                out[o + 72 + slot] = np.uint32((base & 0xFFF) | (real << 12))
+    return out, bool(ok)
+
+
+def stream_unpack_words(packed, wave_step_off, ncols: int, slices: int):
+    import numpy as np
+    packed = np.asarray(packed).view(np.uint32).astype(np.int64)
+    off = np.asarray(wave_step_off).astype(np.int64)
+    width = -(-int(ncols) // int(slices))
+    cm = (1 << STREAM_PACK_COL_BITS) - 1
+    words = np.zeros(int(off[-1]) * 4, dtype=np.int64)
+    lane = np.arange(64)
+    t, slot = lane >> 2, lane & 3
+    same_slot_upto = (slot[None, :] == slot[:, None]) & (lane[None, :] <= lane[:, None])
+    for w in range(len(off) - 1):
+        s0, nwords = int(off[w]), int(off[w + 1] - off[w]) * 4
+        first = s0 * 4 // 128 + w
+        for b in range(-(-nwords // 128)):
+            raw = packed[(first + b) * STREAM_PACK_DWORDS:(first + b + 1) * STREAM_PACK_DWORDS]
+            d = raw[:64]
+            rows1 = (raw[64 + slot * 2 + (t >> 3)] >> ((t & 7) * 4)) & 15
+            hdr = raw[72 + slot]
+            f0, f1 = (d >> 30) & 1, (d >> 31) & 1
+            c0 = (same_slot_upto * f0[None, :]).sum(axis=1)
+            c1 = np.array([f0[slot == g].sum() for g in slot]) + (same_slot_upto * f1[None, :]).sum(axis=1)
+            base, real = hdr & 0xFFF, (hdr >> 12) & 0x3F
+            pad = ((slot * 16) << 24) | int(ncols)
+            w0 = (base + c0) * width + (d & cm) + ((slot * 16 + ((d >> 26) & 15)) << 24)
+            w1 = (base + c1) * width + ((d >> STREAM_PACK_COL_BITS) & cm) + ((slot * 16 + rows1) << 24)
+            both = np.concatenate([np.where(t < real, w0, pad), np.where(t + 16 < real, w1, pad)])
+            n_here = min(128, nwords - b * 128)
+            words[s0 * 4 + b * 128:s0 * 4 + b * 128 + n_here] = both[:n_here]
+    return (words & 0xFFFFFFFF).astype(np.uint32).view(np.int32)
 
 
 def build_stream_plan_native(rowptr: torch.Tensor, col: torch.Tensor, ncols: int, slices: int, streams: int = 4,
@@ -356,7 +445,8 @@
                       n_hub=native.n_hub, words=native.view("words", i32), vals=None, perm=native.view("perm", i32),
                       wave_step_off=native.view("wave_step_off", i64), wave_row=native.view("wave_row", i32),
                       wave_part=native.view("wave_part", i32), hub_row=native.view("hub_row", i32),
-                      hub_off=native.view("hub_off", i32), chunk=chunk)
+                      hub_off=native.view("hub_off", i32), chunk=chunk,
+                      packed=native.view("packed", i32) if native.packed_dwords() else None)
     plan._native = native
     return plan
 
```

Measured after the change: 46.98 billion (median of 6 runs). +1.8%, better.
